# Simple-Robotics/aligator

Hardware: NVIDIA H100
Metric: riccati_knots_per_sec (higher is better)
Workload: dtype f64

## Files before the change

### aligator_b200/build.py

```python
from __future__ import annotations

import concurrent.futures as cf
import hashlib
import os
import re
import subprocess
import sys

PKG = os.path.dirname(os.path.abspath(__file__))
CSRC = os.path.join(PKG, "csrc")
OBJ = os.path.join(CSRC, "build")
LIB = os.path.join(PKG, "libaligator_b200_gar.so")
NVCC = os.environ.get("NVCC", "/usr/local/cuda/bin/nvcc")
ARCH = ["-gencode", "arch=compute_90a,code=sm_90a"]
FLAGS = ["-O3", "-lineinfo", "-std=c++17", "-Xcompiler", "-fPIC", "-ccbin", "/usr/bin/g++"]


def configs():
    txt = open(os.path.join(CSRC, "riccati_configs.h")).read()
    body = txt.split("#else", 1)[1]
    return [tuple(int(v) for v in m.groups())
            for m in re.finditer(r"X\((\d+),\s*(\d+),\s*(\d+),\s*(\d+)\)", body)]


def _digest(paths, extra=""):
    h = hashlib.sha256((" ".join(ARCH + FLAGS) + extra).encode())
    for p in paths:
        h.update(open(p, "rb").read())
    return h.hexdigest()[:16]


def _run(cmd):
    r = subprocess.run(cmd, capture_output=True, text=True)
    if r.returncode != 0:
        raise RuntimeError("build failed: %s\n%s\n%s" % (" ".join(cmd), r.stdout, r.stderr))
    return r.stdout + r.stderr


def build(verbose=False, force=False, ptxas_v=False):
    os.makedirs(OBJ, exist_ok=True)
    hdrs = [os.path.join(CSRC, f) for f in ("riccati_group.cuh", "riccati_launch.cuh", "riccati_configs.h")]
    hdrs.append(os.path.join(PKG, "..", "include", "aligator_b200", "gar.h"))
    hdrs_block = hdrs + [os.path.join(CSRC, f) for f in ("riccati_block.cuh", "riccati_block_launch.h",
                                                          "lq_assemble.h", "kkt_error.h", "linesearch.h",
                                                          "proxddp_inner.h")]
    extra = ["-Xptxas", "-v"] if ptxas_v else []
    jobs = []
    for (nx, nu, nc, g) in configs():
        src = os.path.join(CSRC, "kernel_inst.cu")
        tag = _digest(hdrs + [src], "%d_%d_%d_%d%s" % (nx, nu, nc, g, extra))
        obj = os.path.join(OBJ, "k_%d_%d_%d_%s.o" % (nx, nu, nc, tag))
        cmd = [NVCC] + ARCH + FLAGS + extra + ["-DAB2_NX=%d" % nx, "-DAB2_NU=%d" % nu, "-DAB2_NC=%d" % nc,
                                              "-DAB2_G=%d" % g, "-c", src, "-o", obj]
        jobs.append((obj, cmd))
    src = os.path.join(CSRC, "gar_cuda.cu")
    tag = _digest(hdrs_block + [src])
    obj = os.path.join(OBJ, "capi_%s.o" % tag)
    jobs.append((obj, [NVCC] + ARCH + FLAGS + ["-c", src, "-o", obj]))
    src = os.path.join(CSRC, "block_kernel.cu")
    obj = os.path.join(OBJ, "block_%s.o" % _digest(hdrs_block + [src], str(extra)))
    jobs.append((obj, [NVCC] + ARCH + FLAGS + extra + ["-c", src, "-o", obj]))
    src = os.path.join(CSRC, "kkt_error.cu")
    obj = os.path.join(OBJ, "kkt_%s.o" % _digest([os.path.join(CSRC, "kkt_error.h"), src], str(extra)))
    jobs.append((obj, [NVCC] + ARCH + FLAGS + extra + ["-c", src, "-o", obj]))
    src = os.path.join(CSRC, "lq_assemble.cu")
    obj = os.path.join(OBJ, "assemble_%s.o" % _digest([hdrs[-1], os.path.join(CSRC, "lq_assemble.h"), src], str(extra)))
    jobs.append((obj, [NVCC] + ARCH + FLAGS + extra + ["-c", src, "-o", obj]))
    src = os.path.join(CSRC, "linesearch.cu")
    obj = os.path.join(OBJ, "linesearch_%s.o" % _digest([os.path.join(CSRC, "linesearch.h"), src], str(extra)))
    jobs.append((obj, [NVCC] + ARCH + FLAGS + extra + ["-c", src, "-o", obj]))
    src = os.path.join(CSRC, "proxddp_inner.cu")
    obj = os.path.join(OBJ, "inner_%s.o" % _digest([hdrs[-1], os.path.join(CSRC, "proxddp_inner.h"), src], str(extra)))
    jobs.append((obj, [NVCC] + ARCH + FLAGS + extra + ["-c", src, "-o", obj]))
    todo =[(o, c) for (o, c) in jobs if force or not os.path.exists(o)]
    logs = []
    if todo:
        with cf.ThreadPoolExecutor(max_workers=max(1, min(len(todo), os.cpu_count() or 4))) as ex:
            for out in ex.map(lambda oc: _run(oc[1]), todo):
                logs.append(out)
    objs = [o for (o, _) in jobs]
    stamp = os.path.join(OBJ, "link.stamp")
    want = _digest(objs)
    if force or todo or not os.path.exists(LIB) or not os.path.exists(stamp) or open(stamp).read() != want:
        _run([NVCC] + ARCH + ["-shared", "-o", LIB] + objs + ["-ccbin", "/usr/bin/g++"])
        open(stamp, "w").write(want)
    keep = set(os.path.basename(o) for o in objs) | {"link.stamp"}
    for f in os.listdir(OBJ):
        if f not in keep:
            os.remove(os.path.join(OBJ, f))
    if verbose:
        print("\n".join(logs))
        print("built", LIB)
    return LIB


if __name__ == "__main__":
    build(verbose=True, force="--force" in sys.argv, ptxas_v="--ptxas" in sys.argv)
```

### aligator_b200/csrc/gar_cuda.cu

```cuda
#include <cuda_runtime.h>

#include <cstdio>
#include <cstdlib>
#include <cstring>
#include <string>
#include <vector>

#include "../../include/aligator_b200/gar.h"
#include "kkt_error.h"
#include "linesearch.h"
#include "lq_assemble.h"
#include "proxddp_inner.h"
#include "riccati_block_launch.h"
#include "riccati_configs.h"
#include "riccati_launch.cuh"

namespace ab2 {

__global__ void first_step_policy_kernel(const double *__restrict__ fb, const double *__restrict__ ff,
                                         double *__restrict__ dst, int batch, int N, int nr, int nu, int nx, int head) {
  const int per = nu * (nx + 1);
  for (long i = blockIdx.x * (long)blockDim.x + threadIdx.x; i < (long)batch * per; i += (long)gridDim.x * blockDim.x) {
    const int b = (int)(i / per), e = (int)(i % per), r = e / (nx + 1), c = e % (nx + 1);
    const size_t k0 = ((size_t)b * N + head) * nr + r;
    dst[i] = (c < nx) ? fb[k0 * nx + c] : ff[k0];
  }
}

constexpr int kMaxPeers = 8;
struct PeerPtrs {
  double *buf[kMaxPeers];
  unsigned long long *data_flag[kMaxPeers];
  unsigned long long *ack_flag[kMaxPeers];
};
__device__ __forceinline__ void st_release_sys(unsigned long long *p, unsigned long long v) {
  asm volatile("st.release.sys.global.u64 [%0], %1;" ::"l"(p), "l"(v) : "memory");
}
__device__ __forceinline__ unsigned long long ld_acquire_sys(const unsigned long long *p) {
  unsigned long long v;
  asm volatile("ld.acquire.sys.global.u64 %0, [%1];" : "=l"(v) : "l"(p) : "memory");
  return v;
}
__global__ void __launch_bounds__(256)
    policy_allgather_kernel(const double *__restrict__ fb, const double *__restrict__ ff, const PeerPtrs peers,
                            const int world, const int rank, const int batch, const int N, const int nr, const int nu,
                            const int nx, const unsigned long long step, unsigned int *done_counter) {
  const int per = nu * (nx + 1);
  const long total = (long)batch * per;
  if (threadIdx.x == 0) {
    if (step >= 3)
      for (int w = 0; w < world; ++w)
        while (ld_acquire_sys(peers.ack_flag[rank] + w) + 2 < step)
          __nanosleep(64);
  }
  __syncthreads();
  const size_t half = (size_t)(step % 3) * world * total;
  for (long i = blockIdx.x * (long)blockDim.x + threadIdx.x; i < total; i += (long)gridDim.x * blockDim.x) {
    const int b = (int)(i / per), e = (int)(i % per), r = e / (nx + 1), c = e % (nx + 1);
    const double v = (c < nx) ? fb[((size_t)b * N * nr + r) * nx + c] : ff[(size_t)b * N * nr + r];
    for (int w = 0; w < world; ++w)
      peers.buf[w][half + (size_t)rank * total + i] = v;
  }
  __threadfence_system();
  __syncthreads();
  if (threadIdx.x == 0) {
    const unsigned int prev = atomicAdd(done_counter, 1u);
    if (prev == gridDim.x - 1) {
      *done_counter = 0;
      __threadfence_system();
      for (int w = 0; w < world; ++w)
        st_release_sys(peers.data_flag[w] + rank, step);
    }
  }
}
__global__ void policy_publish_kernel(const PeerPtrs peers, const int world, const int rank, const unsigned long long step) {
  const int w = threadIdx.x;
  __threadfence_system();
  if (w < world) {
    st_release_sys(peers.data_flag[w] + rank, step);
    if (step >= 3)
      while (ld_acquire_sys(peers.ack_flag[rank] + w) + 2 < step)
        __nanosleep(64);
  }
}
__global__ void policy_wait_kernel(const PeerPtrs peers, const int world, const int rank, const unsigned long long step) {
  const int w = threadIdx.x;
  if (w < world) {
    st_release_sys(peers.ack_flag[w] + rank, step - 1);
    while (ld_acquire_sys(peers.data_flag[rank] + w) < step)
      __nanosleep(64);
  }
}

__global__ void gains_kernel(const double *__restrict__ fb, const double *__restrict__ ff, double *__restrict__ dst,
                             long nrec, int nr, int nx, int N, int head) {
  const int per = nr * (nx + 1);
  for (long i = blockIdx.x * (long)blockDim.x + threadIdx.x; i < nrec * per; i += (long)gridDim.x * blockDim.x) {
    long rec = i / per;
    if (head) {
      const long b = rec / N;
      const int t = (int)(rec % N) + head;
      rec = b * N + (t >= N ? t - N : t);
    }
    const int e = (int)(i % per), c = e / nr, r = e % nr;
    dst[i] = (c == 0) ? ff[rec * nr + r] : fb[(rec * nr + r) * nx + (c - 1)];
  }
}

__global__ void fddp_prep_kernel(const double *__restrict__ fs, double *__restrict__ slack, double *__restrict__ G0,
                                 double *__restrict__ g0, int batch, int N, int nx) {
  const long nS = (long)batch * N * nx, nG = (long)batch * nx * nx, ng = (long)batch * nx;
  for (long i = blockIdx.x * (long)blockDim.x + threadIdx.x; i < nS + nG + ng; i += (long)gridDim.x * blockDim.x) {
    if (i < nS) {
      const long b = i / ((long)N * nx), r = i % ((long)N * nx);
      slack[i] = fs[b * (N + 1) * nx + nx + r];
    } else if (i < nS + nG) {
      const long e = (i - nS) % ((long)nx * nx);
      G0[i - nS] = (e % nx == e / nx) ? -1.0 : 0.0;
    } else {
      const long j = i - nS - nG, b = j / nx, c = j % nx;
      g0[j] = fs[b * (N + 1) * nx + c];
    }
  }
}
__global__ void fddp_vx_kernel(const double *__restrict__ Vxx, const double *__restrict__ vx, const double *__restrict__ fs,
                               double *__restrict__ Vx_out, int batch, int N, int nx) {
  const long total = (long)batch * (N + 1) * nx;
  for (long i = blockIdx.x * (long)blockDim.x + threadIdx.x; i < total; i += (long)gridDim.x * blockDim.x) {
    const long kn = i / nx;
    const int r = (int)(i % nx);
    const double *V = Vxx + kn * nx * nx, *f = fs + kn * nx;
    double acc = 0.0;
    for (int c = 0; c < nx; ++c)
      acc += (r >= c ? V[r + (size_t)c * nx] : V[c + (size_t)r * nx]) * f[c];
    Vx_out[i] = vx[i] + acc;
  }
}
__global__ void fddp_quuks_kernel(const double *__restrict__ Ju, const double *__restrict__ Lu, const double *__restrict__ Vx,
                                  double *__restrict__ out, int batch, int N, int nx, int nu) {
  const long total = (long)batch * N * nu;
  for (long i = blockIdx.x * (long)blockDim.x + threadIdx.x; i < total; i += (long)gridDim.x * blockDim.x) {
    const long kn = i / nu, b = kn / N, t = kn % N;
    const int c = (int)(i % nu);
    const double *B = Ju + kn * nx * nu + (size_t)c * nx, *v = Vx + (b * (N + 1) + t + 1) * nx;
    double acc = Lu[i];
    for (int r = 0; r < nx; ++r)
      acc += B[r] * v[r];
    out[i] = -acc;
  }
}

#define X(NX, NU, NC, G) extern const KernelEntry kEntry_##NX##_##NU##_##NC;
AB2_FOR_EACH_CONFIG(X)
#undef X
static const KernelEntry *const kTable[] = {
#define X(NX, NU, NC, G) &kEntry_##NX##_##NU##_##NC,
    AB2_FOR_EACH_CONFIG(X)
#undef X
};

static const KernelEntry *find_kernel(int nx, int nu, int nc) {
  for (const KernelEntry *e : kTable)
    if (e->nx == nx && e->nu == nu && e->nc == nc)
      return e;
  return nullptr;
}

}

namespace {
thread_local std::string g_err;
int fail(int code, const std::string &msg) {
  g_err = msg;
  return code;
}
#define CUDA_TRY(expr)                                                                      \
  do {                                                                                      \
    cudaError_t _e = (expr);                                                                \
    if (_e != cudaSuccess)                                                                  \
      return fail(AB2_ERR_CUDA, std::string(#expr) + ": " + cudaGetErrorString(_e));        \
  } while (0)
}

struct ab2_gar_solver {
  ab2_gar_dims d;
  const ab2::KernelEntry *k;
  int srec, trec, nr;
  ab2::SweepParams p;
  double *own_stage = nullptr, *own_term = nullptr, *own_G0 = nullptr, *own_g0 = nullptr;
  double *own_stage_sym = nullptr;
  double *gains_tmp = nullptr, *kkt_tmp = nullptr, *theta_dev = nullptr, *ls_tmp = nullptr;
  double *fddp_slack = nullptr, *fddp_G0 = nullptr, *fddp_g0 = nullptr, *fddp_vx = nullptr;
  double *inner_tmp = nullptr;
  int nth = 0;
  int rec_nth = 0;
  int legs = 0;
  bool dense = false;
  int fac_head = 0;
  double *cond = nullptr;
  int pg_world = 0, pg_rank = 0;
  unsigned long long pg_step = 0;
  void *pg_local = nullptr;
  void *pg_peer_base[8] = {};
  ab2::PeerPtrs pg_ptrs{};
  unsigned int *pg_done = nullptr;
  size_t pg_buf_doubles = 0;
  unsigned long long pg_pushed_step = 0;
  bool pg_in_sweep = true;
  double *out[AB2_OUT_COUNT] = {};
  size_t out_doubles[AB2_OUT_COUNT] = {};
  size_t out_rec[AB2_OUT_COUNT] = {};
  int out_knots[AB2_OUT_COUNT] = {};
  int *status = nullptr, *pivstat = nullptr;
  bool have_problem = false, have_backward = false, have_forward = false;
  long launches = 0;
  int variant = -1;
  int group_doubles[4] = {0, 0, 0, 0};
  static constexpr int kPipeStreams = 4;
  cudaStream_t pipe_stream[kPipeStreams] = {};
  cudaEvent_t pipe_done[kPipeStreams] = {};
  cudaEvent_t pipe_fork = nullptr;
};

static size_t stage_total(const ab2_gar_solver *s) {
  return (size_t)s->d.batch * s->d.horizon * s->srec;
}

extern "C" {

const char *ab2_gar_last_error(void) { return g_err.c_str(); }
const char *ab2_gar_version(void) { return "aligator_b200 gar 0.1 (sm_90a)"; }

size_t ab2_gar_stage_record_doubles(int nx, int nu, int nc) {
  size_t n = 2 * (size_t)nx * nx + 2 * (size_t)nx * nu + (size_t)nu * nu + 2 * (size_t)nx + nu +
             (size_t)nc * (nx + nu + 1);
  return (n + 1) & ~(size_t)1;
}
size_t ab2_gar_term_record_doubles(int nx, int nct) {
  return (size_t)nx * nx + nx + (size_t)nct * nx + nct;
}
size_t ab2_gar_stage_record_doubles_th(int nx, int nu, int nc, int nth) {
  size_t n = 2 * (size_t)nx * nx + 2 * (size_t)nx * nu + (size_t)nu * nu + 2 * (size_t)nx + nu +
             (size_t)nc * (nx + nu + 1) + (size_t)nth * (nx + nu + nc + nth + 1);
  return (n + 1) & ~(size_t)1;
}
size_t ab2_gar_term_record_doubles_th(int nx, int nct, int nth) {
  return ab2_gar_term_record_doubles(nx, nct) + (size_t)nth * (nx + nct + nth + 1);
}
int ab2_gar_supported(int nx, int nu, int nc, int nc0) {
  if (nx < 1 || nu < 1 || nc < 0 || nc0 < 0)
    return 0;
  const ab2::KernelEntry *k = ab2::find_kernel(nx, nu, nc);
  if (k && nx + nc0 <= k->G)
    return 1;
  return ab2::block_supported(nx, nu, nc, nc0) ? 2 : 0;
}

static int create_impl(const ab2_gar_dims *dims, int nth, int legs, ab2_gar_solver **out);
int ab2_gar_create(const ab2_gar_dims *dims, ab2_gar_solver **out) { return create_impl(dims, 0, 0, out); }
int ab2_gar_create_parametric(const ab2_gar_dims *dims, int nth, ab2_gar_solver **out) {
  return create_impl(dims, nth, 0, out);
}
int ab2_gar_create_dense(const ab2_gar_dims *dims, ab2_gar_solver **out) { return create_impl(dims, 0, -1, out); }
int ab2_gar_create_parallel(const ab2_gar_dims *dims, int num_legs, ab2_gar_solver **out) {
  if (num_legs < 2)
    return fail(AB2_ERR_INVALID, "num_legs (" + std::to_string(num_legs) + ") should be greater than or equal to 2");
  if (dims && dims->horizon + 1 < num_legs)
    return fail(AB2_ERR_INVALID, "every leg needs at least one knot: horizon + 1 >= num_legs");
  return create_impl(dims, dims ? dims->nx : 0, num_legs, out);
}

static int create_impl(const ab2_gar_dims *dims, int nth, int legs, ab2_gar_solver **out) {
  if (!dims || !out)
    return fail(AB2_ERR_INVALID, "null argument");
  const ab2_gar_dims &d = *dims;
  if (d.nx < 1 || d.nu < 1 || d.nc < 0 || d.nct < 0 || d.nc0 < 0 || d.horizon < 0 || d.batch < 1 || nth < 0)
    return fail(AB2_ERR_INVALID, "bad dimensions");
  const bool dense = legs < 0;
  if (dense)
    legs = 0;
  const int rec_nth = legs > 1 ? 0 : nth;
  if (dense && !ab2::dense_supported(d.nx, d.nu, d.nc, d.nct, d.nc0))
    return fail(AB2_ERR_UNSUPPORTED, "the stage-dense KKT system (nu + nc + 2 nx rows) does not fit one CTA");
  const ab2::KernelEntry *k = ab2::find_kernel(d.nx, d.nu, d.nc);
  if (k && (d.nx + d.nc0 > k->G || nth > 0))
    k = nullptr;
  if (legs > 1 && !ab2::condensed_supported(d.nx, d.nc0, legs))
    return fail(AB2_ERR_UNSUPPORTED, "the condensed system of " + std::to_string(legs) + " legs does not fit one CTA's shared memory");
  if (!k && !ab2::block_supported(d.nx, d.nu, d.nc, d.nc0, nth))
    return fail(AB2_ERR_UNSUPPORTED,
                "(nx,nu,nc,nc0) = (" + std::to_string(d.nx) + "," + std::to_string(d.nu) + "," +
                    std::to_string(d.nc) + "," + std::to_string(d.nc0) +
                    ") does not fit one CTA (227 KB of shared memory, 256 rows)");
  int ndev = 0;
  CUDA_TRY(cudaGetDeviceCount(&ndev));
  if (d.device < 0 || d.device >= ndev)
    return fail(AB2_ERR_CUDA, "no such CUDA device");
  CUDA_TRY(cudaSetDevice(d.device));
  auto *s = new ab2_gar_solver();
  s->d = d;
  s->k = k;
  s->nth = nth;
  s->rec_nth = rec_nth;
  s->legs = legs;
  s->srec = (int)ab2_gar_stage_record_doubles_th(d.nx, d.nu, d.nc, rec_nth);
  if (k && k->srec_pad != s->srec) {
    delete s;
    return fail(AB2_ERR_INVALID, "internal: record size mismatch");
  }
  s->trec = (int)ab2_gar_term_record_doubles_th(d.nx, d.nct, rec_nth);
  s->nr = d.nu + d.nc + d.nx;
  s->dense = dense;
  if (dense) {
    s->k = nullptr;
    s->nr = d.nu + d.nc + 2 * d.nx;
  }
  if (s->k)
    s->k->group_doubles(d.nc0, s->group_doubles);
  const int N = d.horizon, B = d.batch, nx = d.nx;
  auto setup = [&](int what, size_t rec, int knots) {
    s->out_rec[what] = rec;
    s->out_knots[what] = knots;
    s->out_doubles[what] = (size_t)B * knots * rec;
  };
  setup(AB2_OUT_FF, s->nr, N);
  setup(AB2_OUT_FB, (size_t)s->nr * nx, N);
  setup(AB2_OUT_VXX, (size_t)nx * nx, N + 1);
  setup(AB2_OUT_VX, nx, N + 1);
  setup(AB2_OUT_FFT, d.nct, 1);
  setup(AB2_OUT_FBT, (size_t)d.nct * nx, 1);
  setup(AB2_OUT_KKT0, nx + d.nc0, 1);
  setup(AB2_OUT_XS, nx, N + 1);
  setup(AB2_OUT_US, d.nu, N);
  setup(AB2_OUT_VS, d.nc, N);
  setup(AB2_OUT_VST, d.nct, 1);
  setup(AB2_OUT_LBD0, d.nc0, 1);
  setup(AB2_OUT_LBDAS, nx, N);
  setup(AB2_OUT_FTH, (size_t)s->nr * nth, N);
  setup(AB2_OUT_VXT, (size_t)nx * nth, N + 1);
  setup(AB2_OUT_VTT, (size_t)nth * nth, N + 1);
  setup(AB2_OUT_VT, nth, N + 1);
  setup(AB2_OUT_KKT0FTH, (size_t)(nx + d.nc0) * nth, 1);
  setup(AB2_OUT_THGRAD, nth, 1);
  setup(AB2_OUT_THHESS, (size_t)nth * nth, 1);
  for (int w = 0; w < AB2_OUT_COUNT; ++w) {
    const size_t bytes = (s->out_doubles[w] > 0 ? s->out_doubles[w] + 2 : 2) * sizeof(double);
    cudaError_t e = cudaMalloc(&s->out[w], bytes);
    if (e == cudaSuccess)
      e = cudaMemset(s->out[w], 0, bytes);
    if (e != cudaSuccess) {
      ab2_gar_destroy(s);
      return fail(AB2_ERR_CUDA, std::string("cudaMalloc outputs: ") + cudaGetErrorString(e));
    }
  }
  {
    cudaError_t e = cudaMalloc(&s->status, sizeof(int) * B);
    if (e == cudaSuccess)
      e = cudaMemset(s->status, 0, sizeof(int) * B);
    if (e != cudaSuccess) {
      ab2_gar_destroy(s);
      return fail(AB2_ERR_CUDA, std::string("cudaMalloc status: ") + cudaGetErrorString(e));
    }
  }
  {
    cudaError_t e = cudaMalloc(&s->pivstat, sizeof(int) * B);
    if (e == cudaSuccess)
      e = cudaMemset(s->pivstat, 0, sizeof(int) * B);
    if (e != cudaSuccess) {
      ab2_gar_destroy(s);
      return fail(AB2_ERR_CUDA, std::string("cudaMalloc pivstat: ") + cudaGetErrorString(e));
    }
  }
  if (legs > 1) {
    const size_t td = (size_t)d.nc0 + (size_t)d.nx * (2 * legs - 1);
    cudaError_t e = cudaMalloc(&s->cond, sizeof(double) * B * td);
    if (e == cudaSuccess)
      e = cudaMemset(s->cond, 0, sizeof(double) * B * td);
    if (e != cudaSuccess) {
      ab2_gar_destroy(s);
      return fail(AB2_ERR_CUDA, std::string("cudaMalloc cond: ") + cudaGetErrorString(e));
    }
  }
  ab2::SweepParams &p = s->p;
  std::memset(&p, 0, sizeof(p));
  p.legs = legs;
  p.cond = s->cond;
  p.N = N;
  p.nct = d.nct;
  p.nc0 = d.nc0;
  p.batch = B;
  p.ff = s->out[AB2_OUT_FF];
  p.fb = s->out[AB2_OUT_FB];
  p.Vxx = s->out[AB2_OUT_VXX];
  p.vx = s->out[AB2_OUT_VX];
  p.ffT = s->out[AB2_OUT_FFT];
  p.fbT = s->out[AB2_OUT_FBT];
  p.kkt0 = s->out[AB2_OUT_KKT0];
  p.xs = s->out[AB2_OUT_XS];
  p.us = s->out[AB2_OUT_US];
  p.vs = s->out[AB2_OUT_VS];
  p.vsT = s->out[AB2_OUT_VST];
  p.lbd0 = s->out[AB2_OUT_LBD0];
  p.lbdas = s->out[AB2_OUT_LBDAS];
  p.status = s->status;
  p.pivstat = s->pivstat;
  p.nth = nth;
  p.theta = nullptr;
  p.fth = s->out[AB2_OUT_FTH];
  p.Vxt = s->out[AB2_OUT_VXT];
  p.Vtt = s->out[AB2_OUT_VTT];
  p.vt = s->out[AB2_OUT_VT];
  p.kkt0fth = s->out[AB2_OUT_KKT0FTH];
  p.thGrad = s->out[AB2_OUT_THGRAD];
  p.thHess = s->out[AB2_OUT_THHESS];
  {
    int sms = 0;
    cudaDeviceGetAttribute(&sms, cudaDevAttrMultiProcessorCount, d.device);
    p.num_sms = sms > 0 ? sms : 132;
  }
  if (const char *f = std::getenv("AB2_PEER_IN_SWEEP"))
    s->pg_in_sweep = std::atoi(f) != 0;
  if (const char *f = std::getenv("AB2_DEBUG_FLAGS"))
    p.dbg = std::atoi(f);
  if (std::getenv("AB2_PHASE_CLOCKS")) {
    cudaMalloc(&p.clk, 16 * sizeof(long long));
    cudaMemset(p.clk, 0, 16 * sizeof(long long));
  }
  *out = s;
  return AB2_OK;
}

int ab2_gar_destroy(ab2_gar_solver *s) {
  if (!s)
    return AB2_OK;
  cudaSetDevice(s->d.device);
  for (int w = 0; w < AB2_OUT_COUNT; ++w)
    if (s->out[w])
      cudaFree(s->out[w]);
  if (s->status)
    cudaFree(s->status);
  if (s->pivstat)
    cudaFree(s->pivstat);
  for (int w = 0; w < s->pg_world; ++w)
    if (w != s->pg_rank && s->pg_peer_base[w])
      cudaIpcCloseMemHandle(s->pg_peer_base[w]);
  if (s->pg_local)
    cudaFree(s->pg_local);
  if (s->pg_done)
    cudaFree(s->pg_done);
  for (double *q : {s->own_stage_sym, s->own_stage, s->own_term, s->own_G0, s->own_g0, s->gains_tmp, s->kkt_tmp, s->theta_dev, s->cond, s->ls_tmp, s->fddp_slack, s->fddp_G0,
                    s->fddp_g0, s->fddp_vx, s->inner_tmp})
    if (q)
      cudaFree(q);
  for (int i = 0; i < ab2_gar_solver::kPipeStreams; ++i) {
    if (s->pipe_done[i])
      cudaEventDestroy(s->pipe_done[i]);
    if (s->pipe_stream[i])
      cudaStreamDestroy(s->pipe_stream[i]);
  }
  if (s->pipe_fork)
    cudaEventDestroy(s->pipe_fork);
  delete s;
  return AB2_OK;
}

int ab2_gar_set_tuning(ab2_gar_solver *s, const ab2_gar_tuning *t) {
  if (!s || !t)
    return fail(AB2_ERR_INVALID, "null argument");
  if (t->variant < -1 || t->variant > 10)
    return fail(AB2_ERR_INVALID, "variant must be -1 (default) or 0..10");
  if (t->variant == 9 && !ab2::block_supported(s->d.nx, s->d.nu, s->d.nc, s->d.nc0))
    return fail(AB2_ERR_UNSUPPORTED, "variant 9 (CTA per instance) does not fit this shape");
  if (t->stagger_ns < 0 || t->stagger_ns > 100000 || t->ctas_per_sm < 0 || t->ctas_per_sm > 32)
    return fail(AB2_ERR_INVALID, "stagger_ns must be in [0, 100000], ctas_per_sm in [0, 32]");
  s->variant = t->variant;
  s->p.stagger_ns = t->stagger_ns;
  s->p.ctas_per_sm = t->ctas_per_sm;
  return AB2_OK;
}

int ab2_gar_set_problem(ab2_gar_solver *s, const double *stage, const double *term, const double *G0,
                        const double *g0, int memspace, void *stream) {
  if (!s)
    return fail(AB2_ERR_INVALID, "null solver");
  CUDA_TRY(cudaSetDevice(s->d.device));
  cudaStream_t st = (cudaStream_t)stream;
  const size_t n_stage = stage_total(s), n_term = (size_t)s->d.batch * s->trec,
               n_G0 = (size_t)s->d.batch * s->d.nc0 * s->d.nx, n_g0 = (size_t)s->d.batch * s->d.nc0;
  if (memspace == AB2_DEVICE) {
    if (stage) {
      s->p.stage = stage;
      s->p.stage_head = 0;
    }
    if (term)
      s->p.term = term;
    if (G0)
      s->p.G0 = G0;
    if (g0)
      s->p.g0 = g0;
  } else if (memspace == AB2_HOST) {
    auto up = [&](double *&own, const double *src, size_t n, const double *&dst) -> int {
      if (!src)
        return AB2_OK;
      if (!own)
        CUDA_TRY(cudaMalloc(&own, (n > 0 ? n : 1) * sizeof(double)));
      if (n)
        CUDA_TRY(cudaMemcpyAsync(own, src, n * sizeof(double), cudaMemcpyHostToDevice, st));
      dst = own;
      return AB2_OK;
    };
    int rc;
    if ((rc = up(s->own_stage, stage, n_stage, s->p.stage)) != AB2_OK)
      return rc;
    if (stage)
      s->p.stage_head = 0;
    if ((rc = up(s->own_term, term, n_term, s->p.term)) != AB2_OK)
      return rc;
    if ((rc = up(s->own_G0, G0, n_G0, s->p.G0)) != AB2_OK)
      return rc;
    if ((rc = up(s->own_g0, g0, n_g0, s->p.g0)) != AB2_OK)
      return rc;
  } else {
    return fail(AB2_ERR_INVALID, "memspace must be AB2_HOST or AB2_DEVICE");
  }
  s->have_problem = s->p.stage && s->p.term && (s->p.G0 || s->d.nc0 == 0) && (s->p.g0 || s->d.nc0 == 0);
  if (s->d.horizon == 0 && s->p.term)
    s->have_problem = true;
  return AB2_OK;
}

static ab2::SweepParams slice_params(const ab2_gar_solver *s, int b0, int nb) {
  ab2::SweepParams q = s->p;
  const size_t b = (size_t)b0;
  const int N = s->d.horizon, nx = s->d.nx;
  q.batch = nb;
  q.stage += b * N * s->srec;
  q.term += b * s->trec;
  if (q.G0)
    q.G0 += b * s->d.nc0 * nx;
  if (q.g0)
    q.g0 += b * s->d.nc0;
  q.ff += b * s->out_knots[AB2_OUT_FF] * s->out_rec[AB2_OUT_FF];
  q.fb += b * s->out_knots[AB2_OUT_FB] * s->out_rec[AB2_OUT_FB];
  q.Vxx += b * s->out_knots[AB2_OUT_VXX] * s->out_rec[AB2_OUT_VXX];
  q.vx += b * s->out_knots[AB2_OUT_VX] * s->out_rec[AB2_OUT_VX];
  q.ffT += b * s->out_rec[AB2_OUT_FFT];
  q.fbT += b * s->out_rec[AB2_OUT_FBT];
  q.kkt0 += b * s->out_rec[AB2_OUT_KKT0];
  q.xs += b * s->out_knots[AB2_OUT_XS] * s->out_rec[AB2_OUT_XS];
  q.us += b * s->out_knots[AB2_OUT_US] * s->out_rec[AB2_OUT_US];
  q.vs += b * s->out_knots[AB2_OUT_VS] * s->out_rec[AB2_OUT_VS];
  q.vsT += b * s->out_rec[AB2_OUT_VST];
  q.lbd0 += b * s->out_rec[AB2_OUT_LBD0];
  q.lbdas += b * s->out_knots[AB2_OUT_LBDAS] * s->out_rec[AB2_OUT_LBDAS];
  q.status += b;
  q.pivstat += b;
  if (s->nth > 0) {
    q.fth += b * s->out_knots[AB2_OUT_FTH] * s->out_rec[AB2_OUT_FTH];
    q.Vxt += b * s->out_knots[AB2_OUT_VXT] * s->out_rec[AB2_OUT_VXT];
    q.Vtt += b * s->out_knots[AB2_OUT_VTT] * s->out_rec[AB2_OUT_VTT];
    q.vt += b * s->out_knots[AB2_OUT_VT] * s->out_rec[AB2_OUT_VT];
    q.kkt0fth += b * s->out_rec[AB2_OUT_KKT0FTH];
    q.thGrad += b * s->out_rec[AB2_OUT_THGRAD];
    q.thHess += b * s->out_rec[AB2_OUT_THHESS];
    if (q.theta)
      q.theta += b * s->nth;
  }
  if (q.cond)
    q.cond += b * ((size_t)s->d.nc0 + (size_t)nx * (2 * s->legs - 1));
  return q;
}

static int run_kernels(ab2_gar_solver *s, ab2::SweepParams q, int bwd, int fwd, cudaStream_t st) {
  if (s->legs > 1) {
    if (bwd) {
      CUDA_TRY(cudaMemsetAsync(q.status, 0, sizeof(int) * q.batch, st));
      CUDA_TRY(cudaMemsetAsync(q.pivstat, 0, sizeof(int) * q.batch, st));
      q.do_bwd = 1;
      q.do_fwd = 0;
      CUDA_TRY(ab2::launch_block(q, s->d.nx, s->d.nu, s->d.nc, st, nullptr));
      CUDA_TRY(ab2::launch_condensed(q, s->d.nx, st));
      s->launches += 2;
    }
    if (fwd) {
      q.do_bwd = 0;
      q.do_fwd = 1;
      CUDA_TRY(ab2::launch_block(q, s->d.nx, s->d.nu, s->d.nc, st, nullptr));
      s->launches += 1;
    }
    return AB2_OK;
  }
  q.do_bwd = bwd;
  q.do_fwd = fwd;
  if (s->dense)
    CUDA_TRY(ab2::launch_dense(q, s->d.nx, s->d.nu, s->d.nc, st));
  else if (s->k && s->variant != 9)
    CUDA_TRY(s->k->launch(q, s->variant, s->group_doubles, st, nullptr));
  else
    CUDA_TRY(ab2::launch_block(q, s->d.nx, s->d.nu, s->d.nc, st, nullptr));
  s->launches += 1;
  return AB2_OK;
}

static int launch(ab2_gar_solver *s, double mueq, int bwd, int fwd, void *stream) {
  if (!s)
    return fail(AB2_ERR_INVALID, "null solver");
  if (!s->have_problem)
    return fail(AB2_ERR_STATE, "set_problem has not been called with all four buffers");
  if (fwd && !bwd && !s->have_backward)
    return fail(AB2_ERR_STATE, "forward() before backward()");
  if (bwd && !(mueq > 0.0) && (s->d.nc > 0 || s->d.nct > 0))
    return fail(AB2_ERR_INVALID, "mueq must be > 0 when constraints are present");
  CUDA_TRY(cudaSetDevice(s->d.device));
  s->p.mueq = mueq;
  s->p.do_bwd = bwd;
  s->p.do_fwd = fwd;
  ab2::SweepParams q = s->p;
  q.peer_world = 0;
  if (bwd && s->pg_in_sweep && s->pg_peer_base[0] && s->k && s->variant != 9 && s->legs <= 1 && !s->dense &&
      s->d.horizon > 0) {
    const unsigned long long step = s->pg_step + 1;
    const size_t total = (size_t)s->d.batch * s->d.nu * (s->d.nx + 1);
    q.peer_world = s->pg_world;
    for (int w = 0; w < s->pg_world; ++w)
      q.peer_dst[w] = s->pg_ptrs.buf[w];
    q.peer_off = (long long)((step % 3) * s->pg_world * total + (size_t)s->pg_rank * total);
    s->pg_pushed_step = step;
  }
  if (int rc = run_kernels(s, q, bwd, fwd, (cudaStream_t)stream))
    return rc;
  if (bwd) {
    s->have_backward = true;
    s->fac_head = 0;
  }
  s->have_forward = fwd != 0;
  return AB2_OK;
}

int ab2_gar_backward(ab2_gar_solver *s, double mueq, void *stream) { return launch(s, mueq, 1, 0, stream); }
int ab2_gar_forward(ab2_gar_solver *s, void *stream) { return launch(s, s ? s->p.mueq : 0.0, 0, 1, stream); }
int ab2_gar_sweep(ab2_gar_solver *s, double mueq, void *stream) { return launch(s, mueq, 1, 1, stream); }
int ab2_gar_forward_theta(ab2_gar_solver *s, const double *theta, int memspace, void *stream) {
  if (!s)
    return fail(AB2_ERR_INVALID, "null solver");
  if (theta && (s->nth == 0 || s->legs > 1))
    return fail(AB2_ERR_INVALID, "theta given to a solver without parameters (nth = 0; the parallel solver ignores theta, parallel-solver.hxx:211)");
  CUDA_TRY(cudaSetDevice(s->d.device));
  s->p.theta = nullptr;
  if (theta) {
    if (memspace == AB2_DEVICE) {
      s->p.theta = theta;
    } else {
      if (!s->theta_dev)
        CUDA_TRY(cudaMalloc(&s->theta_dev, (size_t)s->d.batch * s->nth * sizeof(double)));
      CUDA_TRY(cudaMemcpyAsync(s->theta_dev, theta, (size_t)s->d.batch * s->nth * sizeof(double),
                               cudaMemcpyHostToDevice, (cudaStream_t)stream));
      s->p.theta = s->theta_dev;
    }
  }
  const int rc = launch(s, s->p.mueq, 0, 1, stream);
  s->p.theta = nullptr;
  return rc;
}

int ab2_gar_assemble(ab2_gar_solver *s, const ab2_lq_inputs *in, void *stream) {
  if (!s || !in)
    return fail(AB2_ERR_INVALID, "null argument");
  if (s->rec_nth > 0)
    return fail(AB2_ERR_UNSUPPORTED, "assemble: parametric problems (nth > 0) are not supported");
  const ab2_gar_dims &d = s->d;
  const bool stage_ok = d.horizon == 0 || (in->Jx && in->Ju && in->slack && in->Lxx && in->Lxu && in->Luu &&
                                           in->Lx && in->Lu);
  const bool cstr_ok = d.nc == 0 || d.horizon == 0 || (in->cJx && in->cJu && in->Lv && in->shifted && in->lo && in->hi);
  const bool hess_ok = (!in->Hxx && !in->Hxu && !in->Huu) || (in->Hxx && in->Hxu && in->Huu);
  const bool term_ok = in->Lxx_N && in->Lx_N &&
                       (d.nct == 0 || (in->cJx_N && in->Lv_N && in->shifted_N && in->loN && in->hiN));
  const bool init_ok = d.nc0 == 0 || (in->G0 && in->g0);
  if (!stage_ok || !cstr_ok || !hess_ok || !term_ok || !init_ok)
    return fail(AB2_ERR_INVALID, "ab2_lq_inputs: a required array is NULL for these dimensions");
  CUDA_TRY(cudaSetDevice(d.device));
  auto own = [&](double *&buf, size_t n) -> int {
    if (!buf)
      CUDA_TRY(cudaMalloc(&buf, (n > 0 ? n : 1) * sizeof(double)));
    return AB2_OK;
  };
  int rc;
  if ((rc = own(s->own_stage, stage_total(s))) != AB2_OK || (rc = own(s->own_term, (size_t)d.batch * s->trec)) != AB2_OK ||
      (rc = own(s->own_G0, (size_t)d.batch * d.nc0 * d.nx)) != AB2_OK || (rc = own(s->own_g0, (size_t)d.batch * d.nc0)) != AB2_OK)
    return rc;
  CUDA_TRY(ab2::launch_lq_assemble(*in, s->own_stage, s->own_term, s->own_G0, s->own_g0, d.batch, d.horizon, d.nx,
                                   d.nu, d.nc, d.nct, d.nc0, s->srec, s->trec, (cudaStream_t)stream));
  s->launches += d.horizon > 0 ? 2 : 1;
  s->p.stage = s->own_stage;
  s->p.stage_head = 0;
  s->p.term = s->own_term;
  s->p.G0 = s->own_G0;
  s->p.g0 = s->own_g0;
  s->have_problem = true;
  return AB2_OK;
}

static int copy_ring(const double *base, size_t rec, int knots, int nring, int head, int b0, int nb, int t0, int nt,
                     double *dst, cudaMemcpyKind kind, cudaStream_t st);

int ab2_gar_problem_ptr(ab2_gar_solver *s, int what, const double **out) {
  if (!s || !out || what < 0 || what > 3)
    return fail(AB2_ERR_INVALID, "bad argument");
  const double *ptrs[4] = {s->p.stage, s->p.term, s->p.G0, s->p.g0};
  *out = ptrs[what];
  return AB2_OK;
}

int ab2_gar_get_problem(ab2_gar_solver *s, int what, double *dst, int memspace, void *stream) {
  if (!s || !dst || what < 0 || what > 3)
    return fail(AB2_ERR_INVALID, "bad argument");
  if (!s->have_problem)
    return fail(AB2_ERR_STATE, "no problem set");
  const double *ptrs[4] = {s->p.stage, s->p.term, s->p.G0, s->p.g0};
  const size_t n[4] = {stage_total(s), (size_t)s->d.batch * s->trec, (size_t)s->d.batch * s->d.nc0 * s->d.nx,
                       (size_t)s->d.batch * s->d.nc0};
  CUDA_TRY(cudaSetDevice(s->d.device));
  if (what == 0 && s->p.stage_head != 0 && n[0])
    return copy_ring(s->p.stage, (size_t)s->srec, s->d.horizon, s->d.horizon, s->p.stage_head, 0, s->d.batch, 0,
                     s->d.horizon, dst, memspace == AB2_DEVICE ? cudaMemcpyDeviceToDevice : cudaMemcpyDeviceToHost,
                     (cudaStream_t)stream);
  if (n[what])
    CUDA_TRY(cudaMemcpyAsync(dst, ptrs[what], n[what] * sizeof(double),
                             memspace == AB2_DEVICE ? cudaMemcpyDeviceToDevice : cudaMemcpyDeviceToHost,
                             (cudaStream_t)stream));
  return AB2_OK;
}

static inline __host__ __device__ int sym_source(int e, int nx, int nu, int nc) {
  const int off_q = nx * nx + nx * nu + nx, tq = nx * (nx + 1) / 2, tr = nu * (nu + 1) / 2;
  if (e < off_q)
    return e;
  e -= off_q;
  if (e < nx * nx) {
    int i = e % nx, j = e / nx;
    if (i < j) {
      const int t = i;
      i = j;
      j = t;
    }
    return off_q + j * nx - j * (j - 1) / 2 + (i - j);
  }
  e -= nx * nx;
  if (e < nx * nu)
    return off_q + tq + e;
  e -= nx * nu;
  if (e < nu * nu) {
    int i = e % nu, j = e / nu;
    if (i < j) {
      const int t = i;
      i = j;
      j = t;
    }
    return off_q + tq + nx * nu + j * nu - j * (j - 1) / 2 + (i - j);
  }
  e -= nu * nu;
  return off_q + tq + nx * nu + tr + e;
}
namespace ab2 {
__global__ void __launch_bounds__(256) expand_sym_kernel(const double *__restrict__ src, double *__restrict__ dst, const long nrec,
                                                         const int nx, const int nu, const int nc, const int srec_full,
                                                         const int srec_pad, const int srec_sym) {
  extern __shared__ int lut[];
  for (int e = threadIdx.x; e < srec_pad; e += blockDim.x)
    lut[e] = e < srec_full ? sym_source(e, nx, nu, nc) : -1;
  __syncthreads();
  const long total = nrec * srec_pad;
  for (long i = blockIdx.x * (long)blockDim.x + threadIdx.x; i < total; i += (long)gridDim.x * blockDim.x) {
    const long r = i / srec_pad;
    const int e = (int)(i - r * srec_pad), o = lut[e];
    dst[i] = o >= 0 ? src[r * srec_sym + o] : 0.0;
  }
}
}

size_t ab2_gar_stage_record_doubles_sym(int nx, int nu, int nc) {
  if (nx < 1 || nu < 0 || nc < 0)
    return 0;
  return (size_t)nx * nx + (size_t)nx * nu + nx + (size_t)nx * (nx + 1) / 2 + (size_t)nx * nu + (size_t)nu * (nu + 1) / 2 + nx + nu +
         (size_t)nc * nx + (size_t)nc * nu + nc;
}

int ab2_gar_pack_stage_sym(int nx, int nu, int nc, const double *stage, double *stage_sym, long nrec) {
  if (!stage || !stage_sym || nrec < 0 || nx < 1 || nu < 0 || nc < 0)
    return fail(AB2_ERR_INVALID, "bad argument");
  const int full = nx * nx + nx * nu + nx + nx * nx + nx * nu + nu * nu + nx + nu + nc * nx + nc * nu + nc;
  const size_t pad = ab2_gar_stage_record_doubles(nx, nu, nc), sym = ab2_gar_stage_record_doubles_sym(nx, nu, nc);
  std::vector<int> dst_of(sym, 0);
  for (int e = full - 1; e >= 0; --e) {
    const int off_q = nx * nx + nx * nu + nx;
    int keep = 1;
    int r = e - off_q;
    if (r >= 0 && r < nx * nx)
      keep = (r % nx) >= (r / nx);
    r -= nx * nx + nx * nu;
    if (r >= 0 && r < nu * nu)
      keep = (r % nu) >= (r / nu);
    if (keep)
      dst_of[sym_source(e, nx, nu, nc)] = e;
  }
  for (long k = 0; k < nrec; ++k)
    for (size_t o = 0; o < sym; ++o)
      stage_sym[(size_t)k * sym + o] = stage[(size_t)k * pad + dst_of[o]];
  return AB2_OK;
}

static int sweep_host_impl(ab2_gar_solver *s, const double *stage, const double *term, const double *G0,
                           const double *g0, double mueq, int nchunks, const int *whats,
                           double *const *dsts, int nwhat, void *stream, bool sym);
int ab2_gar_sweep_host(ab2_gar_solver *s, const double *stage, const double *term, const double *G0,
                       const double *g0, double mueq, int nchunks, const int *whats,
                       double *const *dsts, int nwhat, void *stream) {
  return sweep_host_impl(s, stage, term, G0, g0, mueq, nchunks, whats, dsts, nwhat, stream, false);
}
int ab2_gar_sweep_host_sym(ab2_gar_solver *s, const double *stage_sym, const double *term, const double *G0,
                           const double *g0, double mueq, int nchunks, const int *whats,
                           double *const *dsts, int nwhat, void *stream) {
  if (s && (s->rec_nth > 0 || s->legs > 1 || s->dense))
    return fail(AB2_ERR_UNSUPPORTED, "sweep_host_sym: plain (nth = 0) serial handles only");
  return sweep_host_impl(s, stage_sym, term, G0, g0, mueq, nchunks, whats, dsts, nwhat, stream, true);
}

static int sweep_host_impl(ab2_gar_solver *s, const double *stage, const double *term, const double *G0,
                           const double *g0, double mueq, int nchunks, const int *whats,
                           double *const *dsts, int nwhat, void *stream, const bool sym) {
  if (!s || !stage || !term || (s->d.nc0 > 0 && (!G0 || !g0)) || nwhat < 0 || (nwhat > 0 && (!whats || !dsts)))
    return fail(AB2_ERR_INVALID, "bad argument");
  for (int i = 0; i < nwhat; ++i)
    if (whats[i] < 0 || whats[i] >= AB2_OUT_COUNT || !dsts[i])
      return fail(AB2_ERR_INVALID, "bad output selector");
  if (!(mueq > 0.0) && (s->d.nc > 0 || s->d.nct > 0))
    return fail(AB2_ERR_INVALID, "mueq must be > 0 when constraints are present");
  CUDA_TRY(cudaSetDevice(s->d.device));
  const int B = s->d.batch, N = s->d.horizon, nx = s->d.nx, nc0 = s->d.nc0;
  constexpr int NS = ab2_gar_solver::kPipeStreams;
  if (!s->pipe_fork) {
    CUDA_TRY(cudaEventCreateWithFlags(&s->pipe_fork, cudaEventDisableTiming));
    for (int i = 0; i < NS; ++i) {
      CUDA_TRY(cudaStreamCreateWithFlags(&s->pipe_stream[i], cudaStreamNonBlocking));
      CUDA_TRY(cudaEventCreateWithFlags(&s->pipe_done[i], cudaEventDisableTiming));
    }
  }
  auto own = [&](double *&buf, size_t n) -> int {
    if (!buf)
      CUDA_TRY(cudaMalloc(&buf, (n > 0 ? n : 1) * sizeof(double)));
    return AB2_OK;
  };
  int rc;
  if ((rc = own(s->own_stage, stage_total(s))) != AB2_OK || (rc = own(s->own_term, (size_t)B * s->trec)) != AB2_OK ||
      (rc = own(s->own_G0, (size_t)B * nc0 * nx)) != AB2_OK || (rc = own(s->own_g0, (size_t)B * nc0)) != AB2_OK)
    return rc;
  const size_t srec_sym = ab2_gar_stage_record_doubles_sym(nx, s->d.nu, s->d.nc);
  if (sym && (rc = own(s->own_stage_sym, (size_t)B * N * srec_sym)) != AB2_OK)
    return rc;
  s->p.stage = s->own_stage;
  s->p.stage_head = 0;
  s->p.term = s->own_term;
  s->p.G0 = s->own_G0;
  s->p.g0 = s->own_g0;
  s->have_problem = true;
  s->p.mueq = mueq;
  s->p.do_bwd = 1;
  s->p.do_fwd = 1;
  if (nchunks <= 0) {
    nchunks = B / 512;
    if (nchunks > 16)
      nchunks = 16;
  }
  if (nchunks < 1)
    nchunks = 1;
  if (nchunks > B)
    nchunks = B;
  cudaStream_t user = (cudaStream_t)stream;
  CUDA_TRY(cudaEventRecord(s->pipe_fork, user));
  for (int i = 0; i < NS && i < nchunks; ++i)
    CUDA_TRY(cudaStreamWaitEvent(s->pipe_stream[i], s->pipe_fork, 0));
  for (int c = 0; c < nchunks; ++c) {
    const int b0 = (int)((long long)B * c / nchunks), b1 = (int)((long long)B * (c + 1) / nchunks);
    const int nb = b1 - b0;
    if (nb <= 0)
      continue;
    cudaStream_t st = s->pipe_stream[c % NS];
    auto up = [&](double *dev, const double *host, size_t per_inst) -> int {
      if (per_inst)
        CUDA_TRY(cudaMemcpyAsync(dev + (size_t)b0 * per_inst, host + (size_t)b0 * per_inst,
                                 (size_t)nb * per_inst * sizeof(double), cudaMemcpyHostToDevice, st));
      return AB2_OK;
    };
    if ((rc = up(s->own_term, term, s->trec)) != AB2_OK ||
        (rc = up(s->own_G0, G0, (size_t)nc0 * nx)) != AB2_OK || (rc = up(s->own_g0, g0, nc0)) != AB2_OK)
      return rc;
    if (sym) {
      if ((rc = up(s->own_stage_sym, stage, (size_t)N * srec_sym)) != AB2_OK)
        return rc;
      const long nrec = (long)nb * N;
      if (nrec > 0) {
        const int full = nx * nx + nx * s->d.nu + nx + nx * nx + nx * s->d.nu + s->d.nu * s->d.nu + nx + s->d.nu +
                         s->d.nc * nx + s->d.nc * s->d.nu + s->d.nc;
        long blocks = (nrec * (long)s->srec + 255) / 256;
        if (blocks > s->p.num_sms * 8L)
          blocks = s->p.num_sms * 8L;
        static bool carve = false;
        if (!carve) {
          CUDA_TRY(cudaFuncSetAttribute(ab2::expand_sym_kernel, cudaFuncAttributePreferredSharedMemoryCarveout,
                                        (int)cudaSharedmemCarveoutMaxShared));
          carve = true;
        }
        if (s->srec * sizeof(int) > 48 * 1024)
          CUDA_TRY(cudaFuncSetAttribute(ab2::expand_sym_kernel, cudaFuncAttributeMaxDynamicSharedMemorySize,
                                        (int)(s->srec * sizeof(int))));
        ab2::expand_sym_kernel<<<(int)blocks, 256, s->srec * sizeof(int), st>>>(
            s->own_stage_sym + (size_t)b0 * N * srec_sym, s->own_stage + (size_t)b0 * N * s->srec, nrec, nx, s->d.nu, s->d.nc,
            full, (int)s->srec, (int)srec_sym);
        CUDA_TRY(cudaGetLastError());
        s->launches += 1;
      }
    } else if ((rc = up(s->own_stage, stage, (size_t)N * s->srec)) != AB2_OK)
      return rc;
    const ab2::SweepParams q = slice_params(s, b0, nb);
    if (int rc2 = run_kernels(s, q, 1, 1, st))
      return rc2;
    for (int i = 0; i < nwhat; ++i) {
      const int w = whats[i];
      const size_t per_inst = (size_t)s->out_knots[w] * s->out_rec[w];
      if (per_inst)
        CUDA_TRY(cudaMemcpyAsync(dsts[i] + (size_t)b0 * per_inst, s->out[w] + (size_t)b0 * per_inst,
                                 (size_t)nb * per_inst * sizeof(double), cudaMemcpyDeviceToHost, st));
    }
  }
  for (int i = 0; i < NS && i < nchunks; ++i) {
    CUDA_TRY(cudaEventRecord(s->pipe_done[i], s->pipe_stream[i]));
    CUDA_TRY(cudaStreamWaitEvent(user, s->pipe_done[i], 0));
  }
  s->have_backward = true;
  s->have_forward = true;
  s->fac_head = 0;
  return AB2_OK;
}

size_t ab2_gar_output_doubles(const ab2_gar_solver *s, int what) {
  if (!s || what < 0 || what >= AB2_OUT_COUNT)
    return 0;
  return s->out_doubles[what];
}

static int copy_ring(const double *base, size_t rec, int knots, int nring, int head, int b0, int nb, int t0, int nt,
                     double *dst, cudaMemcpyKind kind, cudaStream_t st) {
  auto piece = [&](int lt, int pt, int len) -> int {
    if (len <= 0)
      return AB2_OK;
    CUDA_TRY(cudaMemcpy2DAsync(dst + (size_t)(lt - t0) * rec, (size_t)nt * rec * sizeof(double),
                               base + ((size_t)b0 * knots + pt) * rec, (size_t)knots * rec * sizeof(double),
                               (size_t)len * rec * sizeof(double), (size_t)nb, kind, st));
    return AB2_OK;
  };
  const int t1 = t0 + nt;
  auto clip = [&](int lo, int hi, int shift) {
    const int a = t0 > lo ? t0 : lo, b = t1 < hi ? t1 : hi;
    return piece(a, a + shift, b - a);
  };
  int rc;
  if ((rc = clip(0, nring - head, head)) != AB2_OK || (rc = clip(nring - head, nring, head - nring)) != AB2_OK ||
      (rc = clip(nring, knots, 0)) != AB2_OK)
    return rc;
  return AB2_OK;
}
static bool ring_indexed(const ab2_gar_solver *s, int what) {
  return s->fac_head != 0 && (what == AB2_OUT_FF || what == AB2_OUT_FB || what == AB2_OUT_VXX || what == AB2_OUT_VX);
}

int ab2_gar_get(ab2_gar_solver *s, int what, double *dst, int memspace, void *stream) {
  if (!s || !dst || what < 0 || what >= AB2_OUT_COUNT)
    return fail(AB2_ERR_INVALID, "bad argument");
  CUDA_TRY(cudaSetDevice(s->d.device));
  if (s->out_doubles[what] == 0)
    return AB2_OK;
  if (ring_indexed(s, what))
    return copy_ring(s->out[what], s->out_rec[what], s->out_knots[what], s->d.horizon, s->fac_head, 0, s->d.batch, 0,
                     s->out_knots[what], dst, memspace == AB2_DEVICE ? cudaMemcpyDeviceToDevice : cudaMemcpyDeviceToHost,
                     (cudaStream_t)stream);
  CUDA_TRY(cudaMemcpyAsync(dst, s->out[what], s->out_doubles[what] * sizeof(double),
                           memspace == AB2_DEVICE ? cudaMemcpyDeviceToDevice : cudaMemcpyDeviceToHost,
                           (cudaStream_t)stream));
  return AB2_OK;
}

int ab2_gar_get_range(ab2_gar_solver *s, int what, int b0, int nb, int t0, int nt, double *dst,
                      int memspace, void *stream) {
  if (!s || !dst || what < 0 || what >= AB2_OUT_COUNT)
    return fail(AB2_ERR_INVALID, "bad argument");
  const int knots = s->out_knots[what];
  if (b0 < 0 || nb < 0 || b0 + nb > s->d.batch || t0 < 0 || nt < 0 || t0 + nt > knots)
    return fail(AB2_ERR_INVALID, "range out of bounds");
  CUDA_TRY(cudaSetDevice(s->d.device));
  const size_t rec = s->out_rec[what];
  if (rec == 0 || nb == 0 || nt == 0)
    return AB2_OK;
  if (ring_indexed(s, what))
    return copy_ring(s->out[what], rec, knots, s->d.horizon, s->fac_head, b0, nb, t0, nt, dst,
                     memspace == AB2_DEVICE ? cudaMemcpyDeviceToDevice : cudaMemcpyDeviceToHost, (cudaStream_t)stream);
  const double *src = s->out[what] + ((size_t)b0 * knots + t0) * rec;
  CUDA_TRY(cudaMemcpy2DAsync(dst, (size_t)nt * rec * sizeof(double), src, (size_t)knots * rec * sizeof(double),
                             (size_t)nt * rec * sizeof(double), (size_t)nb,
                             memspace == AB2_DEVICE ? cudaMemcpyDeviceToDevice : cudaMemcpyDeviceToHost,
                             (cudaStream_t)stream));
  return AB2_OK;
}

int ab2_gar_first_step_policy(ab2_gar_solver *s, double *dst, void *stream) {
  if (!s || !dst)
    return fail(AB2_ERR_INVALID, "bad argument");
  if (s->d.horizon < 1)
    return fail(AB2_ERR_INVALID, "first_step_policy needs horizon >= 1");
  if (s->dense)
    return fail(AB2_ERR_UNSUPPORTED, "first_step_policy: not offered by the stage-dense solver");
  if (!s->have_backward)
    return fail(AB2_ERR_STATE, "first_step_policy before backward()");
  CUDA_TRY(cudaSetDevice(s->d.device));
  const long total = (long)s->d.batch * s->d.nu * (s->d.nx + 1);
  const int threads = 256;
  long blocks = (total + threads - 1) / threads;
  if (blocks > s->p.num_sms * 8L)
    blocks = s->p.num_sms * 8L;
  ab2::first_step_policy_kernel<<<(int)blocks, threads, 0, (cudaStream_t)stream>>>(
      s->out[AB2_OUT_FB], s->out[AB2_OUT_FF], dst, s->d.batch, s->d.horizon, s->nr, s->d.nu, s->d.nx, s->fac_head);
  CUDA_TRY(cudaGetLastError());
  s->launches += 1;
  return AB2_OK;
}

int ab2_gar_get_gains(ab2_gar_solver *s, double *dst, int memspace, void *stream) {
  if (!s || !dst)
    return fail(AB2_ERR_INVALID, "bad argument");
  if (!s->have_backward)
    return fail(AB2_ERR_STATE, "get_gains before backward()");
  if (s->dense)
    return fail(AB2_ERR_UNSUPPORTED, "get_gains: the results_.gains_ layout is the proximal solver's");
  CUDA_TRY(cudaSetDevice(s->d.device));
  const long nrec = (long)s->d.batch * s->d.horizon;
  const size_t total = (size_t)nrec * s->nr * (s->d.nx + 1);
  if (total == 0)
    return AB2_OK;
  double *out = dst;
  if (memspace != AB2_DEVICE) {
    if (!s->gains_tmp)
      CUDA_TRY(cudaMalloc(&s->gains_tmp, total * sizeof(double)));
    out = s->gains_tmp;
  }
  long blocks = ((long)total + 255) / 256;
  if (blocks > s->p.num_sms * 8L)
    blocks = s->p.num_sms * 8L;
  ab2::gains_kernel<<<(int)blocks, 256, 0, (cudaStream_t)stream>>>(s->out[AB2_OUT_FB], s->out[AB2_OUT_FF], out, nrec,
                                                                    s->nr, s->d.nx, s->d.horizon, s->fac_head);
  CUDA_TRY(cudaGetLastError());
  s->launches += 1;
  if (memspace != AB2_DEVICE)
    CUDA_TRY(cudaMemcpyAsync(dst, out, total * sizeof(double), cudaMemcpyDeviceToHost, (cudaStream_t)stream));
  return AB2_OK;
}

int ab2_gar_kkt_error(ab2_gar_solver *s, double mueq, double *dst, int memspace, void *stream) {
  if (!s || !dst)
    return fail(AB2_ERR_INVALID, "bad argument");
  if (!s->have_problem || !s->have_backward || !s->have_forward)
    return fail(AB2_ERR_STATE, "kkt_error needs a problem and a completed sweep (no forward pass since the last backward)");
  if (s->rec_nth > 0)
    return fail(AB2_ERR_UNSUPPORTED, "kkt_error: parametric problems (nth > 0) are not supported");
  CUDA_TRY(cudaSetDevice(s->d.device));
  if (!s->kkt_tmp)
    CUDA_TRY(cudaMalloc(&s->kkt_tmp, (size_t)s->d.batch * 3 * sizeof(double)));
  ab2::KktErrorArgs a;
  a.batch = s->d.batch;
  a.N = s->d.horizon;
  a.nx = s->d.nx;
  a.nu = s->d.nu;
  a.nc = s->d.nc;
  a.nct = s->d.nct;
  a.nc0 = s->d.nc0;
  a.srec = s->srec;
  a.trec = s->trec;
  a.stage_head = s->p.stage_head;
  a.mueq = mueq;
  a.stage = s->p.stage;
  a.term = s->p.term;
  a.G0 = s->p.G0;
  a.g0 = s->p.g0;
  a.xs = s->out[AB2_OUT_XS];
  a.us = s->out[AB2_OUT_US];
  a.vs = s->out[AB2_OUT_VS];
  a.vsT = s->out[AB2_OUT_VST];
  a.lbd0 = s->out[AB2_OUT_LBD0];
  a.lbdas = s->out[AB2_OUT_LBDAS];
  a.out = (memspace == AB2_DEVICE) ? dst : s->kkt_tmp;
  CUDA_TRY(ab2::launch_kkt_error(a, (cudaStream_t)stream));
  s->launches += 1;
  if (memspace != AB2_DEVICE)
    CUDA_TRY(cudaMemcpyAsync(dst, s->kkt_tmp, (size_t)s->d.batch * 3 * sizeof(double), cudaMemcpyDeviceToHost,
                             (cudaStream_t)stream));
  return AB2_OK;
}

int ab2_gar_device_ptr(ab2_gar_solver *s, int what, double **out) {
  if (!s || !out || what < 0 || what >= AB2_OUT_COUNT)
    return fail(AB2_ERR_INVALID, "bad argument");
  *out = s->out[what];
  return AB2_OK;
}

int ab2_gar_status(ab2_gar_solver *s, int *dst, int memspace, void *stream) {
  if (!s || !dst)
    return fail(AB2_ERR_INVALID, "bad argument");
  CUDA_TRY(cudaSetDevice(s->d.device));
  CUDA_TRY(cudaMemcpyAsync(dst, s->status, sizeof(int) * s->d.batch,
                           memspace == AB2_DEVICE ? cudaMemcpyDeviceToDevice : cudaMemcpyDeviceToHost,
                           (cudaStream_t)stream));
  return AB2_OK;
}

static ab2::LineSearchArgs ls_args(const ab2_gar_solver *s) {
  ab2::LineSearchArgs a;
  a.batch = s->d.batch;
  a.N = s->d.horizon;
  a.nx = s->d.nx;
  a.nu = s->d.nu;
  a.nc = s->d.nc;
  a.nct = s->d.nct;
  a.nc0 = s->d.nc0;
  a.dxs = s->out[AB2_OUT_XS];
  a.dus = s->out[AB2_OUT_US];
  a.dvs = s->out[AB2_OUT_VS];
  a.dvsT = s->out[AB2_OUT_VST];
  a.dlam0 = s->out[AB2_OUT_LBD0];
  a.dlams = s->out[AB2_OUT_LBDAS];
  return a;
}
static int ls_result(ab2_gar_solver *s, double *dst, int memspace, cudaStream_t st, double **dev) {
  if (memspace == AB2_DEVICE) {
    *dev = dst;
    return AB2_OK;
  }
  if (!s->ls_tmp)
    CUDA_TRY(cudaMalloc(&s->ls_tmp, (size_t)s->d.batch * sizeof(double)));
  *dev = s->ls_tmp;
  (void)st;
  return AB2_OK;
}
int ab2_gar_linear_step(ab2_gar_solver *s, double alpha, const ab2_ls_iterate *cur, const ab2_ls_trial *trial,
                        void *stream) {
  if (!s || !cur || !trial)
    return fail(AB2_ERR_INVALID, "null argument");
  if (!s->have_forward)
    return fail(AB2_ERR_STATE, "linear_step needs the step of a forward pass");
  const ab2_gar_dims &d = s->d;
  const bool ok = cur->xs && trial->xs && (d.horizon == 0 || (cur->us && trial->us && cur->lams && trial->lams)) &&
                  (d.nc == 0 || d.horizon == 0 || (cur->vs && trial->vs)) && (d.nct == 0 || (cur->vsT && trial->vsT)) &&
                  (d.nc0 == 0 || (cur->lam0 && trial->lam0));
  if (!ok)
    return fail(AB2_ERR_INVALID, "linear_step: a required array is NULL for these dimensions");
  CUDA_TRY(cudaSetDevice(d.device));
  ab2::LinearStepIO io{cur->xs, cur->us, cur->vs, cur->vsT, cur->lam0, cur->lams,
                       trial->xs, trial->us, trial->vs, trial->vsT, trial->lam0, trial->lams};
  CUDA_TRY(ab2::launch_linear_step(ls_args(s), io, alpha, (cudaStream_t)stream));
  s->launches += 1;
  return AB2_OK;
}
int ab2_gar_directional_derivative(ab2_gar_solver *s, const double *Lxs, const double *Lus, double *dst, int memspace,
                                   void *stream) {
  if (!s || !Lxs || !dst || (s->d.horizon > 0 && !Lus))
    return fail(AB2_ERR_INVALID, "null argument");
  if (!s->have_forward)
    return fail(AB2_ERR_STATE, "directional_derivative needs the step of a forward pass");
  CUDA_TRY(cudaSetDevice(s->d.device));
  double *dev = nullptr;
  if (int rc = ls_result(s, dst, memspace, (cudaStream_t)stream, &dev))
    return rc;
  CUDA_TRY(ab2::launch_directional_derivative(ls_args(s), Lxs, Lus, dev, (cudaStream_t)stream));
  s->launches += 1;
  if (memspace != AB2_DEVICE)
    CUDA_TRY(cudaMemcpyAsync(dst, dev, (size_t)s->d.batch * sizeof(double), cudaMemcpyDeviceToHost, (cudaStream_t)stream));
  return AB2_OK;
}
int ab2_gar_al_value(ab2_gar_solver *s, const ab2_ls_iterate *plus, const double *cost, double mudyn, double mucstr,
                     double *dst, int memspace, void *stream) {
  if (!s || !plus || !dst)
    return fail(AB2_ERR_INVALID, "null argument");
  const ab2_gar_dims &d = s->d;
  if ((d.nc0 > 0 && !plus->lam0) || (d.horizon > 0 && !plus->lams) || (d.nc > 0 && d.horizon > 0 && !plus->vs) ||
      (d.nct > 0 && !plus->vsT))
    return fail(AB2_ERR_INVALID, "al_value: a required multiplier array is NULL for these dimensions");
  CUDA_TRY(cudaSetDevice(d.device));
  double *dev = nullptr;
  if (int rc = ls_result(s, dst, memspace, (cudaStream_t)stream, &dev))
    return rc;
  CUDA_TRY(ab2::launch_al_value(d.batch, d.horizon, d.nx, d.nc, d.nct, d.nc0, plus->lam0, plus->lams, plus->vs, plus->vsT,
                                cost, mudyn, mucstr, dev, (cudaStream_t)stream));
  s->launches += 1;
  if (memspace != AB2_DEVICE)
    CUDA_TRY(cudaMemcpyAsync(dst, dev, (size_t)d.batch * sizeof(double), cudaMemcpyDeviceToHost, (cudaStream_t)stream));
  return AB2_OK;
}

static ab2::InnerDims inner_dims(const ab2_gar_solver *s) {
  const ab2_gar_dims &d = s->d;
  return ab2::InnerDims{d.batch, d.horizon, d.nx, d.nu, d.nc, d.nct, d.nc0};
}
static int inner_result(ab2_gar_solver *s, double *dst, int memspace, double **dev) {
  if (memspace == AB2_DEVICE) {
    *dev = dst;
    return AB2_OK;
  }
  if (!s->inner_tmp)
    CUDA_TRY(cudaMalloc(&s->inner_tmp, (size_t)s->d.batch * 2 * sizeof(double)));
  *dev = s->inner_tmp;
  return AB2_OK;
}
int ab2_gar_multipliers(ab2_gar_solver *s, const ab2_mult_inputs *in, const ab2_mult_outputs *out, double *dst,
                        int memspace, void *stream) {
  if (!s || !in || !out || !dst)
    return fail(AB2_ERR_INVALID, "null argument");
  const ab2_gar_dims &d = s->d;
  const bool stages = d.horizon > 0;
  if (stages && (in->xnext != nullptr) == (in->fs != nullptr))
    return fail(AB2_ERR_INVALID, "multipliers: give exactly one of xnext and fs");
  const bool ok = (!stages || ((in->fs || in->xs) && in->lams && out->slack && out->lams_plus)) &&
                  (d.nc0 == 0 || (in->init_value && in->lam0 && out->lam0_plus)) &&
                  (d.nc == 0 || !stages ||
                   (in->vs && in->prev_vs && in->cval && in->lo && in->hi && out->vs_plus && out->shifted && out->Lv)) &&
                  (d.nct == 0 || (in->vsT && in->prev_vsT && in->cval_N && in->loN && in->hiN && out->vsT_plus &&
                                  out->shifted_N && out->Lv_N));
  if (!ok)
    return fail(AB2_ERR_INVALID, "multipliers: a required array is NULL for these dimensions");
  if (!(in->mu > 0.0) || !(in->mu_dyn > 0.0))
    return fail(AB2_ERR_INVALID, "multipliers: mu and mu_dyn must be positive");
  CUDA_TRY(cudaSetDevice(d.device));
  double *dev = nullptr;
  if (int rc = inner_result(s, dst, memspace, &dev))
    return rc;
  CUDA_TRY(ab2::launch_multipliers(inner_dims(s), *in, *out, dev, (cudaStream_t)stream));
  s->launches += 1;
  if (memspace != AB2_DEVICE)
    CUDA_TRY(cudaMemcpyAsync(dst, dev, (size_t)d.batch * 2 * sizeof(double), cudaMemcpyDeviceToHost, (cudaStream_t)stream));
  return AB2_OK;
}
int ab2_gar_lagrangian_gradient(ab2_gar_solver *s, const ab2_lag_inputs *in, const ab2_lag_outputs *out, void *stream) {
  if (!s || !in || !out)
    return fail(AB2_ERR_INVALID, "null argument");
  const ab2_gar_dims &d = s->d;
  const bool stages = d.horizon > 0;
  if (!out->Lx && !out->Lx_N && !out->Lu && !out->Lxs && !out->Lus)
    return fail(AB2_ERR_INVALID, "lagrangian_gradient: no output array given");
  const bool ok = in->lx_N && (!stages || (in->lx && in->lu && in->Jx && in->Ju && in->lams)) &&
                  (d.nc == 0 || !stages || (in->cJx && in->cJu && in->vs)) && (d.nct == 0 || (in->cJx_N && in->vsT)) &&
                  (d.nc0 == 0 || (in->G0 && in->lam0));
  if (!ok)
    return fail(AB2_ERR_INVALID, "lagrangian_gradient: a required input array is NULL for these dimensions");
  CUDA_TRY(cudaSetDevice(d.device));
  CUDA_TRY(ab2::launch_lagrangian_gradient(inner_dims(s), *in, *out, (cudaStream_t)stream));
  s->launches += 1;
  return AB2_OK;
}
int ab2_gar_criterion(ab2_gar_solver *s, const double *Lxs, const double *Lus, const double *init_value,
                      const double *slack, const double *Lv, const double *Lv_N, double *dst, int memspace,
                      void *stream) {
  if (!s || !dst)
    return fail(AB2_ERR_INVALID, "null argument");
  const ab2_gar_dims &d = s->d;
  const bool stages = d.horizon > 0;
  const bool ok = Lxs && (!stages || Lus) && (d.nc0 == 0 || !stages || init_value) && (d.horizon < 2 || slack) &&
                  (d.nc == 0 || !stages || Lv) && (d.nct == 0 || Lv_N);
  if (!ok)
    return fail(AB2_ERR_INVALID, "criterion: a required array is NULL for these dimensions");
  CUDA_TRY(cudaSetDevice(d.device));
  double *dev = nullptr;
  if (int rc = inner_result(s, dst, memspace, &dev))
    return rc;
  CUDA_TRY(ab2::launch_criterion(inner_dims(s), Lxs, Lus, init_value, slack, Lv, Lv_N, dev, (cudaStream_t)stream));
  s->launches += 1;
  if (memspace != AB2_DEVICE)
    CUDA_TRY(cudaMemcpyAsync(dst, dev, (size_t)d.batch * 2 * sizeof(double), cudaMemcpyDeviceToHost, (cudaStream_t)stream));
  return AB2_OK;
}

int ab2_fddp_backward_pass(ab2_gar_solver *s, const ab2_fddp_inputs *in, double *Vx_out, double *Quuks_out, void *stream) {
  if (!s || !in)
    return fail(AB2_ERR_INVALID, "null argument");
  const ab2_gar_dims &d = s->d;
  if (d.nc != 0 || d.nct != 0 || d.nc0 != d.nx || s->rec_nth != 0 || s->legs > 1 || d.horizon < 1)
    return fail(AB2_ERR_INVALID, "fddp_backward_pass needs a serial solver with nc = nct = 0, nc0 = nx, horizon >= 1");
  if (!in->Jx || !in->Ju || !in->fs || !in->Lxx || !in->Lxu || !in->Luu || !in->Lx || !in->Lu || !in->Lxx_N || !in->Lx_N)
    return fail(AB2_ERR_INVALID, "ab2_fddp_inputs: a required array is NULL");
  CUDA_TRY(cudaSetDevice(d.device));
  cudaStream_t st = (cudaStream_t)stream;
  const int B = d.batch, N = d.horizon, nx = d.nx, nu = d.nu;
  auto own = [&](double *&buf, size_t n) -> int {
    if (!buf)
      CUDA_TRY(cudaMalloc(&buf, (n > 0 ? n : 1) * sizeof(double)));
    return AB2_OK;
  };
  int rc;
  if ((rc = own(s->fddp_slack, (size_t)B * N * nx)) != AB2_OK || (rc = own(s->fddp_G0, (size_t)B * nx * nx)) != AB2_OK ||
      (rc = own(s->fddp_g0, (size_t)B * nx)) != AB2_OK || (rc = own(s->fddp_vx, (size_t)B * (N + 1) * nx)) != AB2_OK)
    return rc;
  ab2::fddp_prep_kernel<<<s->p.num_sms * 4, 256, 0, st>>>(in->fs, s->fddp_slack, s->fddp_G0, s->fddp_g0, B, N, nx);
  CUDA_TRY(cudaGetLastError());
  s->launches += 1;
  ab2_lq_inputs lq;
  std::memset(&lq, 0, sizeof(lq));
  lq.Jx = in->Jx;
  lq.Ju = in->Ju;
  lq.slack = s->fddp_slack;
  lq.Lxx = in->Lxx;
  lq.Lxu = in->Lxu;
  lq.Luu = in->Luu;
  lq.Lx = in->Lx;
  lq.Lu = in->Lu;
  lq.Lxx_N = in->Lxx_N;
  lq.Lx_N = in->Lx_N;
  lq.G0 = s->fddp_G0;
  lq.g0 = s->fddp_g0;
  lq.preg = in->preg;
  lq.mu_inv = 1.0;
  if ((rc = ab2_gar_assemble(s, &lq, stream)) != AB2_OK)
    return rc;
  if ((rc = ab2_gar_backward(s, 1.0, stream)) != AB2_OK)
    return rc;
  double *vxo = Vx_out ? Vx_out : s->fddp_vx;
  ab2::fddp_vx_kernel<<<s->p.num_sms * 4, 256, 0, st>>>(s->out[AB2_OUT_VXX], s->out[AB2_OUT_VX], in->fs, vxo, B, N, nx);
  CUDA_TRY(cudaGetLastError());
  s->launches += 1;
  if (Quuks_out) {
    ab2::fddp_quuks_kernel<<<s->p.num_sms * 4, 256, 0, st>>>(in->Ju, in->Lu, vxo, Quuks_out, B, N, nx, nu);
    CUDA_TRY(cudaGetLastError());
    s->launches += 1;
  }
  return AB2_OK;
}

int ab2_gar_collapse_feedback(ab2_gar_solver *s, void *stream) {
  if (!s)
    return fail(AB2_ERR_INVALID, "null solver");
  if (s->legs <= 1)
    return AB2_OK;
  if (!s->have_backward)
    return fail(AB2_ERR_STATE, "collapse_feedback before backward()");
  if (s->d.horizon < 1)
    return AB2_OK;
  CUDA_TRY(cudaSetDevice(s->d.device));
  CUDA_TRY(ab2::launch_collapse(s->p, s->d.nx, s->d.nu, s->d.nc, (cudaStream_t)stream));
  s->launches += 1;
  return AB2_OK;
}

int ab2_gar_pivot_stats(ab2_gar_solver *s, int *dst, int memspace, void *stream) {
  if (!s || !dst)
    return fail(AB2_ERR_INVALID, "bad argument");
  if (!s->have_backward)
    return fail(AB2_ERR_STATE, "pivot_stats before backward()");
  CUDA_TRY(cudaSetDevice(s->d.device));
  CUDA_TRY(cudaMemcpyAsync(dst, s->pivstat, sizeof(int) * s->d.batch,
                           memspace == AB2_DEVICE ? cudaMemcpyDeviceToDevice : cudaMemcpyDeviceToHost,
                           (cudaStream_t)stream));
  return AB2_OK;
}

int ab2_gar_cycle_append(ab2_gar_solver *s, const double *new_last, int memspace, void *stream) {
  if (!s || !new_last)
    return fail(AB2_ERR_INVALID, "bad argument");
  const int N = s->d.horizon, B = s->d.batch;
  if (N < 1)
    return fail(AB2_ERR_INVALID, "cycle_append needs horizon >= 1");
  if (s->rec_nth > 0)
    return fail(AB2_ERR_UNSUPPORTED, "cycle_append: parametric problems (nth > 0) are not supported");
  CUDA_TRY(cudaSetDevice(s->d.device));
  cudaStream_t st = (cudaStream_t)stream;
  if (s->legs > 1) {
    for (int w : {AB2_OUT_FF, AB2_OUT_FB, AB2_OUT_VXX, AB2_OUT_VX, AB2_OUT_FTH, AB2_OUT_VXT, AB2_OUT_VTT, AB2_OUT_VT})
      if (s->out_doubles[w])
        CUDA_TRY(cudaMemsetAsync(s->out[w], 0, s->out_doubles[w] * sizeof(double), st));
  }
  if (s->legs <= 1) {
    s->fac_head = (s->fac_head + 1) % N;
    const int slot = (N - 1 + s->fac_head) % N;
    for (int w : {AB2_OUT_FF, AB2_OUT_FB, AB2_OUT_VXX, AB2_OUT_VX}) {
      const size_t rec = s->out_rec[w];
      if (rec == 0)
        continue;
      CUDA_TRY(cudaMemset2DAsync(s->out[w] + (size_t)slot * rec, (size_t)s->out_knots[w] * rec * sizeof(double), 0,
                                 rec * sizeof(double), (size_t)B, st));
    }
  }
  if (s->out_doubles[AB2_OUT_KKT0])
    CUDA_TRY(cudaMemsetAsync(s->out[AB2_OUT_KKT0], 0, s->out_doubles[AB2_OUT_KKT0] * sizeof(double), st));
  if (s->own_stage && s->p.stage == s->own_stage) {
    s->p.stage_head = (s->p.stage_head + 1) % N;
    const int slot = (N - 1 + s->p.stage_head) % N;
    CUDA_TRY(cudaMemcpy2DAsync(s->own_stage + (size_t)slot * s->srec, (size_t)N * s->srec * sizeof(double),
                               new_last, (size_t)s->srec * sizeof(double), (size_t)s->srec * sizeof(double),
                               (size_t)B,
                               memspace == AB2_DEVICE ? cudaMemcpyDeviceToDevice : cudaMemcpyHostToDevice, st));
  }
  CUDA_TRY(cudaGetLastError());
  s->have_backward = false;
  s->have_forward = false;
  return AB2_OK;
}

int ab2_gar_phase_clocks(ab2_gar_solver *s, long long *dst16) {
  if (!s || !dst16 || !s->p.clk)
    return fail(AB2_ERR_STATE, "phase clocks are off (set AB2_PHASE_CLOCKS=1 before create)");
  CUDA_TRY(cudaMemcpy(dst16, s->p.clk, 16 * sizeof(long long), cudaMemcpyDeviceToHost));
  CUDA_TRY(cudaMemset(s->p.clk, 0, 16 * sizeof(long long)));
  return AB2_OK;
}

int ab2_gar_ring_heads(const ab2_gar_solver *s, int *factor_head, int *stage_head) {
  if (!s)
    return fail(AB2_ERR_INVALID, "null solver");
  if (factor_head)
    *factor_head = s->fac_head;
  if (stage_head)
    *stage_head = s->p.stage_head;
  return AB2_OK;
}

int ab2_gar_synchronize(ab2_gar_solver *s, void *stream) {
  if (!s)
    return fail(AB2_ERR_INVALID, "null solver");
  CUDA_TRY(cudaSetDevice(s->d.device));
  CUDA_TRY(cudaStreamSynchronize((cudaStream_t)stream));
  return AB2_OK;
}

int ab2_gar_peer_gather_init(ab2_gar_solver *s, int world, int rank, void *ipc_handle_out) {
  if (!s || !ipc_handle_out || world < 1 || world > ab2::kMaxPeers || rank < 0 || rank >= world)
    return fail(AB2_ERR_INVALID, "peer_gather_init: bad argument (world <= 8)");
  if (s->d.horizon < 1)
    return fail(AB2_ERR_INVALID, "peer_gather needs horizon >= 1");
  if (s->pg_local)
    return fail(AB2_ERR_STATE, "peer_gather_init called twice");
  CUDA_TRY(cudaSetDevice(s->d.device));
  const size_t per = (size_t)s->d.nu * (s->d.nx + 1);
  s->pg_buf_doubles = 3 * (size_t)world * s->d.batch * per;
  const size_t bytes = s->pg_buf_doubles * sizeof(double) + 2 * ab2::kMaxPeers * sizeof(unsigned long long);
  CUDA_TRY(cudaMalloc(&s->pg_local, bytes));
  CUDA_TRY(cudaMemset(s->pg_local, 0, bytes));
  CUDA_TRY(cudaMalloc(&s->pg_done, sizeof(unsigned int)));
  CUDA_TRY(cudaMemset(s->pg_done, 0, sizeof(unsigned int)));
  s->pg_world = world;
  s->pg_rank = rank;
  cudaIpcMemHandle_t h;
  CUDA_TRY(cudaIpcGetMemHandle(&h, s->pg_local));
  static_assert(sizeof(h) == 64, "IPC handle size");
  std::memcpy(ipc_handle_out, &h, sizeof(h));
  return AB2_OK;
}

int ab2_gar_peer_gather_connect(ab2_gar_solver *s, const void *all_handles) {
  if (!s || !all_handles || !s->pg_local)
    return fail(AB2_ERR_STATE, "peer_gather_connect before peer_gather_init");
  CUDA_TRY(cudaSetDevice(s->d.device));
  for (int w = 0; w < s->pg_world; ++w) {
    void *base = s->pg_local;
    if (w != s->pg_rank) {
      cudaIpcMemHandle_t h;
      std::memcpy(&h, (const char *)all_handles + 64 * (size_t)w, sizeof(h));
      const cudaError_t e = cudaIpcOpenMemHandle(&base, h, cudaIpcMemLazyEnablePeerAccess);
      if (e != cudaSuccess) {
        cudaGetLastError();
        for (int v = 0; v < w; ++v) {
          if (v != s->pg_rank && s->pg_peer_base[v])
            cudaIpcCloseMemHandle(s->pg_peer_base[v]);
          s->pg_peer_base[v] = nullptr;
        }
        return fail(AB2_ERR_CUDA, std::string("peer_gather_connect: cudaIpcOpenMemHandle(rank ") + std::to_string(w) +
                                      "): " + cudaGetErrorString(e));
      }
    }
    s->pg_peer_base[w] = base;
    s->pg_ptrs.buf[w] = (double *)base;
    unsigned long long *fl = (unsigned long long *)((double *)base + s->pg_buf_doubles);
    s->pg_ptrs.data_flag[w] = fl;
    s->pg_ptrs.ack_flag[w] = fl + ab2::kMaxPeers;
  }
  return AB2_OK;
}

int ab2_gar_policy_allgather(ab2_gar_solver *s, void *stream) {
  if (!s || !s->pg_peer_base[0])
    return fail(AB2_ERR_STATE, "policy_allgather before peer_gather_connect");
  if (!s->have_backward)
    return fail(AB2_ERR_STATE, "policy_allgather before backward()");
  CUDA_TRY(cudaSetDevice(s->d.device));
  const long total = (long)s->d.batch * s->d.nu * (s->d.nx + 1);
  long blocks = (total + 255) / 256;
  if (blocks > s->p.num_sms * 2L)
    blocks = s->p.num_sms * 2L;
  s->pg_step += 1;
  if (s->pg_pushed_step == s->pg_step)
    ab2::policy_publish_kernel<<<1, 32, 0, (cudaStream_t)stream>>>(s->pg_ptrs, s->pg_world, s->pg_rank, s->pg_step);
  else
    ab2::policy_allgather_kernel<<<(int)blocks, 256, 0, (cudaStream_t)stream>>>(
        s->out[AB2_OUT_FB], s->out[AB2_OUT_FF], s->pg_ptrs, s->pg_world, s->pg_rank, s->d.batch, s->d.horizon, s->nr,
        s->d.nu, s->d.nx, s->pg_step, s->pg_done);
  CUDA_TRY(cudaGetLastError());
  s->launches += 1;
  return AB2_OK;
}

int ab2_gar_policy_allgather_wait(ab2_gar_solver *s, void *stream) {
  if (!s || !s->pg_peer_base[0] || s->pg_step == 0)
    return fail(AB2_ERR_STATE, "policy_allgather_wait before policy_allgather");
  CUDA_TRY(cudaSetDevice(s->d.device));
  static bool carve = false;
  if (!carve) {
    CUDA_TRY(cudaFuncSetAttribute(ab2::policy_wait_kernel, cudaFuncAttributePreferredSharedMemoryCarveout,
                                  (int)cudaSharedmemCarveoutMaxShared));
    carve = true;
  }
  ab2::policy_wait_kernel<<<1, 32, 0, (cudaStream_t)stream>>>(s->pg_ptrs, s->pg_world, s->pg_rank, s->pg_step);
  CUDA_TRY(cudaGetLastError());
  s->launches += 1;
  return AB2_OK;
}

int ab2_gar_peer_gather_buffer(ab2_gar_solver *s, double **out, long *step) {
  if (!s || !out || !s->pg_local)
    return fail(AB2_ERR_STATE, "peer_gather_buffer before peer_gather_init");
  const size_t half = (size_t)(s->pg_step % 3) * s->pg_world * s->d.batch * s->d.nu * (s->d.nx + 1);
  *out = (double *)s->pg_local + half;
  if (step)
    *step = (long)s->pg_step;
  return AB2_OK;
}

int ab2_gar_pinned_alloc(size_t bytes, void **out) {
  if (!out)
    return fail(AB2_ERR_INVALID, "null argument");
  *out = nullptr;
  CUDA_TRY(cudaHostAlloc(out, bytes > 0 ? bytes : 1, cudaHostAllocPortable));
  return AB2_OK;
}
void ab2_gar_pinned_free(void *p) {
  if (p)
    cudaFreeHost(p);
}

long ab2_gar_launch_count(const ab2_gar_solver *s) { return s ? s->launches : 0; }

int ab2_gar_kernel_info(const ab2_gar_solver *s, int *group_lanes, int *smem_bytes_per_cta,
                        int *threads_per_cta, int *grid, int *regs_per_thread) {
  if (!s)
    return fail(AB2_ERR_INVALID, "null solver");
  int info[6] = {0, 0, 0, 0, 0, 0};
  CUDA_TRY(cudaSetDevice(s->d.device));
  if (s->k && s->variant != 9)
    CUDA_TRY(s->k->launch(s->p, s->variant, s->group_doubles, 0, info));
  else
    CUDA_TRY(ab2::launch_block(s->p, s->d.nx, s->d.nu, s->d.nc, 0, info));
  if (group_lanes)
    *group_lanes = info[0];
  if (smem_bytes_per_cta)
    *smem_bytes_per_cta = info[1];
  if (threads_per_cta)
    *threads_per_cta = info[2];
  if (grid)
    *grid = info[3];
  if (regs_per_thread)
    *regs_per_thread = info[4] | (info[5] << 16);
  return AB2_OK;
}

}
```

### aligator_b200/csrc/riccati_group.cuh

```cuda
#pragma once

#include <cmath>
#include <cstddef>
#include <cstdint>
#include <utility>

#if defined(__CUDACC__)
#define AB2_HD __host__ __device__ __forceinline__
#define AB2_D __device__ __forceinline__
#define AB2_UNROLL _Pragma("unroll")
#else
#define AB2_HD inline
#define AB2_D inline
#define AB2_UNROLL
#endif

namespace ab2 {

enum : int { ST_OK = 0, ST_STAGE_FACTOR_FAILED = 1, ST_INIT_FACTOR_FAILED = 2 };

struct SweepParams {
  int N;
  int nct;
  int nc0;
  int batch;
  double mueq;
  int do_bwd, do_fwd;
  const double *stage;
  const double *term;
  const double *G0;
  const double *g0;
  double *ff;
  double *fb;
  double *Vxx;
  double *vx;
  double *ffT;
  double *fbT;
  double *kkt0;
  double *xs;
  double *us;
  double *vs;
  double *vsT;
  double *lbd0;
  double *lbdas;
  int *status;
  int *pivstat;
  int stagger_ns;
  int num_sms;
  int ctas_per_sm;
  int stage_head;
  int dbg;
  int nth;
  const double *theta;
  double *fth;
  double *Vxt;
  double *Vtt;
  double *vt;
  double *kkt0fth;
  double *thGrad;
  double *thHess;
  int legs;
  long long *clk;
  double *cond;
  int peer_world;
  double *peer_dst[8];
  long long peer_off;
};

enum : int { ST_CONDENSED_FACTOR_FAILED = 4 };

AB2_HD int stage_slot(const SweepParams &p, int t) {
  const int s = t + p.stage_head;
  return s >= p.N ? s - p.N : s;
}
AB2_HD int leg_begin(int N, int i, int T) { return (int)((long long)i * (N + 1) / T); }
AB2_HD int cond_offset(int b, int nc0, int nx) { return b == 0 ? 0 : nc0 + (b - 1) * nx; }

template <int NX_, int NU_, int NC_, int G_, bool DB_ = false, bool RB_ = true, bool MMA_ = false> struct Cfg {
  static constexpr int NX = NX_, NU = NU_, NC = NC_, G = G_;
  static constexpr bool DB = DB_;
  static constexpr int NCOL = NX + NU + 1;
  static constexpr int NXU = NX + NU;
  static constexpr int NK = NU + NC;
  static constexpr int NR = NU + NC + NX;
  static constexpr int FCOL = NX + NU;
  static constexpr bool EVEN = (NX % 2) == 0;
  static constexpr bool REGBK = RB_ && (NU_ + NC_ <= 8);
  static constexpr bool FASTBK = RB_ && NC_ == 0 && NU_ <= 8;
  static constexpr int ev(int x) { return (x + 1) & ~1; }
  static constexpr bool MMA = MMA_;
  static constexpr int MTX = (NX + 7) / 8;
  static constexpr int KT = (NX + 3) / 4;
  static constexpr int NJ = NX + 1 + NU;
  static constexpr int NT = (NJ + 7) / 8;
  static constexpr int NT2 = (NX + 1 + 7) / 8;
  static constexpr int KT2 = (NU + NC + 3) / 4;
  static constexpr int fstride(int n) {
    int s = n;
    while (s % 16 != 4 && s % 16 != 12)
      ++s;
    return s;
  }
  static constexpr int VS = MMA ? fstride(4 * KT) : NX;
  static constexpr int VROWS = MMA ? 8 * MTX : NX;
  static constexpr int SW = MMA ? ((8 * NT) % 16 == 8 ? 8 * NT : 8 * NT + 8) : 0;
  static constexpr int WROWS = MMA ? 4 * KT : 0;
  static constexpr int SX = MMA ? fstride(8 * NT2) : 0;
  static constexpr int XROWS = MMA ? 4 * KT2 : 0;
  static constexpr bool VXX_BULK = false;
#ifndef AB2_PARK
#define AB2_PARK 1
#endif
  static constexpr bool PARK = MMA_ && DB_ && (AB2_PARK != 0);
  static constexpr int LUT_INTS = MMA ? 32 * (NT + NT * NT) : 0;
  static constexpr int OFF_A = 0;
  static constexpr int OFF_B = OFF_A + NX * NX;
  static constexpr int OFF_F = OFF_B + NX * NU;
  static constexpr int OFF_Q = OFF_F + NX;
  static constexpr int OFF_S = OFF_Q + NX * NX;
  static constexpr int OFF_R = OFF_S + NX * NU;
  static constexpr int OFF_QV = OFF_R + NU * NU;
  static constexpr int OFF_RV = OFF_QV + NX;
  static constexpr int OFF_C = OFF_RV + NU;
  static constexpr int OFF_D = OFF_C + NC * NX;
  static constexpr int OFF_DV = OFF_D + NC * NU;
  static constexpr int SREC = OFF_DV + NC;
  static constexpr int SREC_PAD = ev(SREC);
  static constexpr int M_DBL = OFF_Q;
  static constexpr int SPLIT = ev(M_DBL);
  static constexpr int RS = ev(NX + 1);
  static constexpr int S_REC = 0;
  static constexpr int RSTRIDE = SREC_PAD + (MMA ? 2 : 0);
  static constexpr int S_VN = S_REC + (DB ? 2 : 1) * RSTRIDE;
  static constexpr int S_VXN = S_VN + ev(VROWS * VS);
  static constexpr int S_KKT = S_VXN + ev(NX);
  static constexpr int S_RHS = S_KKT + ev(NK * NK);
  static constexpr int S_SOL = S_RHS + (MMA ? 0 : NK * RS);
  static constexpr int S_DD = S_SOL + (MMA ? 0 : NK * RS);
  static constexpr int S_SD = S_DD + ev(NK);
  static constexpr int S_X = S_SD + ev(NK);
  static constexpr int S_INT = S_X + 2 * ev(NX);
  static constexpr int S_WSM = S_INT + ev(NK + 1);
  static constexpr int S_XM = S_WSM;
  static constexpr int S_KK = S_XM + ev(XROWS * SX);
  static constexpr int S_MMA_END = S_WSM + (ev(WROWS * SW) > 2 * ev(XROWS * SX) ? ev(WROWS * SW) : 2 * ev(XROWS * SX));
  static constexpr int S_STAGE_END = S_MMA_END;
  static_assert(!MMA || SREC_PAD < 0xffff, "record offsets are packed in 16 bits");
  static_assert(!MMA || (G_ == 32 && NC_ == 0 && (NX_ % 2 == 0)),
                "the tensor-core step needs a full warp, nc = 0, even nx");

  static AB2_HD int col_offset(int jp) {
    if (jp < NX)
      return jp * NX;
    if (jp == NX)
      return OFF_F;
    if (jp <= NX + NU)
      return OFF_B + (jp - NX - 1) * NX;
    return 0;
  }
  static AB2_HD int h0_offset(int ip, int jp) {
    const int ti = ip < NX ? 0 : (ip == NX ? 1 : (ip <= NX + NU ? 2 : 3));
    const int tj = jp < NX ? 0 : (jp == NX ? 1 : (jp <= NX + NU ? 2 : 3));
    const int ci = ip - NX - 1, cj = jp - NX - 1;
    if (ti == 0 && tj == 0)
      return OFF_Q + jp * NX + ip;
    if (ti == 0 && tj == 2)
      return OFF_S + cj * NX + ip;
    if (ti == 2 && tj == 0)
      return OFF_S + ci * NX + jp;
    if (ti == 2 && tj == 2)
      return OFF_R + cj * NU + ci;
    if (ti == 0 && tj == 1)
      return OFF_QV + ip;
    if (ti == 2 && tj == 1)
      return OFF_RV + ci;
    return -1;
  }

  static constexpr bool FB_BULK = ((NR * NX) % 2) == 0;
  static constexpr bool FWD_FUSED = FB_BULK && (NX % 2 == 0) && (NR + NX <= G);
  static constexpr int FWD_ROWS = FWD_FUSED ? NR + NX : NR;
  static constexpr bool FWD_FF = FWD_FUSED && (NR % 2 == 0);
  static constexpr int FWD_SLOT =
      FWD_FUSED ? (NR + NX) * NX + NX + (FWD_FF ? NR : 0) : ev(NR * NX);
  static constexpr int FWD_RING_RAW = (S_STAGE_END - 2 * ev(NX)) / FWD_SLOT;
  static constexpr int FWD_RING_MIN =
      FWD_FUSED ? ((5 * FWD_SLOT + 2 * ev(NX)) * 100 <= S_STAGE_END * 112 ? 5 : 4) : 1;
  static constexpr int FWD_RING = FWD_RING_RAW > 8 ? 8 : (FWD_RING_RAW < FWD_RING_MIN ? FWD_RING_MIN : FWD_RING_RAW);
  static constexpr int NXE = ev(NX);
  static constexpr int FWD_END = FWD_RING * FWD_SLOT + 2 * ev(NX);
  static_assert(NU >= 1, "stage knots need nu >= 1");
  static_assert(NCOL <= G, "lane-per-column mapping needs nx+nu+1 <= G");
  static_assert(NK <= G, "cooperative Bunch-Kaufman needs nu+nc <= G");
  static_assert(G == 8 || G == 16 || G == 32, "group size");

  static AB2_HD int group_doubles(int nc0) {
    const int n0 = NX + nc0;
    const int k0 = n0 * n0 + 6 * n0 + 2;
    int m = S_STAGE_END > k0 ? S_STAGE_END : k0;
    m = m > FWD_END ? m : FWD_END;
    return (m + 1) & ~1;
  }
  static AB2_HD int term_rec(int nct) { return NX * NX + NX + nct * NX + nct; }
};

struct D2 {
  double x, y;
};
AB2_D D2 lds2(const double *p) {
#if defined(__CUDA_ARCH__)
  const double2 v = *reinterpret_cast<const double2 *>(p);
  return D2{v.x, v.y};
#else
  return D2{p[0], p[1]};
#endif
}
AB2_D D2 ldg2(const double *p) {
#if defined(__CUDA_ARCH__)
  const double2 v = *reinterpret_cast<const double2 *>(p);
  return D2{v.x, v.y};
#else
  return D2{p[0], p[1]};
#endif
}
AB2_D void prefetch_l2(const void *p) {
#if defined(__CUDA_ARCH__)
  asm volatile("prefetch.global.L2 [%0];" ::"l"(p));
#else
  (void)p;
#endif
}
template <int N, bool ALIGNED> AB2_D void load_row(const double *p, double (&v)[N]) {
  if constexpr (ALIGNED && (N % 2 == 0)) {
    AB2_UNROLL
    for (int k = 0; k < N; k += 2) {
      const D2 a = ldg2(p + k);
      v[k] = a.x;
      v[k + 1 < N ? k + 1 : k] = a.y;
    }
  } else {
    AB2_UNROLL
    for (int k = 0; k < N; ++k)
      v[k] = p[k];
  }
}
template <int N, bool ALIGNED> AB2_D double dot_bcast(const double *row, const double (&v)[N], double acc) {
  if constexpr (ALIGNED) {
    AB2_UNROLL
    for (int k = 0; k + 1 < N; k += 2) {
      const D2 a = lds2(row + k);
      acc += a.x * v[k];
      acc += a.y * v[k + 1];
    }
    if constexpr (N % 2)
      acc += row[N - 1] * v[N - 1];
  } else {
    AB2_UNROLL
    for (int k = 0; k < N; ++k)
      acc += row[k] * v[k];
  }
  return acc;
}

template <int CHUNK = 1, class Ctx>
AB2_D bool bk_factor_group(Ctx &ctx, double *a, const int lda, const int n,
                            double *dd, double *sd, int *perm, int *kind, int &pv) {
  const double alpha = 0.6403882032022076;
  const int lane = ctx.lane;
#define A_(i, j) a[(i) + (j) * lda]
  if (lane < n)
    perm[lane] = lane;
  ctx.sync();
  bool ok = true;
  int k = 0;
  while (k < n) {
    const double akk = A_(k, k);
    const double abs_akk = fabs(akk);
    int imax = k + 1;
    double colmax = 0.0, cval = 0.0;
    if constexpr (CHUNK > 1) {
      for (int i0 = k + 1; i0 < n; i0 += CHUNK) {
        double v[CHUNK];
        AB2_UNROLL
        for (int u = 0; u < CHUNK; ++u)
          v[u] = A_((i0 + u < n) ? i0 + u : n - 1, k);
        AB2_UNROLL
        for (int u = 0; u < CHUNK; ++u)
          if (i0 + u < n && fabs(v[u]) > colmax) {
            colmax = fabs(v[u]);
            cval = v[u];
            imax = i0 + u;
          }
      }
    } else {
      for (int i = k + 1; i < n; ++i) {
        const double v = A_(i, k);
        if (fabs(v) > colmax) {
          colmax = fabs(v);
          cval = v;
          imax = i;
        }
      }
    }
    if (fmax(abs_akk, colmax) == 0.0) {
      ok = false;
      ctx.sync();
      if (lane >= k && lane < n) {
        dd[lane] = 0.0;
        sd[lane] = 0.0;
        kind[lane] = 0;
        for (int j = k; j < lane; ++j)
          A_(lane, j) = 0.0;
      }
      break;
    }
    int kp = k, kstep = 1;
    double aii = akk;
    if (!(abs_akk >= colmax * alpha)) {
      double rowmax = 0.0;
      for (int j = k; j < imax; ++j)
        rowmax = fmax(rowmax, fabs(A_(imax, j)));
      for (int i = imax + 1; i < n; ++i)
        rowmax = fmax(rowmax, fabs(A_(i, imax)));
      aii = A_(imax, imax);
      if (abs_akk >= (alpha * colmax) * (colmax / rowmax)) {
        kp = k;
      } else if (fabs(aii) >= alpha * rowmax) {
        kp = imax;
      } else {
        kp = imax;
        kstep = 2;
      }
    }
    const int kk = k + kstep - 1;
    pv += (kstep == 2 ? 1 : 0) + (kp != kk ? 0x10000 : 0);
    if (kp != kk) {
      ctx.sync();
      const int i = lane;
      if (i < n) {
        if (i > kp) {
          const double t = A_(i, kk);
          A_(i, kk) = A_(i, kp);
          A_(i, kp) = t;
        } else if (i > kk && i < kp) {
          const double t = A_(i, kk);
          A_(i, kk) = A_(kp, i);
          A_(kp, i) = t;
        } else if (i < k) {
          const double t = A_(kk, i);
          A_(kk, i) = A_(kp, i);
          A_(kp, i) = t;
        } else if (i == kk) {
          const double t = A_(kk, kk);
          A_(kk, kk) = A_(kp, kp);
          A_(kp, kp) = t;
          const int tp = perm[kk];
          perm[kk] = perm[kp];
          perm[kp] = tp;
        }
        if (kstep == 2 && i == k) {
          const double t = A_(k + 1, k);
          A_(k + 1, k) = A_(kp, k);
          A_(kp, k) = t;
        }
      }
    }
    ctx.sync();
    if (kstep == 1) {
      const double d11 = 1.0 / ((kp == k) ? akk : aii);
      double xi = 0.0;
      if (lane > k && lane < n) {
        xi = A_(lane, k);
        A_(lane, k) = xi * d11;
      }
      if (lane == k) {
        dd[k] = d11;
        sd[k] = 0.0;
        kind[k] = 0;
      }
      ctx.sync();
      if (lane > k && lane < n) {
        if constexpr (CHUNK > 1) {
          for (int j0 = k + 1; j0 <= lane; j0 += CHUNK) {
            double l[CHUNK], r[CHUNK];
            AB2_UNROLL
            for (int u = 0; u < CHUNK; ++u) {
              const int j = (j0 + u <= lane) ? j0 + u : lane;
              l[u] = A_(j, k);
              r[u] = A_(lane, j);
            }
            AB2_UNROLL
            for (int u = 0; u < CHUNK; ++u)
              if (j0 + u <= lane)
                A_(lane, j0 + u) = r[u] - l[u] * xi;
          }
        } else {
          for (int j = k + 1; j <= lane; ++j)
            A_(lane, j) -= A_(j, k) * xi;
        }
      }
    } else {
      const double d21_abs = fabs(cval);
      const double d21_inv = 1.0 / d21_abs;
      const double d11 = d21_inv * aii;
      const double d22 = d21_inv * akk;
      const double t = 1.0 / ((d11 * d22) - 1.0);
      const double d = t * d21_inv;
      const double d21 = cval * d21_inv;
      double x0 = 0.0, x1 = 0.0;
      if (lane > k + 1 && lane < n) {
        x0 = A_(lane, k);
        x1 = A_(lane, k + 1);
        const double wk = ((x0 * d11) - (x1 * d21)) * d;
        const double wkp1 = ((x1 * d22) - (x0 * d21)) * d;
        A_(lane, k) = wk;
        A_(lane, k + 1) = wkp1;
      }
      if (lane == k) {
        dd[k] = d11 * d;
        sd[k] = -d21 * d;
        dd[k + 1] = d22 * d;
        sd[k + 1] = 0.0;
        kind[k] = 1;
        kind[k + 1] = 2;
        A_(k + 1, k) = 0.0;
      }
      ctx.sync();
      if (lane > k + 1 && lane < n) {
        if constexpr (CHUNK > 1) {
          for (int j0 = k + 2; j0 <= lane; j0 += CHUNK) {
            double l0[CHUNK], l1[CHUNK], r[CHUNK];
            AB2_UNROLL
            for (int u = 0; u < CHUNK; ++u) {
              const int j = (j0 + u <= lane) ? j0 + u : lane;
              l0[u] = A_(j, k);
              l1[u] = A_(j, k + 1);
              r[u] = A_(lane, j);
            }
            AB2_UNROLL
            for (int u = 0; u < CHUNK; ++u)
              if (j0 + u <= lane)
                A_(lane, j0 + u) = r[u] - (x0 * l0[u] + x1 * l1[u]);
          }
        } else {
          for (int j = k + 2; j <= lane; ++j)
            A_(lane, j) -= x0 * A_(j, k) + x1 * A_(j, k + 1);
        }
      }
    }
    ctx.sync();
    k += kstep;
  }
  ctx.sync();
#undef A_
  return ok;
}

template <int NK, class F>
AB2_D void bk_solve_column(const F &f, const double *rhs, double *sol, const int stride,
                           double (&x)[NK]) {
  AB2_UNROLL
  for (int i = 0; i < NK; ++i)
    x[i] = rhs[f.perm(i) * stride];
  AB2_UNROLL
  for (int c = 0; c < NK; ++c) {
    AB2_UNROLL
    for (int i = c + 1; i < NK; ++i)
      x[i] -= f.L(i, c) * x[c];
  }
  AB2_UNROLL
  for (int k = 0; k < NK; ++k) {
    const int kd = f.kind(k);
    const int k1 = (k + 1 < NK) ? k + 1 : k;
    if (kd == 0) {
      x[k] *= f.dd(k);
    } else if (kd == 1 && k + 1 < NK) {
      const double xk = x[k], xk1 = x[k1];
      const double sdk = f.sd(k);
      x[k] = xk * f.dd(k) + xk1 * sdk;
      x[k1] = xk1 * f.dd(k1) + xk * sdk;
    }
  }
  AB2_UNROLL
  for (int c = NK - 1; c >= 0; --c) {
    AB2_UNROLL
    for (int i = c + 1; i < NK; ++i)
      x[c] -= f.L(i, c) * x[i];
  }
  AB2_UNROLL
  for (int i = 0; i < NK; ++i)
    sol[f.perm(i) * stride] = x[i];
  AB2_UNROLL
  for (int i = 0; i < NK; ++i)
    x[i] = sol[i * stride];
}

template <int NK> struct SmemFactor {
  const double *a, *d, *s;
  const int *pm, *kd;
  AB2_D double L(int i, int c) const { return a[i + c * NK]; }
  AB2_D double dd(int k) const { return d[k]; }
  AB2_D double sd(int k) const { return s[k]; }
  AB2_D int kind(int k) const { return kd[k]; }
  AB2_D int perm(int i) const { return pm[i]; }
};

AB2_D double rcp_fast(double x) {
#if defined(__CUDA_ARCH__)
  double r;
  asm("rcp.approx.ftz.f64 %0, %1;" : "=d"(r) : "d"(x));
  double e = fma(-x, r, 1.0);
  r = fma(r, e, r);
  e = fma(-x, r, 1.0);
  r = fma(r, e, r);
  return r;
#else
  return 1.0 / x;
#endif
}

template <int N> struct FastFactor {
  double a[N][N];
  double d[N];
  AB2_D double L(int i, int c) const { return a[i][c]; }
  AB2_D bool factor() {
    const double alpha = 0.6403882032022076;
    bool good = true;
    AB2_UNROLL
    for (int k = 0; k < N; ++k) {
      const double akk = a[k][k];
      const double abs_akk = fabs(akk);
      good = good && (abs_akk > 0.0);
      AB2_UNROLL
      for (int i = k + 1; i < N; ++i)
        good = good && (fabs(a[i][k]) * alpha <= abs_akk);
      const double d11 = rcp_fast(akk);
      d[k] = d11;
      AB2_UNROLL
      for (int j = k + 1; j < N; ++j) {
        const double d11xj = a[j][k] * d11;
        AB2_UNROLL
        for (int i = j; i < N; ++i)
          a[i][j] -= d11xj * a[i][k];
      }
      AB2_UNROLL
      for (int i = k + 1; i < N; ++i)
        a[i][k] *= d11;
    }
    return good;
  }
  AB2_D void solve(const double *rhs, const int stride, double (&x)[N]) const {
    AB2_UNROLL
    for (int i = 0; i < N; ++i)
      x[i] = rhs[i * stride];
    AB2_UNROLL
    for (int c = 0; c < N; ++c) {
      AB2_UNROLL
      for (int i = c + 1; i < N; ++i)
        x[i] -= a[i][c] * x[c];
    }
    AB2_UNROLL
    for (int k = 0; k < N; ++k)
      x[k] *= d[k];
    AB2_UNROLL
    for (int c = N - 1; c >= 0; --c) {
      AB2_UNROLL
      for (int i = c + 1; i < N; ++i)
        x[c] -= a[i][c] * x[i];
    }
  }
};

template <int N> struct RegFactor {
  double a[N][N];
  double d[N], s[N];
  int pm[N], kd[N];
  AB2_D double L(int i, int c) const { return a[i][c]; }
  AB2_D double dd(int k) const { return d[k]; }
  AB2_D double sd(int k) const { return s[k]; }
  AB2_D int kind(int k) const { return kd[k]; }
  AB2_D int perm(int i) const { return pm[i]; }

  AB2_D void swap_sym(const int KK, const int C, const int K0, const bool two) {
    AB2_UNROLL
    for (int i = 0; i < N; ++i) {
      if (i > C) {
        const double t = a[i][KK];
        a[i][KK] = a[i][C];
        a[i][C] = t;
      } else if (i > KK && i < C) {
        const double t = a[i][KK];
        a[i][KK] = a[C][i];
        a[C][i] = t;
      } else if (i < K0) {
        const double t = a[KK][i];
        a[KK][i] = a[C][i];
        a[C][i] = t;
      }
    }
    {
      const double t = a[KK][KK];
      a[KK][KK] = a[C][C];
      a[C][C] = t;
      const int tp = pm[KK];
      pm[KK] = pm[C];
      pm[C] = tp;
    }
    if (two) {
      const double t = a[KK][K0];
      a[KK][K0] = a[C][K0];
      a[C][K0] = t;
    }
  }

  template <int K> AB2_D void step(bool &ok, bool &skip, bool &dead, int &pv) {
    constexpr int k = K;
    const double alpha = 0.6403882032022076;
    if (skip || dead) {
      skip = false;
      return;
    }
    const double akk = a[k][k];
    const double abs_akk = fabs(akk);
    int imax = k + 1;
    double colmax = 0.0;
    AB2_UNROLL
    for (int i = k + 1; i < N; ++i) {
      const double v = fabs(a[i][k]);
      if (v > colmax) {
        colmax = v;
        imax = i;
      }
    }
    if (fmax(abs_akk, colmax) == 0.0) {
      ok = false;
      dead = true;
      AB2_UNROLL
      for (int i = k; i < N; ++i) {
        AB2_UNROLL
        for (int j = k; j < i; ++j)
          a[i][j] = 0.0;
      }
      return;
    }
    int kp = k, kstep = 1;
    if (!(abs_akk >= colmax * alpha)) {
      double rowmax = 0.0, aii = akk;
      AB2_UNROLL
      for (int c = k + 1; c < N; ++c)
        if (imax == c) {
          AB2_UNROLL
          for (int j = k; j < c; ++j)
            rowmax = fmax(rowmax, fabs(a[c][j]));
          AB2_UNROLL
          for (int i = c + 1; i < N; ++i)
            rowmax = fmax(rowmax, fabs(a[i][c]));
          aii = a[c][c];
        }
      if (abs_akk >= (alpha * colmax) * (colmax / rowmax)) {
        kp = k;
      } else if (fabs(aii) >= alpha * rowmax) {
        kp = imax;
      } else {
        kp = imax;
        kstep = 2;
      }
    }
    constexpr int k1 = (k + 1 < N) ? k + 1 : k;
    pv += (kstep == 2 ? 1 : 0) + (kp != k + kstep - 1 ? 0x10000 : 0);
    if (kstep == 1) {
      if (kp != k) {
        AB2_UNROLL
        for (int c = k + 1; c < N; ++c)
          if (kp == c)
            swap_sym(k, c, k, false);
      }
      const double d11 = 1.0 / a[k][k];
      d[k] = d11;
      AB2_UNROLL
      for (int j = k + 1; j < N; ++j) {
        const double d11xj = a[j][k] * d11;
        AB2_UNROLL
        for (int i = j; i < N; ++i)
          a[i][j] -= d11xj * a[i][k];
      }
      AB2_UNROLL
      for (int i = k + 1; i < N; ++i)
        a[i][k] *= d11;
    } else if (k + 1 < N) {
      if (kp != k1) {
        AB2_UNROLL
        for (int c = k + 2; c < N; ++c)
          if (kp == c)
            swap_sym(k1, c, k, true);
      }
      const double d21v = a[k1][k];
      const double d21_abs = fabs(d21v);
      const double d21_inv = 1.0 / d21_abs;
      const double d11 = d21_inv * a[k1][k1];
      const double d22 = d21_inv * a[k][k];
      const double t = 1.0 / ((d11 * d22) - 1.0);
      const double dm = t * d21_inv;
      const double d21 = d21v * d21_inv;
      d[k] = d11 * dm;
      s[k] = -d21 * dm;
      d[k1] = d22 * dm;
      kd[k] = 1;
      kd[k1] = 2;
      AB2_UNROLL
      for (int j = k + 2; j < N; ++j) {
        const double wk = ((a[j][k] * d11) - (a[j][k1] * d21)) * dm;
        const double wkp1 = ((a[j][k1] * d22) - (a[j][k] * d21)) * dm;
        AB2_UNROLL
        for (int i = j; i < N; ++i)
          a[i][j] -= a[i][k] * wk + a[i][k1] * wkp1;
        a[j][k] = wk;
        a[j][k1] = wkp1;
      }
      a[k1][k] = 0.0;
      skip = true;
    }
  }
  template <int... Ks>
  AB2_D void steps(bool &ok, bool &skip, bool &dead, int &pv, std::integer_sequence<int, Ks...>) {
    (step<Ks>(ok, skip, dead, pv), ...);
  }

  AB2_D bool factor(int &pv) {
    bool ok = true, skip = false, dead = false;
    AB2_UNROLL
    for (int i = 0; i < N; ++i) {
      pm[i] = i;
      kd[i] = 0;
      d[i] = 0.0;
      s[i] = 0.0;
    }
    steps(ok, skip, dead, pv, std::make_integer_sequence<int, N>{});
    return ok;
  }
};

template <class Ctx>
AB2_D void bk_solve_vec_group(Ctx &ctx, const double *a, const int lda, const int n,
                               const double *dd, const double *sd, const int *perm,
                               const int *kind, const double *b, double *x, double *out) {
  const int lane = ctx.lane;
  if (lane < n)
    x[lane] = b[perm[lane]];
  for (int c = 0; c < n; ++c) {
    ctx.sync();
    const double xc = x[c];
    if (lane > c && lane < n)
      x[lane] -= a[lane + c * lda] * xc;
  }
  ctx.sync();
  if (lane < n) {
    const int kd = kind[lane];
    if (kd == 0) {
      x[lane] *= dd[lane];
    } else if (kd == 1) {
      const double xk = x[lane], xk1 = x[lane + 1];
      const double s = sd[lane];
      x[lane] = xk * dd[lane] + xk1 * s;
      x[lane + 1] = xk1 * dd[lane + 1] + xk * s;
    }
  }
  for (int i = n - 1; i >= 1; --i) {
    ctx.sync();
    const double xi = x[i];
    if (lane < i)
      x[lane] -= a[i + lane * lda] * xi;
  }
  ctx.sync();
  if (lane < n)
    out[perm[lane]] = x[lane];
  ctx.sync();
}


template <class Ctx>
AB2_D bool kkt0_fast(Ctx &ctx, double *a, const int lda, const int n, const double rhs, double &x_out) {
  const double alpha = 0.6403882032022076;
  const int lane = ctx.lane;
  const bool in = lane < n;
  double myd = 0.0;
  for (int k = 0; k < n; ++k) {
    ctx.sync();
    const double akk = a[k + k * lda];
    const bool below = lane > k && in;
    const double my = below ? a[lane + k * lda] : 0.0;
    const bool ok = (fabs(my) * alpha <= fabs(akk)) && (fabs(akk) > 0.0);
    if (!ctx.all(ok))
      return false;
    const double d = 1.0 / akk;
    if (lane == k)
      myd = d;
    int j = k + 1;
    for (; j + 4 <= n; j += 4) {
      const double m0 = ctx.shfl(my, j), m1 = ctx.shfl(my, j + 1), m2 = ctx.shfl(my, j + 2),
                   m3 = ctx.shfl(my, j + 3);
      double *pj = a + (in ? lane : 0) + j * lda;
      const double r0 = pj[0], r1 = pj[lda], r2 = pj[2 * lda], r3 = pj[3 * lda];
      if (in && lane >= j)
        pj[0] = r0 - (m0 * d) * my;
      if (in && lane >= j + 1)
        pj[lda] = r1 - (m1 * d) * my;
      if (in && lane >= j + 2)
        pj[2 * lda] = r2 - (m2 * d) * my;
      if (in && lane >= j + 3)
        pj[3 * lda] = r3 - (m3 * d) * my;
    }
    for (; j < n; ++j) {
      const double mj = ctx.shfl(my, j);
      if (in && lane >= j)
        a[lane + j * lda] -= (mj * d) * my;
    }
    if (below)
      a[lane + k * lda] = my * d;
  }
  ctx.sync();
  double x = rhs;
  for (int c = 0; c + 1 < n; ++c) {
    const double xc = ctx.shfl(x, c);
    if (lane > c && in)
      x -= a[lane + c * lda] * xc;
  }
  x *= myd;
  for (int i = n - 1; i >= 1; --i) {
    const double xi = ctx.shfl(x, i);
    if (lane < i)
      x -= a[i + lane * lda] * xi;
  }
  x_out = x;
  ctx.sync();
  return true;
}

AB2_D void stg2(double *p, double x, double y) {
#if defined(__CUDA_ARCH__)
  *reinterpret_cast<double2 *>(p) = make_double2(x, y);
#else
  p[0] = x;
  p[1] = y;
#endif
}

AB2_D void sts2(double *p, double x, double y) {
#if defined(__CUDA_ARCH__)
  *reinterpret_cast<double2 *>(p) = make_double2(x, y);
#else
  p[0] = x;
  p[1] = y;
#endif
}

template <class C> AB2_HD void fill_mma_lut(int *lut, const int lane, const int first = 0, const int step = 1) {
  constexpr int NT = C::NT;
  const int g = lane >> 2, q = lane & 3;
  for (int r = first; r < NT + NT * NT; r += step) {
    if (r < NT) {
      lut[r * 32 + lane] = C::col_offset(8 * r + g);
    } else {
      const int mt = (r - NT) / NT, nt = (r - NT) % NT;
      const int o0 = C::h0_offset(8 * mt + g, 8 * nt + 2 * q);
      const int o1 = C::h0_offset(8 * mt + g, 8 * nt + 2 * q + 1);
      const unsigned u0 = o0 < 0 ? (unsigned)C::SREC_PAD : (unsigned)o0;
      const unsigned u1 = o1 < 0 ? (unsigned)C::SREC_PAD : (unsigned)o1;
      lut[r * 32 + lane] = (int)(u0 | (u1 << 16));
    }
  }
}

template <class C, class Ctx>
AB2_D void stage_loop_mma(Ctx &ctx, const SweepParams &p, double *__restrict__ sm, int &st, int &pv,
                          const int inst) {
  constexpr int NX = C::NX, NU = C::NU, NK = C::NK, NR = C::NR;
  constexpr int MTX = C::MTX, KT = C::KT, NT = C::NT, NT2 = C::NT2, KT2 = C::KT2;
  constexpr int VS = C::VS, SW = C::SW, SX = C::SX;
  const int lane = ctx.lane;
  const int g = lane >> 2, q = lane & 3;
  const int N = p.N;
#define AB2_STAGE_B (p.stage + (size_t)inst * N * C::SREC_PAD)
#define AB2_FF_B (p.ff + (size_t)inst * N * NR)
#define AB2_FB_B (p.fb + (size_t)inst * N * NR * NX)
#define AB2_VXX_B (p.Vxx + (size_t)inst * (N + 1) * NX * NX)
#define AB2_VX_B (p.vx + (size_t)inst * (N + 1) * NX)
  double *Vn = sm + C::S_VN;
  double *vxn = sm + C::S_VXN;
  double *kkt = sm + C::S_KKT;
  double *dd = sm + C::S_DD;
  double *sd = sm + C::S_SD;
  int *perm = reinterpret_cast<int *>(sm + C::S_INT);
  int *kind = perm + NK;
  double *Wsm = sm + C::S_WSM;
  double *X = sm + C::S_XM;
  double *KKs = sm + C::S_KK;

  const int *lut = ctx.cta_ints();
  if (lane < (C::DB ? 4 : 2))
    sm[C::S_REC + (lane >> 1) * C::RSTRIDE + C::SREC_PAD + (lane & 1)] = 0.0;
  for (int i = lane; i < C::S_MMA_END - C::S_WSM; i += 32)
    Wsm[i] = 0.0;
  ctx.sync();

  const bool colS = lane <= NX;
  int cur = 0;
  for (int t = N - 1; t >= 0; --t) {
    ctx.wait_copy(C::DB ? cur : 0);
    double *rec = sm + C::S_REC + (C::DB ? cur : 0) * C::RSTRIDE;
    if (C::DB) {
      if (t > 0)
        ctx.issue_copy(cur ^ 1, sm + C::S_REC + (cur ^ 1) * C::RSTRIDE,
                       AB2_STAGE_B + (size_t)stage_slot(p, t - 1) * C::SREC_PAD, C::SREC_PAD);
      cur ^= 1;
    }
    const int pfd = (p.dbg & 8) ? 2 : 4;
    if (t >= pfd && (p.dbg & 4)) {
      const char *nxt = reinterpret_cast<const char *>(AB2_STAGE_B + (size_t)stage_slot(p, t - pfd) * C::SREC_PAD);
      for (int o = lane * 128; o < C::SREC_PAD * 8; o += C::G * 128)
        prefetch_l2(nxt + o);
    }

    double Mf[NT][KT];
    AB2_UNROLL
    for (int tt = 0; tt < NT; ++tt) {
      AB2_UNROLL
      for (int kt = 0; kt < KT; ++kt)
        Mf[tt][kt] = rec[lut[tt * 32 + lane] + 4 * kt + q];
    }
    {
      double W[MTX][NT][2];
      AB2_UNROLL
      for (int mt = 0; mt < MTX; ++mt) {
        AB2_UNROLL
        for (int nt = 0; nt < NT; ++nt) {
          W[mt][nt][0] = 0.0;
          W[mt][nt][1] = 0.0;
        }
      }
      AB2_UNROLL
      for (int kt = 0; kt < KT; ++kt) {
        AB2_UNROLL
        for (int mt = 0; mt < MTX; ++mt) {
          const double va = Vn[(8 * mt + g) * VS + 4 * kt + q];
          AB2_UNROLL
          for (int nt = 0; nt < NT; ++nt)
            ctx.mma(W[mt][nt], va, Mf[nt][kt]);
        }
      }
      AB2_UNROLL
      for (int mt = 0; mt < MTX; ++mt) {
        const int i = 8 * mt + g;
        if (i < NX) {
          AB2_UNROLL
          for (int nt = 0; nt < NT; ++nt) {
            AB2_UNROLL
            for (int e = 0; e < 2; ++e)
              if (8 * nt + 2 * q + e == NX)
                W[mt][nt][e] += vxn[i];
            sts2(Wsm + i * SW + 8 * nt + 2 * q, W[mt][nt][0], W[mt][nt][1]);
          }
        }
      }
    }
    ctx.sync();
    if (!C::DB)
      ctx.wait_copy(1);
    double H[NT][NT][2];
    AB2_UNROLL
    for (int mt = 0; mt < NT; ++mt) {
      AB2_UNROLL
      for (int nt = 0; nt < NT; ++nt) {
        AB2_UNROLL
        for (int e = 0; e < 2; ++e) {
          const unsigned o = ((unsigned)lut[(NT + mt * NT + nt) * 32 + lane] >> (16 * e)) & 0xffffu;
          H[mt][nt][e] = rec[o];
        }
      }
    }
    AB2_UNROLL
    for (int kt = 0; kt < KT; ++kt) {
      AB2_UNROLL
      for (int nt = 0; nt < NT; ++nt) {
        const double wb = (4 * kt + q < NX) ? Wsm[(4 * kt + q < NX ? 4 * kt + q : 0) * SW + 8 * nt + g] : 0.0;
        AB2_UNROLL
        for (int mt = 0; mt < NT; ++mt)
          ctx.mma(H[mt][nt], Mf[mt][kt], wb);
      }
    }
    ctx.sync();
    if (!C::DB && t > 0)
      ctx.issue_copy(1, rec + C::SPLIT, AB2_STAGE_B + (size_t)stage_slot(p, t - 1) * C::SREC_PAD + C::SPLIT,
                     C::SREC_PAD - C::SPLIT);
    AB2_UNROLL
    for (int mt = 0; mt < NT; ++mt) {
      const int c = 8 * mt + g - NX - 1;
      if (c >= 0 && c < NU) {
        AB2_UNROLL
        for (int nt = 0; nt < NT; ++nt) {
          AB2_UNROLL
          for (int e = 0; e < 2; ++e) {
            const int jp = 8 * nt + 2 * q + e;
            if (jp <= NX)
              X[c * SX + jp] = H[mt][nt][e];
            else if (jp - NX - 1 < NU)
              kkt[c + (jp - NX - 1) * NK] = H[mt][nt][e];
          }
        }
      }
    }
    if (C::PARK) {
      AB2_UNROLL
      for (int mt = 0; mt < MTX; ++mt) {
        const int i = 8 * mt + g;
        if (i < NX) {
          AB2_UNROLL
          for (int nt = 0; nt < NT2; ++nt) {
            const int j0 = 8 * nt + 2 * q;
            if (j0 + 1 < NX)
              sts2(Vn + i * VS + j0, H[mt][nt][0], H[mt][nt][1]);
            else if (j0 == NX)
              vxn[i] = H[mt][nt][0];
          }
        }
      }
    }
    ctx.sync();
    double *fbt = AB2_FB_B + (size_t)t * NR * NX;
    double *fft = AB2_FF_B + (size_t)t * NR;
    {
      double kz[NK];
      FastFactor<NK> F;
      AB2_UNROLL
      for (int c = 0; c < NK; ++c) {
        AB2_UNROLL
        for (int i = c; i < NK; ++i)
          F.a[i][c] = kkt[i + c * NK];
      }
      if (F.factor()) {
        if (colS)
          F.solve(X + lane, SX, kz);
      } else {
        if (!bk_factor_group(ctx, kkt, NK, NK, dd, sd, perm, kind, pv))
          st |= ST_STAGE_FACTOR_FAILED;
        if (colS) {
          const SmemFactor<NK> G{kkt, dd, sd, perm, kind};
          bk_solve_column<NK>(G, X + lane, KKs + lane, SX, kz);
        }
      }
      if (colS) {
        double *const odst = (lane < NX) ? fbt + lane : fft;
        const int ostride = (lane < NX) ? NX : 1;
        AB2_UNROLL
        for (int c = 0; c < NK; ++c) {
          const double v = -kz[c];
          KKs[c * SX + lane] = v;
          odst[c * ostride] = v;
        }
      }
    }
    ctx.sync();
    double KKf[KT2][NT2];
    AB2_UNROLL
    for (int k2 = 0; k2 < KT2; ++k2) {
      AB2_UNROLL
      for (int nt = 0; nt < NT2; ++nt)
        KKf[k2][nt] = KKs[(4 * k2 + q) * SX + 8 * nt + g];
    }
    {
      double EA[MTX][NT2][2], VV[MTX][NT2][2], Bf[MTX][KT2], Xf[MTX][KT2];
      AB2_UNROLL
      for (int mt = 0; mt < MTX; ++mt) {
        const int i = 8 * mt + g;
        const int ic2 = i < NX ? i : 0;
        AB2_UNROLL
        for (int nt = 0; nt < NT2; ++nt) {
          const int j0 = 8 * nt + 2 * q;
          if (!C::PARK) {
            VV[mt][nt][0] = H[mt][nt][0];
            VV[mt][nt][1] = H[mt][nt][1];
          } else if (j0 + 1 < NX) {
            const D2 v = lds2(Vn + ic2 * VS + j0);
            VV[mt][nt][0] = v.x;
            VV[mt][nt][1] = v.y;
          } else {
            VV[mt][nt][0] = vxn[ic2];
            VV[mt][nt][1] = 0.0;
          }
        }
      }
      AB2_UNROLL
      for (int mt = 0; mt < MTX; ++mt) {
        const int i = 8 * mt + g;
        const int ic = i < NX ? i : 0;
        AB2_UNROLL
        for (int nt = 0; nt < NT2; ++nt) {
          AB2_UNROLL
          for (int e = 0; e < 2; ++e) {
            const int jj = 8 * nt + 2 * q + e;
            const int off = (jj < NX) ? jj * NX : ((jj == NX) ? C::OFF_F : 0);
            EA[mt][nt][e] = rec[off + ic];
          }
        }
        AB2_UNROLL
        for (int k2 = 0; k2 < KT2; ++k2) {
          const int c = 4 * k2 + q;
          const double bv = rec[C::OFF_B + (c < NU ? c : 0) * NX + ic];
          Bf[mt][k2] = (c < NU) ? bv : 0.0;
          const double xv = X[c * SX + i];
          Xf[mt][k2] = (c < NK) ? xv : 0.0;
        }
      }
      AB2_UNROLL
      for (int k2 = 0; k2 < KT2; ++k2) {
        AB2_UNROLL
        for (int mt = 0; mt < MTX; ++mt) {
          AB2_UNROLL
          for (int nt = 0; nt < NT2; ++nt) {
            ctx.mma(EA[mt][nt], Bf[mt][k2], KKf[k2][nt]);
            ctx.mma(VV[mt][nt], Xf[mt][k2], KKf[k2][nt]);
          }
        }
      }
      if (!C::DB && t > 0) {
        ctx.sync();
        ctx.issue_copy(0, rec, AB2_STAGE_B + (size_t)stage_slot(p, t - 1) * C::SREC_PAD, C::SPLIT);
      }
      if (C::VXX_BULK && t > 0)
        ctx.bulk_store_wait_read();
      AB2_UNROLL
      for (int mt = 0; mt < MTX; ++mt) {
        const int i = 8 * mt + g;
        if (i < NX) {
          AB2_UNROLL
          for (int nt = 0; nt < NT2; ++nt) {
            AB2_UNROLL
            for (int e = 0; e < 2; ++e) {
              const int jj = 8 * nt + 2 * q + e;
              if (jj < NX)
                fbt[(NK + i) * NX + jj] = EA[mt][nt][e];
              else if (jj == NX)
                fft[NK + i] = EA[mt][nt][e];
            }
          }
        }
      }
      if (C::VXX_BULK)
        ctx.sync();
      AB2_UNROLL
      for (int mt = 0; mt < MTX; ++mt) {
        const int i = 8 * mt + g;
        if (i < NX) {
          AB2_UNROLL
          for (int nt = 0; nt < NT2; ++nt) {
            AB2_UNROLL
            for (int e = 0; e < 2; ++e) {
              const int jj = 8 * nt + 2 * q + e;
              const double v = VV[mt][nt][e];
              if (jj < NX) {
                if (t == 0)
                  AB2_VXX_B[i + jj * NX] = v;
                if (i >= jj) {
                  Vn[i * VS + jj] = v;
                  Vn[jj * VS + i] = v;
                }
              } else if (jj == NX) {
                AB2_VX_B[(size_t)t * NX + i] = v;
                vxn[i] = v;
              }
            }
          }
        }
      }
    }
    if (C::VXX_BULK && t > 0)
      ctx.async_fence();
    ctx.sync();
    if (t > 0) {
      double *Vt = AB2_VXX_B + (size_t)t * NX * NX;
      if (C::VXX_BULK) {
        ctx.bulk_store(Vt, Vn, NX * NX);
      } else if (lane < NX) {
        if (C::EVEN && (VS % 2 == 0)) {
          AB2_UNROLL
          for (int i = 0; i < NX; i += 2) {
            const D2 v = lds2(Vn + lane * VS + i);
            stg2(Vt + i + lane * NX, v.x, v.y);
          }
        } else {
          AB2_UNROLL
          for (int i = 0; i < NX; ++i)
            Vt[i + lane * NX] = Vn[lane * VS + i];
        }
      }
    }
  }
  if (C::VXX_BULK) {
    ctx.bulk_store_wait_read();
    ctx.sync();
  }
}
#undef AB2_STAGE_B
#undef AB2_FF_B
#undef AB2_FB_B
#undef AB2_VXX_B
#undef AB2_VX_B

template <class C, class Ctx>
AB2_D void riccati_group_sweep(Ctx &ctx, const SweepParams &p, const int inst,
                                double *__restrict__ sm) {
  constexpr int NX = C::NX, NU = C::NU, NC = C::NC, NK = C::NK, NR = C::NR;
  constexpr int NXU = C::NXU, NCOL = C::NCOL, FCOL = C::FCOL;
  const int lane = ctx.lane;
  const int N = p.N;
  const int nct = p.nct, nc0 = p.nc0;
  const double mueq = p.mueq;

  double *rec = sm + C::S_REC;
  double *Vn = sm + C::S_VN;
  double *vxn = sm + C::S_VXN;
  double *kkt = sm + C::S_KKT;
  double *rhs0 = sm + C::S_RHS;
  double *sol = sm + C::S_SOL;
  double *dd = sm + C::S_DD;
  double *sd = sm + C::S_SD;
  double *xv = sm + C::S_X;
  int *perm = reinterpret_cast<int *>(sm + C::S_INT);
  int *kind = perm + NK;

  const double *stage_b = p.stage + (size_t)inst * N * C::SREC_PAD;
  double *ff_b = p.ff + (size_t)inst * N * NR;
  double *fb_b = p.fb + (size_t)inst * N * NR * NX;
  double *Vxx_b = p.Vxx + (size_t)inst * (N + 1) * NX * NX;
  double *vx_b = p.vx + (size_t)inst * (N + 1) * NX;
  int st = ST_OK;
  int pv = 0;

  const bool colA = lane < NX;
  const bool colB = lane >= NX && lane < NXU;
  const bool colF = lane == FCOL;
  const bool active = lane < NCOL;
  const int jj = colF ? NX : lane;

  if (p.do_bwd) {
    if (N > 0) {
      const double *src = stage_b + (size_t)stage_slot(p, N - 1) * C::SREC_PAD;
      if (C::DB) {
        ctx.issue_copy(0, rec, src, C::SREC_PAD);
      } else {
        ctx.issue_copy(0, rec, src, C::SPLIT);
        ctx.issue_copy(1, rec + C::SPLIT, src + C::SPLIT, C::SREC_PAD - C::SPLIT);
      }
    }
    if constexpr (C::MMA) {
      for (int i = lane; i < C::VROWS * C::VS; i += C::G)
        Vn[i] = 0.0;
      ctx.sync();
    }
    {
      const double *tr = p.term + (size_t)inst * C::term_rec(nct);
      const double *Qt = tr;
      const double *qt = tr + NX * NX;
      const double *Ct = qt + NX;
      const double *dt = Ct + (size_t)nct * NX;
      double *VN = Vxx_b + (size_t)N * NX * NX;
      if (colA || colF) {
        double acc[NX];
        AB2_UNROLL
        for (int i = 0; i < NX; ++i)
          acc[i] = 0.0;
#if defined(__CUDACC__)
#pragma unroll 1
#endif
        for (int m = 0; m < nct; ++m) {
          const double zm = (colF ? dt[m] : Ct[m + (size_t)lane * nct]) / mueq;
          if (colF)
            p.ffT[(size_t)inst * nct + m] = zm;
          else
            p.fbT[(size_t)inst * nct * NX + (size_t)m * NX + lane] = zm;
          AB2_UNROLL
          for (int i = 0; i < NX; ++i)
            acc[i] += Ct[m + (size_t)i * nct] * zm;
        }
        AB2_UNROLL
        for (int i = 0; i < NX; ++i) {
          const double s = (colF ? qt[i] : Qt[i + lane * NX]) + acc[i];
          if (colF) {
            vx_b[(size_t)N * NX + i] = s;
            vxn[i] = s;
          } else {
            VN[i + lane * NX] = s;
            if (i >= lane) {
              Vn[i * C::VS + lane] = s;
              Vn[lane * C::VS + i] = s;
            }
          }
        }
      }
      ctx.sync();
      if (colA && N > 0) {
        AB2_UNROLL
        for (int i = 0; i < NX; ++i)
          VN[i + lane * NX] = Vn[lane * C::VS + i];
      }
    }

    if constexpr (C::MMA) {
      stage_loop_mma<C>(ctx, p, sm, st, pv, inst);
    } else {
    constexpr int RS = C::RS;
    constexpr bool EV = C::EVEN;
    int cur = 0;
    for (int t = N - 1; t >= 0; --t) {
      if (C::DB) {
        ctx.wait_copy(cur);
        rec = sm + C::S_REC + cur * C::RSTRIDE;
        if (t > 0)
          ctx.issue_copy(cur ^ 1, sm + C::S_REC + (cur ^ 1) * C::RSTRIDE,
                         stage_b + (size_t)stage_slot(p, t - 1) * C::SREC_PAD, C::SREC_PAD);
        cur ^= 1;
      } else {
        ctx.wait_copy(0);
        ctx.wait_copy(1);
      }
      double mcol[NX];
      if (EV) {
        AB2_UNROLL
        for (int k = 0; k < NX; k += 2) {
          const D2 v = lds2(rec + (active ? lane : 0) * NX + k);
          mcol[k] = v.x;
          mcol[k + 1 < NX ? k + 1 : k] = v.y;
        }
      } else {
        AB2_UNROLL
        for (int k = 0; k < NX; ++k)
          mcol[k] = rec[(active ? lane : 0) * NX + k];
      }
      double w[NX];
      AB2_UNROLL
      for (int i = 0; i < NX; ++i)
        w[i] = dot_bcast<NX, EV>(Vn + i * C::VS, mcol, 0.0);
      if (colF) {
        AB2_UNROLL
        for (int i = 0; i < NX; ++i)
          w[i] += vxn[i];
      }
      int base1, base2, stride2;
      if (colA) {
        base1 = C::OFF_Q + lane * NX;
        base2 = C::OFF_S + lane;
        stride2 = NX;
      } else if (colB) {
        base1 = C::OFF_S + (lane - NX) * NX;
        base2 = C::OFF_R + (lane - NX) * NU;
        stride2 = 1;
      } else {
        base1 = C::OFF_QV;
        base2 = C::OFF_RV;
        stride2 = 1;
      }
      double *const cdst = colB ? kkt + (lane - NX) * NK : rhs0 + jj;
      const int cstride = colB ? 1 : RS;
      const double csign = colB ? 1.0 : -1.0;
      AB2_UNROLL
      for (int r = 0; r < NU; ++r) {
        const double hr = dot_bcast<NX, EV>(rec + (NX + r) * NX, w, rec[base2 + r * stride2]);
        if (active)
          cdst[r * cstride] = csign * hr;
      }
      if (colB) {
        AB2_UNROLL
        for (int m = 0; m < NC; ++m)
          kkt[NU + m + (lane - NX) * NK] = rec[C::OFF_D + (lane - NX) * NC + m];
      }
      if (lane < NC) {
        AB2_UNROLL
        for (int m = 0; m < NC; ++m)
          kkt[NU + m + (NU + lane) * NK] = (m == lane) ? -mueq : 0.0;
      }
      if (colA || colF) {
        AB2_UNROLL
        for (int m = 0; m < NC; ++m)
          rhs0[(NU + m) * RS + jj] = colF ? -rec[C::OFF_DV + m] : -rec[C::OFF_C + lane * NC + m];
      }
      constexpr bool STASH = C::DB;
      double h[NX];
      AB2_UNROLL
      for (int i = 0; i < NX; ++i) {
        h[i] = dot_bcast<NX, EV>(rec + i * NX, w, rec[base1 + i]);
        if (STASH && (colA || colF))
          rec[base1 + i] = h[i];
      }
      ctx.sync();
      if (!C::DB && t > 0)
        ctx.issue_copy(1, rec + C::SPLIT, stage_b + (size_t)stage_slot(p, t - 1) * C::SREC_PAD + C::SPLIT,
                       C::SREC_PAD - C::SPLIT);
      double kz[NK];
      double *fbt = fb_b + (size_t)t * NR * NX;
      double *fft = ff_b + (size_t)t * NR;
      if constexpr (C::FASTBK) {
        FastFactor<NK> F;
        AB2_UNROLL
        for (int c = 0; c < NK; ++c) {
          AB2_UNROLL
          for (int i = c; i < NK; ++i)
            F.a[i][c] = kkt[i + c * NK];
        }
        if (F.factor()) {
          if (colA || colF)
            F.solve(rhs0 + jj, RS, kz);
        } else {
          if (!bk_factor_group(ctx, kkt, NK, NK, dd, sd, perm, kind, pv))
            st |= ST_STAGE_FACTOR_FAILED;
          if (colA || colF) {
            const SmemFactor<NK> G{kkt, dd, sd, perm, kind};
            bk_solve_column<NK>(G, rhs0 + jj, sol + jj, RS, kz);
          }
        }
      } else if constexpr (C::REGBK) {
        RegFactor<NK> F;
        AB2_UNROLL
        for (int c = 0; c < NK; ++c) {
          AB2_UNROLL
          for (int i = c; i < NK; ++i)
            F.a[i][c] = kkt[i + c * NK];
        }
        if (!F.factor(pv))
          st |= ST_STAGE_FACTOR_FAILED;
        if (colA || colF)
          bk_solve_column<NK>(F, rhs0 + jj, sol + jj, RS, kz);
      } else {
        if (!bk_factor_group(ctx, kkt, NK, NK, dd, sd, perm, kind, pv))
          st |= ST_STAGE_FACTOR_FAILED;
        if (colA || colF) {
          const SmemFactor<NK> F{kkt, dd, sd, perm, kind};
          bk_solve_column<NK>(F, rhs0 + jj, sol + jj, RS, kz);
        }
      }
      if (colA || colF) {
        double ahat[NX];
        AB2_UNROLL
        for (int i = 0; i < NX; ++i)
          ahat[i] = STASH ? rec[lane * NX + i] : mcol[i];
        AB2_UNROLL
        for (int c = 0; c < NU; ++c) {
          const double kc = kz[c];
          if (EV) {
            AB2_UNROLL
            for (int i = 0; i < NX; i += 2) {
              const D2 b = lds2(rec + C::OFF_B + c * NX + i);
              ahat[i] += b.x * kc;
              ahat[i + 1 < NX ? i + 1 : i] += b.y * kc;
            }
          } else {
            AB2_UNROLL
            for (int i = 0; i < NX; ++i)
              ahat[i] += rec[C::OFF_B + c * NX + i] * kc;
          }
        }
        double *const odst = colA ? fbt + lane : fft;
        const int ostride = colA ? NX : 1;
        AB2_UNROLL
        for (int r = 0; r < NK; ++r)
          odst[r * ostride] = kz[r];
        AB2_UNROLL
        for (int i = 0; i < NX; ++i)
          odst[(NK + i) * ostride] = ahat[i];
      }
      if (!C::DB) {
        ctx.sync();
        if (t > 0)
          ctx.issue_copy(0, rec, stage_b + (size_t)stage_slot(p, t - 1) * C::SREC_PAD, C::SPLIT);
      }
      if (colA || colF) {
        if (STASH) {
          AB2_UNROLL
          for (int i = 0; i < NX; ++i)
            h[i] = rec[base1 + i];
        }
        AB2_UNROLL
        for (int r = 0; r < NU; ++r) {
          const double kr = kz[r];
          if (EV) {
            AB2_UNROLL
            for (int i = 0; i < NX; i += 2) {
              const D2 sv = lds2(rhs0 + r * RS + i);
              h[i] -= sv.x * kr;
              h[i + 1 < NX ? i + 1 : i] -= sv.y * kr;
            }
          } else {
            AB2_UNROLL
            for (int i = 0; i < NX; ++i)
              h[i] -= rhs0[r * RS + i] * kr;
          }
        }
        if (NC > 0) {
          double s2[NX];
          AB2_UNROLL
          for (int i = 0; i < NX; ++i)
            s2[i] = 0.0;
          AB2_UNROLL
          for (int m = 0; m < NC; ++m) {
            const double zr = kz[NU + m < NK ? NU + m : 0];
            AB2_UNROLL
            for (int i = 0; i < NX; ++i)
              s2[i] -= rhs0[(NU + m) * RS + i] * zr;
          }
          AB2_UNROLL
          for (int i = 0; i < NX; ++i)
            h[i] += s2[i];
        }
        if (colA) {
          if (t == 0) {
            double *Vt = Vxx_b;
            AB2_UNROLL
            for (int i = 0; i < NX; ++i)
              Vt[i + lane * NX] = h[i];
          }
          AB2_UNROLL
          for (int i = 0; i < NX; ++i)
            if (i >= lane) {
              Vn[i * C::VS + lane] = h[i];
              Vn[lane * C::VS + i] = h[i];
            }
        } else {
          AB2_UNROLL
          for (int i = 0; i < NX; ++i) {
            vx_b[(size_t)t * NX + i] = h[i];
            vxn[i] = h[i];
          }
        }
      }
      if (STASH)
        ctx.proxy_fence_smem();
      ctx.sync();
      if (t > 0 && colA) {
        double *Vt = Vxx_b + (size_t)t * NX * NX;
        AB2_UNROLL
        for (int i = 0; i < NX; ++i)
          Vt[i + lane * NX] = Vn[lane * C::VS + i];
      }
    }

    }

    if (p.peer_world > 0 && N > 0) {
      ctx.sync();
      constexpr int PER = NU * (NX + 1);
      const double *fb0 = p.fb + (size_t)inst * N * NR * NX, *ff0 = p.ff + (size_t)inst * N * NR;
      for (int e = lane; e < PER; e += C::G) {
        const int r = e / (NX + 1), c = e - r * (NX + 1);
        const double v = (c < NX) ? fb0[r * NX + c] : ff0[r];
        for (int w = 0; w < p.peer_world; ++w)
          p.peer_dst[w][p.peer_off + (long long)inst * PER + e] = v;
      }
    }

    {
      const int n0 = NX + nc0;
      double *K0 = sm;
      double *b0 = K0 + n0 * n0;
      double *x0w = b0 + n0;
      double *dd0 = x0w + n0;
      double *sd0 = dd0 + n0;
      double *o0 = sd0 + n0;
      int *perm0 = reinterpret_cast<int *>(o0 + n0);
      int *kind0 = perm0 + n0;
      double vcol[NX];
      double vx0 = 0.0;
      AB2_UNROLL
      for (int i = 0; i < NX; ++i)
        vcol[i] = colA ? Vn[i * C::VS + lane] : 0.0;
      if (lane < NX)
        vx0 = vxn[lane];
      ctx.sync();
      const double *G0 = p.G0 + (size_t)inst * nc0 * NX;
      const double *g0 = p.g0 + (size_t)inst * nc0;
      bool fast_done = false;
      if (!(p.dbg & 1)) {
        const int ld0 = n0 | 1;
        if (colA) {
          AB2_UNROLL
          for (int i = 0; i < NX; ++i)
            if (i >= lane)
              K0[i + lane * ld0] = vcol[i];
          for (int m = 0; m < nc0; ++m)
            K0[NX + m + lane * ld0] = G0[m + (size_t)lane * nc0];
        }
        for (int m = lane; m < nc0; m += C::G)
          for (int m2 = m; m2 < nc0; ++m2)
            K0[NX + m2 + (NX + m) * ld0] = 0.0;
        const double b = (lane < NX) ? -vx0 : ((lane < n0) ? -g0[lane - NX] : 0.0);
        double x = 0.0;
        fast_done = kkt0_fast(ctx, K0, ld0, n0, b, x);
        if (fast_done && lane < n0)
          p.kkt0[(size_t)inst * n0 + lane] = x;
        if (fast_done)
          pv |= 0x8000;
        else
          ctx.sync();
      }
      if (!fast_done) {
        if (colA) {
          AB2_UNROLL
          for (int i = 0; i < NX; ++i)
            if (i >= lane)
              K0[i + lane * n0] = vcol[i];
          for (int m = 0; m < nc0; ++m)
            K0[NX + m + lane * n0] = G0[m + (size_t)lane * nc0];
          b0[lane] = -vx0;
        }
        for (int m = lane; m < nc0; m += C::G) {
          for (int m2 = m; m2 < nc0; ++m2)
            K0[NX + m2 + (NX + m) * n0] = 0.0;
          b0[NX + m] = -g0[m];
        }
        ctx.sync();
        if (!bk_factor_group<4>(ctx, K0, n0, n0, dd0, sd0, perm0, kind0, pv))
          st |= ST_INIT_FACTOR_FAILED;
        bk_solve_vec_group(ctx, K0, n0, n0, dd0, sd0, perm0, kind0, b0, x0w, o0);
        for (int i = lane; i < n0; i += C::G)
          p.kkt0[(size_t)inst * n0 + i] = o0[i];
        ctx.sync();
      }
    }
    if (lane == 0) {
      p.status[inst] = st;
      if (p.pivstat)
        p.pivstat[inst] = pv;
    }
  }

  if (p.do_fwd) {
    const int n0 = NX + nc0;
    const double *k0 = p.kkt0 + (size_t)inst * n0;
    double *xs_b = p.xs + (size_t)inst * (N + 1) * NX;
    double *us_b = p.us + (size_t)inst * N * NU;
    double *vs_b = p.vs + (size_t)inst * N * NC;
    double *lb_b = p.lbdas + (size_t)inst * N * NX;
    constexpr int RING = C::FWD_RING;
    constexpr int FS = C::FWD_SLOT;
    constexpr bool FUSED = C::FWD_FUSED;
    constexpr int ROWS = C::FWD_ROWS;
    constexpr int RPL = (ROWS + C::G - 1) / C::G;
    const int NIT = FUSED ? N + 1 : N;
    constexpr bool EVF = C::EVEN;
    double *ring = sm;
    double *xc = sm + RING * FS;
    double *xnx = xc + C::NXE;
    (void)xv;
    if (!(p.dbg & 2))
      ctx.proxy_fence();
    ctx.sync();
    auto fill_slot = [&](int d, int t) {
      if (FUSED) {
        ctx.copy_expect(d, (t < N ? NR * NX + (C::FWD_FF ? NR : 0) : 0) + NX * NX + NX);
        if (t < N) {
          ctx.copy_add(d, ring + d * FS, fb_b + (size_t)t * NR * NX, NR * NX);
          if (C::FWD_FF)
            ctx.copy_add(d, ring + d * FS + (NR + NX) * NX + NX, ff_b + (size_t)t * NR, NR);
        }
        ctx.copy_add(d, ring + d * FS + NR * NX, Vxx_b + (size_t)t * NX * NX, NX * NX);
        ctx.copy_add(d, ring + d * FS + (NR + NX) * NX, vx_b + (size_t)t * NX, NX);
      } else if (C::FB_BULK) {
        ctx.issue_copy(d, ring + d * FS, fb_b + (size_t)t * NR * NX, NR * NX);
      } else {
        for (int i2 = lane; i2 < NR * NX; i2 += C::G)
          ring[d * FS + i2] = fb_b[(size_t)t * NR * NX + i2];
      }
    };
    AB2_UNROLL
    for (int d = 0; d < RING; ++d)
      if (d < NIT)
        fill_slot(d, d);
    if (lane < NX) {
      const double v = k0[lane];
      xc[lane] = v;
      xs_b[lane] = v;
    }
    for (int m = lane; m < nc0; m += C::G)
      p.lbd0[(size_t)inst * nc0 + m] = k0[NX + m];
    double gff[RING][RPL];
    AB2_UNROLL
    for (int d = 0; d < RING; ++d) {
      AB2_UNROLL
      for (int q = 0; q < RPL; ++q) {
        const int r = lane + q * C::G;
        gff[d][q] = (!C::FWD_FF && r < NR && d < N) ? ff_b[(size_t)d * NR + r] : 0.0;
      }
    }
    ctx.sync();
    for (int t0 = 0; t0 < NIT; t0 += RING) {
      AB2_UNROLL
      for (int d = 0; d < RING; ++d) {
        const int t = t0 + d;
        if (t < NIT) {
          if (C::FB_BULK)
            ctx.wait_copy(d);
          const double *slot = ring + d * FS;
          AB2_UNROLL
          for (int q = 0; q < RPL; ++q) {
            const int r = lane + q * C::G;
            if (FUSED ? ((r < NR && t < N) || (r >= NR && r < ROWS && t >= 1)) : (r < NR)) {
              double s0 = gff[d][q], s1 = 0.0;
              if (FUSED && (C::FWD_FF || r >= NR))
                s0 = slot[(NR + NX) * NX + (r >= NR ? r - NR : NX + r)];
              if (EVF) {
                constexpr bool ROT = ((NX / 2) % 4) == 2;
                const int rot2 = ROT ? ((r >> 1) & 2) : 0;
                AB2_UNROLL
                for (int c = 0; c < NX; c += 2) {
                  const int cc = (ROT && c + 2 == NX) ? (rot2 ? 0 : c) : c + rot2;
                  const D2 gg = lds2(slot + r * NX + cc);
                  const D2 xx = lds2(xc + cc);
                  s0 += gg.x * xx.x;
                  s1 += gg.y * xx.y;
                }
              } else {
                AB2_UNROLL
                for (int c = 0; c < NX; ++c)
                  s0 += slot[r * NX + c] * xc[c];
              }
              const double s = s0 + s1;
              if (r < NU)
                us_b[(size_t)t * NU + r] = s;
              else if (r < NK)
                vs_b[(size_t)t * NC + (r - NU)] = s;
              else if (!FUSED || r < NR) {
                xnx[r - NK] = s;
                xs_b[(size_t)(t + 1) * NX + (r - NK)] = s;
              } else {
                lb_b[(size_t)(t - 1) * NX + (r - NR)] = s;
              }
              if (!C::FWD_FF && (!FUSED || r < NR))
                gff[d][q] = (t + RING < N) ? ff_b[(size_t)(t + RING) * NR + r] : 0.0;
            }
          }
          if (t < N) {
            double *tmp = xc;
            xc = xnx;
            xnx = tmp;
          }
          ctx.sync();
          if (t + RING < NIT)
            fill_slot(d, t + RING);
        }
      }
    }
    if (!FUSED) {
      constexpr int KPI = (C::G / NX) > 0 ? (C::G / NX) : 1;
      constexpr int U = 2;
      const int sub = lane / NX, i = lane % NX;
      if (sub < KPI) {
        for (int t = sub; t < N; t += KPI * U) {
          double vrow[U][NX], xr[U][NX], v0[U];
          AB2_UNROLL
          for (int u = 0; u < U; ++u) {
            const int tt = t + u * KPI;
            if (tt < N) {
              load_row<NX, EVF>(Vxx_b + ((size_t)(tt + 1) * NX + i) * NX, vrow[u]);
              load_row<NX, EVF>(xs_b + (size_t)(tt + 1) * NX, xr[u]);
              v0[u] = vx_b[(size_t)(tt + 1) * NX + i];
            }
          }
          AB2_UNROLL
          for (int u = 0; u < U; ++u) {
            const int tt = t + u * KPI;
            if (tt < N) {
              double s0 = v0[u], s1 = 0.0;
              AB2_UNROLL
              for (int c = 0; c + 1 < NX; c += 2) {
                s0 += vrow[u][c] * xr[u][c];
                s1 += vrow[u][c + 1] * xr[u][c + 1];
              }
              if (NX % 2)
                s0 += vrow[u][NX - 1] * xr[u][NX - 1];
              lb_b[(size_t)tt * NX + i] = s0 + s1;
            }
          }
        }
      }
      ctx.sync();
    }
    for (int m = lane; m < nct; m += C::G) {
      double s = p.ffT[(size_t)inst * nct + m];
      for (int c = 0; c < NX; ++c)
        s += p.fbT[(size_t)inst * nct * NX + (size_t)m * NX + c] * xc[c];
      p.vsT[(size_t)inst * nct + m] = s;
    }
  }
}

}
```

### aligator_b200/csrc/riccati_launch.cuh

```cuda
#pragma once
#include <cuda_runtime.h>

#include "riccati_group.cuh"

namespace ab2 {

__device__ __forceinline__ uint32_t smem_u32(const void *p) {
  return static_cast<uint32_t>(__cvta_generic_to_shared(p));
}

constexpr int NBAR = 8;

template <int G, bool TMA> struct DevCtx {
  int lane;
  unsigned mask;
  uint32_t bar0;
  uint32_t phase;
  int *cta_lut;
  __device__ __forceinline__ int *cta_ints() const { return cta_lut; }

  __device__ __forceinline__ void sync() { __syncwarp(mask); }
  __device__ __forceinline__ double shfl(double v, int src) { return __shfl_sync(mask, v, src, G); }
  __device__ __forceinline__ bool all(bool p) { return __all_sync(mask, p); }

  __device__ __forceinline__ void mma(double (&d)[2], double a, double b) {
    asm volatile("mma.sync.aligned.m8n8k4.row.col.f64.f64.f64.f64 {%0,%1}, {%2}, {%3}, {%0,%1};"
                 : "+d"(d[0]), "+d"(d[1])
                 : "d"(a), "d"(b));
  }

  __device__ __forceinline__ void init(uint64_t *bars) {
    bar0 = smem_u32(bars);
    phase = 0;
    if (TMA) {
      if (lane == 0) {
        for (int b = 0; b < NBAR; ++b)
          asm volatile("mbarrier.init.shared::cta.b64 [%0], 1;" ::"r"(bar0 + 8 * b));
        asm volatile("fence.mbarrier_init.release.cluster;" ::: "memory");
      }
    }
    __syncwarp(mask);
  }

  __device__ __forceinline__ void issue_copy(int part, double *dst, const double *src, int nd) {
    if (TMA) {
      if (lane == 0) {
        const uint32_t bar = bar0 + 8 * part;
        const uint32_t bytes = (uint32_t)nd * 8u;
        asm volatile("mbarrier.arrive.expect_tx.shared::cta.b64 _, [%0], %1;" ::"r"(bar), "r"(bytes)
                     : "memory");
        asm volatile(
            "cp.async.bulk.shared::cluster.global.mbarrier::complete_tx::bytes [%0], [%1], %2, [%3];" ::"r"(
                smem_u32(dst)),
            "l"(src), "r"(bytes), "r"(bar)
            : "memory");
      }
    } else {
      const uint32_t d = smem_u32(dst);
      for (int c = lane; c < nd / 2; c += G)
        asm volatile("cp.async.cg.shared.global [%0], [%1], 16;" ::"r"(d + 16u * c), "l"(src + 2 * c)
                     : "memory");
      asm volatile("cp.async.commit_group;" ::: "memory");
    }
  }

  __device__ __forceinline__ void copy_expect(int part, int nd_total) {
    if (TMA) {
      if (lane == 0)
        asm volatile("mbarrier.arrive.expect_tx.shared::cta.b64 _, [%0], %1;" ::"r"(bar0 + 8 * part),
                     "r"((uint32_t)nd_total * 8u)
                     : "memory");
    }
  }
  __device__ __forceinline__ void copy_add(int part, double *dst, const double *src, int nd) {
    if (TMA) {
      if (lane == 0)
        asm volatile(
            "cp.async.bulk.shared::cluster.global.mbarrier::complete_tx::bytes [%0], [%1], %2, [%3];" ::"r"(
                smem_u32(dst)),
            "l"(src), "r"((uint32_t)nd * 8u), "r"(bar0 + 8 * part)
            : "memory");
    } else {
      const uint32_t d = smem_u32(dst);
      for (int c = lane; c < nd / 2; c += G)
        asm volatile("cp.async.cg.shared.global [%0], [%1], 16;" ::"r"(d + 16u * c), "l"(src + 2 * c)
                     : "memory");
      asm volatile("cp.async.commit_group;" ::: "memory");
    }
  }

  __device__ __forceinline__ void async_fence() { asm volatile("fence.proxy.async.shared::cta;" ::: "memory"); }
  __device__ __forceinline__ void proxy_fence() { asm volatile("fence.proxy.async;" ::: "memory"); }
  __device__ __forceinline__ void proxy_fence_smem() { asm volatile("fence.proxy.async.shared::cta;" ::: "memory"); }
  __device__ __forceinline__ void bulk_store(double *gdst, const double *ssrc, int nd) {
    if (lane == 0) {
      asm volatile("cp.async.bulk.global.shared::cta.bulk_group [%0], [%1], %2;" ::"l"(gdst),
                   "r"(smem_u32(ssrc)), "r"((uint32_t)nd * 8u)
                   : "memory");
      asm volatile("cp.async.bulk.commit_group;" ::: "memory");
    }
  }
  __device__ __forceinline__ void bulk_store_wait_read() {
    if (lane == 0)
      asm volatile("cp.async.bulk.wait_group.read 0;" ::: "memory");
  }

  __device__ __forceinline__ void wait_copy(int part) {
    if (TMA) {
      const uint32_t bar = bar0 + 8 * part;
      uint32_t done = 0;
      while (!done) {
        asm volatile("{\n\t.reg .pred p;\n\t"
                     "mbarrier.try_wait.parity.shared::cta.b64 p, [%1], %2;\n\t"
                     "selp.u32 %0, 1, 0, p;\n\t}"
                     : "=r"(done)
                     : "r"(bar), "r"((phase >> part) & 1u)
                     : "memory");
      }
      phase ^= (1u << part);
    } else {
      asm volatile("cp.async.wait_all;" ::: "memory");
    }
    __syncwarp(mask);
  }
};

template <class C, int WARPS, int MAXREG, bool TMA>
__global__ void __launch_bounds__(WARPS * 32) __maxnreg__(MAXREG)
    riccati_sweep_kernel(const SweepParams p, const int group_doubles) {
  extern __shared__ __align__(16) double smem[];
  constexpr int IPW = 32 / C::G;
  const int warp = threadIdx.x >> 5;
  const int lane32 = threadIdx.x & 31;
  const int gsub = lane32 / C::G;
  const int group_in_cta = warp * IPW + gsub;
  const int inst = blockIdx.x * (WARPS * IPW) + group_in_cta;
  if constexpr (C::MMA) {
    fill_mma_lut<C>(reinterpret_cast<int *>(smem + (size_t)(WARPS * IPW) * group_doubles + (size_t)(WARPS * IPW) * NBAR),
                    lane32, warp, WARPS);
    __syncthreads();
  }
  if (inst >= p.batch)
    return;
  double *sm = smem + (size_t)group_in_cta * group_doubles;
  uint64_t *bars =
      reinterpret_cast<uint64_t *>(smem + (size_t)(WARPS * IPW) * group_doubles) + NBAR * group_in_cta;
  DevCtx<C::G, TMA> ctx;
  ctx.cta_lut = reinterpret_cast<int *>(smem + (size_t)(WARPS * IPW) * group_doubles + (size_t)(WARPS * IPW) * NBAR);
  ctx.lane = lane32 % C::G;
  ctx.mask = (C::G == 32) ? 0xffffffffu : (((1u << C::G) - 1u) << (gsub * C::G));
  ctx.init(bars);
  if (p.stagger_ns > 0) {
    const int slot = (blockIdx.x / p.num_sms) * WARPS + warp;
    __nanosleep((unsigned)(slot * p.stagger_ns));
  }
  riccati_group_sweep<C>(ctx, p, inst, sm);
}

struct KernelEntry {
  int nx, nu, nc, G;
  int srec_pad;
  void (*group_doubles)(int nc0, int gd[4]);
  cudaError_t (*launch)(const SweepParams &, int variant, const int gd[4], cudaStream_t, int *info);
};

template <class C, int WARPS, int MAXREG, bool TMA>
inline cudaError_t launch_one(const SweepParams &p, int gd, cudaStream_t st, int *info) {
  constexpr int IPW = 32 / C::G;
  const int groups = WARPS * IPW;
  size_t smem = (size_t)groups * gd * sizeof(double) + (size_t)groups * 8 * NBAR + (size_t)C::LUT_INTS * 4;
  auto kern = riccati_sweep_kernel<C, WARPS, MAXREG, TMA>;
  cudaError_t e = cudaFuncSetAttribute(kern, cudaFuncAttributeMaxDynamicSharedMemorySize, (int)smem);
  if (e != cudaSuccess)
    return e;
  e = cudaFuncSetAttribute(kern, cudaFuncAttributePreferredSharedMemoryCarveout,
                           (int)cudaSharedmemCarveoutMaxShared);
  if (e != cudaSuccess)
    return e;
  const int grid = (p.batch + groups - 1) / groups;
  {
    static thread_local size_t cached_smem = 0;
    static thread_local int cached_cmax = 0;
    if (cached_smem != smem) {
      e = cudaOccupancyMaxActiveBlocksPerMultiprocessor(&cached_cmax, kern, WARPS * 32, smem);
      if (e != cudaSuccess)
        return e;
      cached_smem = smem;
    }
    const int cmax = cached_cmax;
    int want = p.ctas_per_sm;
    if (want == 0 && cmax > 1) {
      const int sms = p.num_sms > 0 ? p.num_sms : 132;
      auto rounds = [&](int c) { return (grid + sms * c - 1) / (sms * c); };
      want = cmax;
      while ((want - 1) * WARPS >= 12 && rounds(want - 1) == rounds(cmax))
        --want;
    }
    if (want > 0 && want < cmax) {
      const size_t pad = (((size_t)227 * 1024 / want) - 1024) & ~(size_t)15;
      if (pad > smem) {
        smem = pad;
        e = cudaFuncSetAttribute(kern, cudaFuncAttributeMaxDynamicSharedMemorySize, (int)smem);
        if (e != cudaSuccess)
          return e;
      }
    }
  }
  if (info) {
    cudaFuncAttributes fa;
    cudaFuncGetAttributes(&fa, kern);
    info[0] = C::G;
    info[1] = (int)smem;
    info[2] = WARPS * 32;
    info[3] = grid;
    info[4] = fa.numRegs;
    int nb = 0;
    cudaOccupancyMaxActiveBlocksPerMultiprocessor(&nb, kern, WARPS * 32, smem);
    info[5] = nb;
    return cudaSuccess;
  }
  kern<<<grid, WARPS * 32, smem, st>>>(p, gd);
  return cudaGetLastError();
}

template <int NX, int NU, int NC, int G>
inline cudaError_t launch_cfg(const SweepParams &p, int variant, const int gd[4], cudaStream_t st, int *info) {
  using CS = Cfg<NX, NU, NC, G, false>;
  using CD = Cfg<NX, NU, NC, G, true>;
  if (variant < 0) {
    variant = 6;
    if constexpr (G == 32 && NC == 0 && NX % 2 == 0) {
      using CM = Cfg<NX, NU, NC, G, true, true, true>;
      const int sms = p.num_sms > 0 ? p.num_sms : 132;
      const int grid = (p.batch + 1) / 2;
      auto ctas = [&](int gdw, int cap) {
        const size_t smem = (size_t)2 * gdw * sizeof(double) + 2 * 8 * NBAR + (size_t)CM::LUT_INTS * 4;
        const int c = (int)((size_t)227 * 1024 / (smem + 1024));
        return c < cap ? (c < 1 ? 1 : c) : cap;
      };
      auto rounds = [&](int c) { return (grid + sms * c - 1) / (sms * c); };
      const int c7 = ctas(gd[2], 8), c8 = ctas(gd[2], 6), c10 = ctas(gd[3], 8);
      const int r7 = rounds(c7), r8 = rounds(c8), r10 = rounds(c10);
      if (c7 == 8 && r7 <= r8 && r7 <= r10)
        variant = 7;
      else if (r8 <= r7 && r8 <= r10)
        variant = 8;
      else if (r10 < r7)
        variant = 10;
      else
        variant = 7;
    }
  }
  if (variant == 1)
    return launch_one<CS, 4, 72, true>(p, gd[0], st, info);
  if (variant == 2)
    return launch_one<CD, 2, 144, false>(p, gd[1], st, info);
  if (variant == 3)
    return launch_one<CS, 4, 72, false>(p, gd[0], st, info);
  if (variant == 4)
    return launch_one<Cfg<NX, NU, NC, G, false, false>, 4, 72, true>(p, gd[0], st, info);
  if (variant == 5)
    return launch_one<Cfg<NX, NU, NC, G, true, false>, 2, 144, true>(p, gd[1], st, info);
  if (variant == 6)
    return launch_one<CD, 2, 128, true>(p, gd[1], st, info);
  if constexpr (G == 32 && NC == 0 && NX % 2 == 0) {
    using CM = Cfg<NX, NU, NC, G, true, true, true>;
    if (variant == 7)
      return launch_one<CM, 2, 128, true>(p, gd[2], st, info);
    if (variant == 8)
      return launch_one<CM, 2, 168, true>(p, gd[2], st, info);
    if (variant == 10)
      return launch_one<Cfg<NX, NU, NC, G, false, true, true>, 2, 128, true>(p, gd[3], st, info);
  }
  return launch_one<CD, 2, 144, true>(p, gd[1], st, info);
}
template <int NX, int NU, int NC, int G> inline void group_doubles_cfg(int nc0, int gd[4]) {
  gd[0] = Cfg<NX, NU, NC, G, false>::group_doubles(nc0);
  gd[1] = Cfg<NX, NU, NC, G, true>::group_doubles(nc0);
  gd[2] = gd[1];
  gd[3] = gd[0];
  if constexpr (G == 32 && NC == 0 && NX % 2 == 0) {
    gd[2] = Cfg<NX, NU, NC, G, true, true, true>::group_doubles(nc0);
    gd[3] = Cfg<NX, NU, NC, G, false, true, true>::group_doubles(nc0);
  }
}

}
```

Before: 238.9 million.

## Store Vxx in packed lower-triangular layout in warp Riccati kernels

Switches the per-knot value Hessian Vxx to a packed symmetric lower-triangle layout for the warp-group kernels. Knot 0 keeps a separate full matrix, and a new expand kernel rebuilds dense matrices when a caller asks for them. The goal is to roughly halve global-memory writes and reads of Vxx in the backward sweep and the forward rollout. The cost is irregular index arithmetic, unpaired packed loads in the forward pass, a larger shared-memory LUT, and an extra expansion pass on readout.

```diff
diff --git a/aligator_b200/build.py b/aligator_b200/build.py
--- a/aligator_b200/build.py
+++ b/aligator_b200/build.py
@@ -39,7 +39,8 @@
 
 def build(verbose=False, force=False, ptxas_v=False):
     os.makedirs(OBJ, exist_ok=True)
-    hdrs = [os.path.join(CSRC, f) for f in ("riccati_group.cuh", "riccati_launch.cuh", "riccati_configs.h")]
+    hdrs = [os.path.join(CSRC, f) for f in ("riccati_group.cuh", "riccati_launch.cuh", "riccati_configs.h",
+                                            "vxx_layout.h")]
     hdrs.append(os.path.join(PKG, "..", "include", "aligator_b200", "gar.h"))
     hdrs_block = hdrs + [os.path.join(CSRC, f) for f in ("riccati_block.cuh", "riccati_block_launch.h",
                                                           "lq_assemble.h", "kkt_error.h", "linesearch.h",
diff --git a/aligator_b200/csrc/gar_cuda.cu b/aligator_b200/csrc/gar_cuda.cu
--- a/aligator_b200/csrc/gar_cuda.cu
+++ b/aligator_b200/csrc/gar_cuda.cu
@@ -123,17 +123,39 @@
     }
   }
 }
-__global__ void fddp_vx_kernel(const double *__restrict__ Vxx, const double *__restrict__ vx, const double *__restrict__ fs,
-                               double *__restrict__ Vx_out, int batch, int N, int nx) {
+__global__ void fddp_vx_kernel(const double *__restrict__ Vxx, const double *__restrict__ Vxx0, const double *__restrict__ vx,
+                               const double *__restrict__ fs, double *__restrict__ Vx_out, int batch, int N, int nx) {
   const long total = (long)batch * (N + 1) * nx;
+  const int P = vxx_packed_doubles(nx);
   for (long i = blockIdx.x * (long)blockDim.x + threadIdx.x; i < total; i += (long)gridDim.x * blockDim.x) {
     const long kn = i / nx;
     const int r = (int)(i % nx);
-    const double *V = Vxx + kn * nx * nx, *f = fs + kn * nx;
+    const double *f = fs + kn * nx;
     double acc = 0.0;
-    for (int c = 0; c < nx; ++c)
-      acc += (r >= c ? V[r + (size_t)c * nx] : V[c + (size_t)r * nx]) * f[c];
+    if (Vxx0 && !vxx_slot_is_full((int)(kn % (N + 1)))) {
+      const double *V = Vxx + kn * P;
+      for (int c = 0; c < nx; ++c)
+        acc += V[vxx_packed_index(nx, r, c)] * f[c];
+    } else {
+      const double *V = Vxx0 ? Vxx0 + kn / (N + 1) * nx * nx : Vxx + kn * nx * nx;
+      for (int c = 0; c < nx; ++c)
+        acc += (r >= c ? V[r + (size_t)c * nx] : V[c + (size_t)r * nx]) * f[c];
+    }
     Vx_out[i] = vx[i] + acc;
+  }
+}
+__global__ void vxx_expand_kernel(const double *__restrict__ pk, const double *__restrict__ full0, double *__restrict__ dst,
+                                  int N, int nx, int head, int b0, int nb, int t0, int nt) {
+  const long nn = (long)nx * nx, total = (long)nb * nt * nn;
+  const int P = vxx_packed_doubles(nx);
+  for (long i = blockIdx.x * (long)blockDim.x + threadIdx.x; i < total; i += (long)gridDim.x * blockDim.x) {
+    const long kn = i / nn;
+    const int e = (int)(i - kn * nn);
+    const long b = b0 + kn / nt;
+    const int t = t0 + (int)(kn % nt);
+    const int slot = t < N ? (t + head) % N : t;
+    dst[i] = vxx_slot_is_full(slot) ? full0[b * nn + e]
+                                    : pk[(b * (N + 1) + slot) * P + vxx_packed_index(nx, e % nx, e / nx)];
   }
 }
 __global__ void fddp_quuks_kernel(const double *__restrict__ Ju, const double *__restrict__ Lu, const double *__restrict__ Vx,
@@ -215,6 +237,7 @@
   bool have_problem = false, have_backward = false, have_forward = false;
   long launches = 0;
   int variant = -1;
+  bool vxx_packed = false;
   int group_doubles[4] = {0, 0, 0, 0};
   static constexpr int kPipeStreams = 4;
   cudaStream_t pipe_stream[kPipeStreams] = {};
@@ -343,8 +366,12 @@
   setup(AB2_OUT_KKT0FTH, (size_t)(nx + d.nc0) * nth, 1);
   setup(AB2_OUT_THGRAD, nth, 1);
   setup(AB2_OUT_THHESS, (size_t)nth * nth, 1);
+  const size_t vxx_packed_total = (size_t)B * (N + 1) * ab2::vxx_packed_doubles(nx) + (size_t)B * nx * nx;
   for (int w = 0; w < AB2_OUT_COUNT; ++w) {
-    const size_t bytes = (s->out_doubles[w] > 0 ? s->out_doubles[w] + 2 : 2) * sizeof(double);
+    size_t n = s->out_doubles[w];
+    if (w == AB2_OUT_VXX && s->k && vxx_packed_total > n)
+      n = vxx_packed_total;
+    const size_t bytes = (n > 0 ? n + 2 : 2) * sizeof(double);
     cudaError_t e = cudaMalloc(&s->out[w], bytes);
     if (e == cudaSuccess)
       e = cudaMemset(s->out[w], 0, bytes);
@@ -392,6 +419,8 @@
   p.ff = s->out[AB2_OUT_FF];
   p.fb = s->out[AB2_OUT_FB];
   p.Vxx = s->out[AB2_OUT_VXX];
+  if (s->k)
+    p.Vxx0 = p.Vxx + (size_t)B * (N + 1) * ab2::vxx_packed_doubles(nx);
   p.vx = s->out[AB2_OUT_VX];
   p.ffT = s->out[AB2_OUT_FFT];
   p.fbT = s->out[AB2_OUT_FBT];
@@ -529,6 +558,8 @@
   return AB2_OK;
 }
 
+static bool warp_kernel(const ab2_gar_solver *s) { return s->k && s->variant != 9; }
+
 static ab2::SweepParams slice_params(const ab2_gar_solver *s, int b0, int nb) {
   ab2::SweepParams q = s->p;
   const size_t b = (size_t)b0;
@@ -542,8 +573,13 @@
     q.g0 += b * s->d.nc0;
   q.ff += b * s->out_knots[AB2_OUT_FF] * s->out_rec[AB2_OUT_FF];
   q.fb += b * s->out_knots[AB2_OUT_FB] * s->out_rec[AB2_OUT_FB];
-  q.Vxx += b * s->out_knots[AB2_OUT_VXX] * s->out_rec[AB2_OUT_VXX];
-  q.vx += b * s->out_knots[AB2_OUT_VX] * s->out_rec[AB2_OUT_VX];
+  if (warp_kernel(s)) {
+    q.Vxx += b * (N + 1) * ab2::vxx_packed_doubles(nx);
+    q.Vxx0 += b * nx * nx;
+  } else {
+    q.Vxx += b * s->out_knots[AB2_OUT_VXX] * s->out_rec[AB2_OUT_VXX];
+  }
+  q.vx +=b * s->out_knots[AB2_OUT_VX] * s->out_rec[AB2_OUT_VX];
   q.ffT += b * s->out_rec[AB2_OUT_FFT];
   q.fbT += b * s->out_rec[AB2_OUT_FBT];
   q.kkt0 += b * s->out_rec[AB2_OUT_KKT0];
@@ -592,10 +628,11 @@
   }
   q.do_bwd = bwd;
   q.do_fwd = fwd;
+  const bool warp = bwd ? warp_kernel(s) : s->vxx_packed;
   if (s->dense)
     CUDA_TRY(ab2::launch_dense(q, s->d.nx, s->d.nu, s->d.nc, st));
-  else if (s->k && s->variant != 9)
-    CUDA_TRY(s->k->launch(q, s->variant, s->group_doubles, st, nullptr));
+  else if (warp)
+    CUDA_TRY(s->k->launch(q, s->variant == 9 ? -1 : s->variant, s->group_doubles, st, nullptr));
   else
     CUDA_TRY(ab2::launch_block(q, s->d.nx, s->d.nu, s->d.nc, st, nullptr));
   s->launches += 1;
@@ -632,6 +669,7 @@
   if (bwd) {
     s->have_backward = true;
     s->fac_head = 0;
+    s->vxx_packed = warp_kernel(s);
   }
   s->have_forward = fwd != 0;
   return AB2_OK;
@@ -702,6 +740,27 @@
 
 static int copy_ring(const double *base, size_t rec, int knots, int nring, int head, int b0, int nb, int t0, int nt,
                      double *dst, cudaMemcpyKind kind, cudaStream_t st);
+
+static int get_vxx_packed(ab2_gar_solver *s, int head, int b0, int nb, int t0, int nt, double *dst, int memspace,
+                          cudaStream_t st) {
+  const size_t n = (size_t)nb * nt * s->d.nx * s->d.nx;
+  if (n == 0)
+    return AB2_OK;
+  double *out = dst;
+  if (memspace != AB2_DEVICE)
+    CUDA_TRY(cudaMallocAsync(&out, n * sizeof(double), st));
+  long blocks = (long)((n + 255) / 256);
+  if (blocks > s->p.num_sms * 8L)
+    blocks = s->p.num_sms * 8L;
+  ab2::vxx_expand_kernel<<<(int)blocks, 256, 0, st>>>(s->out[AB2_OUT_VXX], s->p.Vxx0, out, s->d.horizon, s->d.nx, head,
+                                                      b0, nb, t0, nt);
+  CUDA_TRY(cudaGetLastError());
+  if (memspace != AB2_DEVICE) {
+    CUDA_TRY(cudaMemcpyAsync(dst, out, n * sizeof(double), cudaMemcpyDeviceToHost, st));
+    CUDA_TRY(cudaFreeAsync(out, st));
+  }
+  return AB2_OK;
+}
 
 int ab2_gar_problem_ptr(ab2_gar_solver *s, int what, const double **out) {
   if (!s || !out || what < 0 || what > 3)
@@ -927,7 +986,10 @@
     for (int i = 0; i < nwhat; ++i) {
       const int w = whats[i];
       const size_t per_inst = (size_t)s->out_knots[w] * s->out_rec[w];
-      if (per_inst)
+      if (w == AB2_OUT_VXX && warp_kernel(s)) {
+        if ((rc = get_vxx_packed(s, 0, b0, nb, 0, N + 1, dsts[i] + (size_t)b0 * per_inst, AB2_HOST, st)) != AB2_OK)
+          return rc;
+      } else if (per_inst)
         CUDA_TRY(cudaMemcpyAsync(dsts[i] + (size_t)b0 * per_inst, s->out[w] + (size_t)b0 * per_inst,
                                  (size_t)nb * per_inst * sizeof(double), cudaMemcpyDeviceToHost, st));
     }
@@ -939,6 +1001,7 @@
   s->have_backward = true;
   s->have_forward = true;
   s->fac_head = 0;
+  s->vxx_packed = warp_kernel(s);
   return AB2_OK;
 }
 
@@ -979,6 +1042,8 @@
   CUDA_TRY(cudaSetDevice(s->d.device));
   if (s->out_doubles[what] == 0)
     return AB2_OK;
+  if (what == AB2_OUT_VXX && s->vxx_packed)
+    return get_vxx_packed(s, s->fac_head, 0, s->d.batch, 0, s->d.horizon + 1, dst, memspace, (cudaStream_t)stream);
   if (ring_indexed(s, what))
     return copy_ring(s->out[what], s->out_rec[what], s->out_knots[what], s->d.horizon, s->fac_head, 0, s->d.batch, 0,
                      s->out_knots[what], dst, memspace == AB2_DEVICE ? cudaMemcpyDeviceToDevice : cudaMemcpyDeviceToHost,
@@ -1000,6 +1065,8 @@
   const size_t rec = s->out_rec[what];
   if (rec == 0 || nb == 0 || nt == 0)
     return AB2_OK;
+  if (what == AB2_OUT_VXX && s->vxx_packed)
+    return get_vxx_packed(s, s->fac_head, b0, nb, t0, nt, dst, memspace, (cudaStream_t)stream);
   if (ring_indexed(s, what))
     return copy_ring(s->out[what], rec, knots, s->d.horizon, s->fac_head, b0, nb, t0, nt, dst,
                      memspace == AB2_DEVICE ? cudaMemcpyDeviceToDevice : cudaMemcpyDeviceToHost, (cudaStream_t)stream);
@@ -1329,7 +1396,8 @@
   if ((rc = ab2_gar_backward(s, 1.0, stream)) != AB2_OK)
     return rc;
   double *vxo = Vx_out ? Vx_out : s->fddp_vx;
-  ab2::fddp_vx_kernel<<<s->p.num_sms * 4, 256, 0, st>>>(s->out[AB2_OUT_VXX], s->out[AB2_OUT_VX], in->fs, vxo, B, N, nx);
+  ab2::fddp_vx_kernel<<<s->p.num_sms * 4, 256, 0, st>>>(s->out[AB2_OUT_VXX], s->vxx_packed ? s->p.Vxx0 : nullptr,
+                                                      s->out[AB2_OUT_VX], in->fs, vxo, B, N, nx);
   CUDA_TRY(cudaGetLastError());
   s->launches += 1;
   if (Quuks_out) {
@@ -1386,12 +1454,14 @@
     s->fac_head = (s->fac_head + 1) % N;
     const int slot = (N - 1 + s->fac_head) % N;
     for (int w : {AB2_OUT_FF, AB2_OUT_FB, AB2_OUT_VXX, AB2_OUT_VX}) {
-      const size_t rec = s->out_rec[w];
+      const size_t rec = (w == AB2_OUT_VXX && s->vxx_packed) ? (size_t)ab2::vxx_packed_doubles(s->d.nx) : s->out_rec[w];
       if (rec == 0)
         continue;
       CUDA_TRY(cudaMemset2DAsync(s->out[w] + (size_t)slot * rec, (size_t)s->out_knots[w] * rec * sizeof(double), 0,
                                  rec * sizeof(double), (size_t)B, st));
     }
+    if (s->vxx_packed && ab2::vxx_slot_is_full(slot))
+      CUDA_TRY(cudaMemsetAsync(s->p.Vxx0, 0, (size_t)B * s->d.nx * s->d.nx * sizeof(double), st));
   }
   if (s->out_doubles[AB2_OUT_KKT0])
     CUDA_TRY(cudaMemsetAsync(s->out[AB2_OUT_KKT0], 0, s->out_doubles[AB2_OUT_KKT0] * sizeof(double), st));
diff --git a/aligator_b200/csrc/riccati_group.cuh b/aligator_b200/csrc/riccati_group.cuh
--- a/aligator_b200/csrc/riccati_group.cuh
+++ b/aligator_b200/csrc/riccati_group.cuh
@@ -4,6 +4,8 @@
 #include <cstddef>
 #include <cstdint>
 #include <utility>
+
+#include "vxx_layout.h"
 
 #if defined(__CUDACC__)
 #define AB2_HD __host__ __device__ __forceinline__
@@ -65,6 +67,7 @@
   int peer_world;
   double *peer_dst[8];
   long long peer_off;
+  double *Vxx0;
 };
 
 enum : int { ST_CONDENSED_FACTOR_FAILED = 4 };
@@ -76,9 +79,13 @@
 AB2_HD int leg_begin(int N, int i, int T) { return (int)((long long)i * (N + 1) / T); }
 AB2_HD int cond_offset(int b, int nc0, int nx) { return b == 0 ? 0 : nc0 + (b - 1) * nx; }
 
-template <int NX_, int NU_, int NC_, int G_, bool DB_ = false, bool RB_ = true, bool MMA_ = false> struct Cfg {
+template <int NX_, int NU_, int NC_, int G_, bool DB_ = false, bool RB_ = true, bool MMA_ = false, bool PK_ = false>
+struct Cfg {
   static constexpr int NX = NX_, NU = NU_, NC = NC_, G = G_;
   static constexpr bool DB = DB_;
+  static constexpr bool VXX_PACKED = PK_;
+  static constexpr int VP = vxx_packed_doubles(NX);
+  static constexpr int VXX_REC = PK_ ? VP : NX * NX;
   static constexpr int NCOL = NX + NU + 1;
   static constexpr int NXU = NX + NU;
   static constexpr int NK = NU + NC;
@@ -112,7 +119,8 @@
 #define AB2_PARK 1
 #endif
   static constexpr bool PARK = MMA_ && DB_ && (AB2_PARK != 0);
-  static constexpr int LUT_INTS = MMA ? 32 * (NT + NT * NT) : 0;
+  static constexpr int VPU = (PK_ && MMA_) ? (VP / 2 + 31) / 32 : 0;
+  static constexpr int LUT_INTS = MMA ? 32 * (NT + NT * NT + VPU) : 0;
   static constexpr int OFF_A = 0;
   static constexpr int OFF_B = OFF_A + NX * NX;
   static constexpr int OFF_F = OFF_B + NX * NU;
@@ -181,11 +189,10 @@
   static constexpr bool FWD_FUSED = FB_BULK && (NX % 2 == 0) && (NR + NX <= G);
   static constexpr int FWD_ROWS = FWD_FUSED ? NR + NX : NR;
   static constexpr bool FWD_FF = FWD_FUSED && (NR % 2 == 0);
-  static constexpr int FWD_SLOT =
-      FWD_FUSED ? (NR + NX) * NX + NX + (FWD_FF ? NR : 0) : ev(NR * NX);
+  static constexpr int FWD_BIAS = NR * NX + VXX_REC;
+  static constexpr int FWD_SLOT = FWD_FUSED ? FWD_BIAS + NX + (FWD_FF ? NR : 0) : ev(NR * NX);
   static constexpr int FWD_RING_RAW = (S_STAGE_END - 2 * ev(NX)) / FWD_SLOT;
-  static constexpr int FWD_RING_MIN =
-      FWD_FUSED ? ((5 * FWD_SLOT + 2 * ev(NX)) * 100 <= S_STAGE_END * 112 ? 5 : 4) : 1;
+  static constexpr int FWD_RING_MIN = FWD_FUSED ? 4 : 1;
   static constexpr int FWD_RING = FWD_RING_RAW > 8 ? 8 : (FWD_RING_RAW < FWD_RING_MIN ? FWD_RING_MIN : FWD_RING_RAW);
   static constexpr int NXE = ev(NX);
   static constexpr int FWD_END = FWD_RING * FWD_SLOT + 2 * ev(NX);
@@ -869,6 +876,19 @@
       lut[r * 32 + lane] = (int)(u0 | (u1 << 16));
     }
   }
+  for (int r = NT + NT * NT + first; r < NT + NT * NT + C::VPU; r += step) {
+    const int e0 = 2 * ((r - NT - NT * NT) * 32 + lane);
+    unsigned u[2];
+    for (int e = 0; e < 2; ++e) {
+      u[e] = 0xffffu;
+      if (e0 + e < C::NX * (C::NX + 1) / 2) {
+        int i, j;
+        vxx_packed_coords(C::NX, e0 + e, i, j);
+        u[e] = (unsigned)(j * C::VS + i);
+      }
+    }
+    lut[r * 32 + lane] = (int)(u[0] | (u[1] << 16));
+  }
 }
 
 template <class C, class Ctx>
@@ -883,7 +903,8 @@
 #define AB2_STAGE_B (p.stage + (size_t)inst * N * C::SREC_PAD)
 #define AB2_FF_B (p.ff + (size_t)inst * N * NR)
 #define AB2_FB_B (p.fb + (size_t)inst * N * NR * NX)
-#define AB2_VXX_B (p.Vxx + (size_t)inst * (N + 1) * NX * NX)
+#define AB2_VXX_B (p.Vxx + (size_t)inst * (N + 1) * C::VXX_REC)
+#define AB2_VXX0_B (C::VXX_PACKED ? p.Vxx0 + (size_t)inst * NX * NX : AB2_VXX_B)
 #define AB2_VX_B (p.vx + (size_t)inst * (N + 1) * NX)
   double *Vn = sm + C::S_VN;
   double *vxn = sm + C::S_VXN;
@@ -1159,7 +1180,7 @@
               const double v = VV[mt][nt][e];
               if (jj < NX) {
                 if (t == 0)
-                  AB2_VXX_B[i + jj * NX] = v;
+                  AB2_VXX0_B[i + jj * NX] = v;
                 if (i >= jj) {
                   Vn[i * VS + jj] = v;
                   Vn[jj * VS + i] = v;
@@ -1177,8 +1198,18 @@
       ctx.async_fence();
     ctx.sync();
     if (t > 0) {
-      double *Vt = AB2_VXX_B + (size_t)t * NX * NX;
-      if (C::VXX_BULK) {
+      double *Vt = AB2_VXX_B + (size_t)t * C::VXX_REC;
+      if constexpr (C::VXX_PACKED) {
+        AB2_UNROLL
+        for (int u = 0; u < C::VPU; ++u) {
+          const int e = 2 * (u * 32 + lane);
+          if (e < C::VP) {
+            const unsigned o = (unsigned)lut[(NT + NT * NT + u) * 32 + lane];
+            const unsigned o0 = o & 0xffffu, o1 = o >> 16;
+            stg2(Vt + e, o0 == 0xffffu ? 0.0 : Vn[o0], o1 == 0xffffu ? 0.0 : Vn[o1]);
+          }
+        }
+      } else if (C::VXX_BULK) {
         ctx.bulk_store(Vt, Vn, NX * NX);
       } else if (lane < NX) {
         if (C::EVEN && (VS % 2 == 0)) {
@@ -1204,7 +1235,19 @@
 #undef AB2_FF_B
 #undef AB2_FB_B
 #undef AB2_VXX_B
+#undef AB2_VXX0_B
 #undef AB2_VX_B
+
+template <class C> AB2_D void store_packed_column(double *dst, const double *Vn, const int lane) {
+  constexpr int NX = C::NX;
+  double *col = dst + vxx_packed_col(NX, lane) - lane;
+  AB2_UNROLL
+  for (int i = 0; i < NX; ++i)
+    if (i >= lane)
+      col[i] = Vn[lane * C::VS + i];
+  if (C::VP > NX * (NX + 1) / 2 && lane == 0)
+    dst[C::VP - 1] = 0.0;
+}
 
 template <class C, class Ctx>
 AB2_D void riccati_group_sweep(Ctx &ctx, const SweepParams &p, const int inst,
@@ -1231,7 +1274,8 @@
   const double *stage_b = p.stage + (size_t)inst * N * C::SREC_PAD;
   double *ff_b = p.ff + (size_t)inst * N * NR;
   double *fb_b = p.fb + (size_t)inst * N * NR * NX;
-  double *Vxx_b = p.Vxx + (size_t)inst * (N + 1) * NX * NX;
+  double *Vxx_b = p.Vxx + (size_t)inst * (N + 1) * C::VXX_REC;
+  double *Vxx0_b = C::VXX_PACKED ? p.Vxx0 + (size_t)inst * NX * NX : Vxx_b;
   double *vx_b = p.vx + (size_t)inst * (N + 1) * NX;
   int st = ST_OK;
   int pv = 0;
@@ -1263,7 +1307,7 @@
       const double *qt = tr + NX * NX;
       const double *Ct = qt + NX;
       const double *dt = Ct + (size_t)nct * NX;
-      double *VN = Vxx_b + (size_t)N * NX * NX;
+      double *VN = N > 0 ? Vxx_b + (size_t)N * C::VXX_REC : Vxx0_b;
       if (colA || colF) {
         double acc[NX];
         AB2_UNROLL
@@ -1289,7 +1333,8 @@
             vx_b[(size_t)N * NX + i] = s;
             vxn[i] = s;
           } else {
-            VN[i + lane * NX] = s;
+            if (!C::VXX_PACKED || N == 0)
+              VN[i + lane * NX] = s;
             if (i >= lane) {
               Vn[i * C::VS + lane] = s;
               Vn[lane * C::VS + i] = s;
@@ -1299,9 +1344,13 @@
       }
       ctx.sync();
       if (colA && N > 0) {
-        AB2_UNROLL
-        for (int i = 0; i < NX; ++i)
-          VN[i + lane * NX] = Vn[lane * C::VS + i];
+        if constexpr (C::VXX_PACKED)
+          store_packed_column<C>(VN, Vn, lane);
+        else {
+          AB2_UNROLL
+          for (int i = 0; i < NX; ++i)
+            VN[i + lane * NX] = Vn[lane * C::VS + i];
+        }
       }
     }
 
@@ -1512,7 +1561,7 @@
         }
         if (colA) {
           if (t == 0) {
-            double *Vt = Vxx_b;
+            double *Vt = Vxx0_b;
             AB2_UNROLL
             for (int i = 0; i < NX; ++i)
               Vt[i + lane * NX] = h[i];
@@ -1535,10 +1584,14 @@
         ctx.proxy_fence_smem();
       ctx.sync();
       if (t > 0 && colA) {
-        double *Vt = Vxx_b + (size_t)t * NX * NX;
-        AB2_UNROLL
-        for (int i = 0; i < NX; ++i)
-          Vt[i + lane * NX] = Vn[lane * C::VS + i];
+        double *Vt = Vxx_b + (size_t)t * C::VXX_REC;
+        if constexpr (C::VXX_PACKED)
+          store_packed_column<C>(Vt, Vn, lane);
+        else {
+          AB2_UNROLL
+          for (int i = 0; i < NX; ++i)
+            Vt[i + lane * NX] = Vn[lane * C::VS + i];
+        }
       }
     }
 
@@ -1654,14 +1707,16 @@
     ctx.sync();
     auto fill_slot = [&](int d, int t) {
       if (FUSED) {
-        ctx.copy_expect(d, (t < N ? NR * NX + (C::FWD_FF ? NR : 0) : 0) + NX * NX + NX);
+        constexpr int VR = C::VXX_REC;
+        ctx.copy_expect(d, (t < N ? NR * NX + (C::FWD_FF ? NR : 0) : 0) + (t > 0 ? VR : 0) + NX);
         if (t < N) {
           ctx.copy_add(d, ring + d * FS, fb_b + (size_t)t * NR * NX, NR * NX);
           if (C::FWD_FF)
-            ctx.copy_add(d, ring + d * FS + (NR + NX) * NX + NX, ff_b + (size_t)t * NR, NR);
-        }
-        ctx.copy_add(d, ring + d * FS + NR * NX, Vxx_b + (size_t)t * NX * NX, NX * NX);
-        ctx.copy_add(d, ring + d * FS + (NR + NX) * NX, vx_b + (size_t)t * NX, NX);
+            ctx.copy_add(d, ring + d * FS + C::FWD_BIAS + NX, ff_b + (size_t)t * NR, NR);
+        }
+        if (t > 0)
+          ctx.copy_add(d, ring + d * FS + NR * NX, Vxx_b + (size_t)t * VR, VR);
+        ctx.copy_add(d, ring + d * FS + C::FWD_BIAS, vx_b + (size_t)t * NX, NX);
       } else if (C::FB_BULK) {
         ctx.issue_copy(d, ring + d * FS, fb_b + (size_t)t * NR * NX, NR * NX);
       } else {
@@ -1704,14 +1759,20 @@
             if (FUSED ? ((r < NR && t < N) || (r >= NR && r < ROWS && t >= 1)) : (r < NR)) {
               double s0 = gff[d][q], s1 = 0.0;
               if (FUSED && (C::FWD_FF || r >= NR))
-                s0 = slot[(NR + NX) * NX + (r >= NR ? r - NR : NX + r)];
+                s0 = slot[C::FWD_BIAS + (r >= NR ? r - NR : NX + r)];
               if (EVF) {
                 constexpr bool ROT = ((NX / 2) % 4) == 2;
                 const int rot2 = ROT ? ((r >> 1) & 2) : 0;
                 AB2_UNROLL
                 for (int c = 0; c < NX; c += 2) {
                   const int cc = (ROT && c + 2 == NX) ? (rot2 ? 0 : c) : c + rot2;
-                  const D2 gg = lds2(slot + r * NX + cc);
+                  D2 gg;
+                  if (C::VXX_PACKED && FUSED && r >= NR) {
+                    gg.x = slot[NR * NX + vxx_packed_index(NX, r - NR, cc)];
+                    gg.y = slot[NR * NX + vxx_packed_index(NX, r - NR, cc + 1)];
+                  } else {
+                    gg = lds2(slot + r * NX + cc);
+                  }
                   const D2 xx = lds2(xc + cc);
                   s0 += gg.x * xx.x;
                   s1 += gg.y * xx.y;
@@ -1749,7 +1810,7 @@
     }
     if (!FUSED) {
       constexpr int KPI = (C::G / NX) > 0 ? (C::G / NX) : 1;
-      constexpr int U = 2;
+      constexpr int U = C::VXX_PACKED ? 1 : 2;
       const int sub = lane / NX, i = lane % NX;
       if (sub < KPI) {
         for (int t = sub; t < N; t += KPI * U) {
@@ -1758,7 +1819,19 @@
           for (int u = 0; u < U; ++u) {
             const int tt = t + u * KPI;
             if (tt < N) {
-              load_row<NX, EVF>(Vxx_b + ((size_t)(tt + 1) * NX + i) * NX, vrow[u]);
+              if constexpr (C::VXX_PACKED) {
+                const double *V = Vxx_b + (size_t)(tt + 1) * C::VXX_REC;
+                const double *lo = V + vxx_packed_col(NX, i) - i, *up = V + i;
+                AB2_UNROLL
+                for (int c = 0; c < NX; ++c) {
+                  if (c >= i)
+                    vrow[u][c] = lo[c];
+                  else
+                    vrow[u][c] = up[vxx_packed_col(NX, c) - c];
+                }
+              } else {
+                load_row<NX, EVF>(Vxx_b + ((size_t)(tt + 1) * NX + i) * NX, vrow[u]);
+              }
               load_row<NX, EVF>(xs_b + (size_t)(tt + 1) * NX, xr[u]);
               v0[u] = vx_b[(size_t)(tt + 1) * NX + i];
             }
diff --git a/aligator_b200/csrc/riccati_launch.cuh b/aligator_b200/csrc/riccati_launch.cuh
--- a/aligator_b200/csrc/riccati_launch.cuh
+++ b/aligator_b200/csrc/riccati_launch.cuh
@@ -225,12 +225,12 @@
 
 template <int NX, int NU, int NC, int G>
 inline cudaError_t launch_cfg(const SweepParams &p, int variant, const int gd[4], cudaStream_t st, int *info) {
-  using CS = Cfg<NX, NU, NC, G, false>;
-  using CD = Cfg<NX, NU, NC, G, true>;
+  using CS = Cfg<NX, NU, NC, G, false, true, false, true>;
+  using CD = Cfg<NX, NU, NC, G, true, true, false, true>;
   if (variant < 0) {
     variant = 6;
     if constexpr (G == 32 && NC == 0 && NX % 2 == 0) {
-      using CM = Cfg<NX, NU, NC, G, true, true, true>;
+      using CM = Cfg<NX, NU, NC, G, true, true, true, true>;
       const int sms = p.num_sms > 0 ? p.num_sms : 132;
       const int grid = (p.batch + 1) / 2;
       auto ctas = [&](int gdw, int cap) {
@@ -258,31 +258,31 @@
   if (variant == 3)
     return launch_one<CS, 4, 72, false>(p, gd[0], st, info);
   if (variant == 4)
-    return launch_one<Cfg<NX, NU, NC, G, false, false>, 4, 72, true>(p, gd[0], st, info);
+    return launch_one<Cfg<NX, NU, NC, G, false, false, false, true>, 4, 72, true>(p, gd[0], st, info);
   if (variant == 5)
-    return launch_one<Cfg<NX, NU, NC, G, true, false>, 2, 144, true>(p, gd[1], st, info);
+    return launch_one<Cfg<NX, NU, NC, G, true, false, false, true>, 2, 144, true>(p, gd[1], st, info);
   if (variant == 6)
     return launch_one<CD, 2, 128, true>(p, gd[1], st, info);
   if constexpr (G == 32 && NC == 0 && NX % 2 == 0) {
-    using CM = Cfg<NX, NU, NC, G, true, true, true>;
+    using CM = Cfg<NX, NU, NC, G, true, true, true, true>;
     if (variant == 7)
       return launch_one<CM, 2, 128, true>(p, gd[2], st, info);
     if (variant == 8)
       return launch_one<CM, 2, 168, true>(p, gd[2], st, info);
     if (variant == 10)
-      return launch_one<Cfg<NX, NU, NC, G, false, true, true>, 2, 128, true>(p, gd[3], st, info);
+      return launch_one<Cfg<NX, NU, NC, G, false, true, true, true>, 2, 128, true>(p, gd[3], st, info);
   }
   return launch_one<CD, 2, 144, true>(p, gd[1], st, info);
 }
 template <int NX, int NU, int NC, int G> inline void group_doubles_cfg(int nc0, int gd[4]) {
-  gd[0] = Cfg<NX, NU, NC, G, false>::group_doubles(nc0);
-  gd[1] = Cfg<NX, NU, NC, G, true>::group_doubles(nc0);
+  gd[0] = Cfg<NX, NU, NC, G, false, true, false, true>::group_doubles(nc0);
+  gd[1] = Cfg<NX, NU, NC, G, true, true, false, true>::group_doubles(nc0);
   gd[2] = gd[1];
   gd[3] = gd[0];
   if constexpr (G == 32 && NC == 0 && NX % 2 == 0) {
-    gd[2] = Cfg<NX, NU, NC, G, true, true, true>::group_doubles(nc0);
-    gd[3] = Cfg<NX, NU, NC, G, false, true, true>::group_doubles(nc0);
-  }
-}
-
-}
+    gd[2] = Cfg<NX, NU, NC, G, true, true, true, true>::group_doubles(nc0);
+    gd[3] = Cfg<NX, NU, NC, G, false, true, true, true>::group_doubles(nc0);
+  }
+}
+
+}
diff --git a/aligator_b200/csrc/vxx_layout.h b/aligator_b200/csrc/vxx_layout.h
--- /dev/null
+++ b/aligator_b200/csrc/vxx_layout.h
@@ -0,0 +1,26 @@
+#pragma once
+
+#if defined(__CUDACC__)
+#define AB2_VXX_HD __host__ __device__ __forceinline__
+#else
+#define AB2_VXX_HD inline
+#endif
+
+namespace ab2 {
+
+AB2_VXX_HD constexpr int vxx_packed_doubles(int nx) { return (nx * (nx + 1) / 2 + 1) & ~1; }
+AB2_VXX_HD constexpr int vxx_packed_col(int nx, int j) { return j * nx - j * (j - 1) / 2; }
+AB2_VXX_HD constexpr int vxx_packed_index(int nx, int i, int j) {
+  return i >= j ? vxx_packed_col(nx, j) + (i - j) : vxx_packed_col(nx, i) + (j - i);
+}
+AB2_VXX_HD constexpr bool vxx_slot_is_full(int slot) { return slot == 0; }
+AB2_VXX_HD void vxx_packed_coords(int nx, int e, int &i, int &j) {
+  j = 0;
+  while (e >= nx - j) {
+    e -= nx - j;
+    ++j;
+  }
+  i = j + e;
+}
+
+}
```

Measured after the change: 254.2 million, median of 6. +6.4%, better.
